# hlesmqh/WS3D

Measured on AMD Instinct MI355X. Metric: KITTI scenes/sec (16384 pts) Stage-1 RPN fwd, 1/2/4/8 GPU; FPS+group HBM GB/s, higher is better.
Workload: dtype f32

## Files before the change

### include/ws3d_ops.h

```cpp
#ifndef WS3D_OPS_H
#define WS3D_OPS_H

#include <stddef.h>
#include <stdint.h>

#ifdef __cplusplus
extern "C" {
#endif

#define WS3D_OK 0
#define WS3D_E_INVALID (-1)
#define WS3D_E_LAUNCH (-2)
#define WS3D_E_WORKSPACE (-3)
#define WS3D_E_UNSUPPORTED (-4)

#if defined(__GNUC__)
#define WS3D_API __attribute__((visibility("default")))
#else
#define WS3D_API
#endif

typedef void *ws3d_stream_t;

#define WS3D_ABI_VERSION 6
WS3D_API int ws3d_abi_version(void);
WS3D_API int ws3d_tune(int key, int value);
WS3D_API int ws3d_dist_mode(void);
WS3D_API const char *ws3d_last_error(void);
WS3D_API int ws3d_device_info(char *name, int name_len, int *cu_count, int *lds_bytes_per_block);


WS3D_API int ws3d_furthest_point_sampling(int b, int n, int m, const float *xyz, float *temp, int32_t *idx,
                                 ws3d_stream_t stream);

WS3D_API int ws3d_furthest_point_sampling_gather(int b, int n, int m, const float *xyz, float *temp,
                                        int32_t *idx, float *new_xyz, ws3d_stream_t stream);

WS3D_API size_t ws3d_fps_workspace_bytes(int b, int n);
WS3D_API int ws3d_furthest_point_sampling_ws(int b, int n, int m, const float *xyz, float *temp, int32_t *idx,
                                             float *new_xyz , void *workspace, size_t workspace_bytes,
                                             ws3d_stream_t stream);

WS3D_API int ws3d_furthest_point_sampling_nested(int b, int n, int m, const float *xyz, int32_t *idx, float *new_xyz,
                                        ws3d_stream_t stream);

WS3D_API int ws3d_furthest_point_sampling_nested_chain(int b, int n, int levels, const int *m, const float *xyz, int32_t *const *idx,
                                                       float *const *new_xyz, ws3d_stream_t stream);

WS3D_API int ws3d_fps_ragged_limit(void);
WS3D_API int ws3d_furthest_point_sampling_ragged(int clouds, const int32_t *offsets, const int32_t *sizes_host, int m, const float *xyz,
                                                 int32_t *idx, ws3d_stream_t stream);

WS3D_API int ws3d_gather_points(int b, int c, int n, int npoints, const float *points, const int32_t *idx,
                       float *out, ws3d_stream_t stream);

WS3D_API int ws3d_gather_points_grad(int b, int c, int n, int npoints, const float *grad_out,
                            const int32_t *idx, float *grad_points, ws3d_stream_t stream);

WS3D_API int ws3d_ball_query(int b, int n, int m, float radius, int nsample, const float *new_xyz,
                    const float *xyz, int32_t *idx, const void *sorted, ws3d_stream_t stream);
WS3D_API int ws3d_ball_query_fill(int b, int n, int m, float radius, int nsample, const float *new_xyz,
                         const float *xyz, int32_t *idx, const void *sorted, ws3d_stream_t stream);
WS3D_API int ws3d_ball_query_pairs(int b, int n, int m, float radius, int nsample, const float *new_xyz, const float *xyz, int32_t *idx,
                          const void *sorted_grid, int32_t *rowc, int32_t *rowsrc, int32_t *total, ws3d_stream_t stream);

WS3D_API int ws3d_ball_query_pairs2(int b, int n, int m, const float *new_xyz, const float *xyz, const void *sorted_grid,
                                    float radius0, int nsample0, int32_t *idx0, int32_t *rowc0, int32_t *rowsrc0, int32_t *total0,
                                    float radius1, int nsample1, int32_t *idx1, int32_t *rowc1, int32_t *rowsrc1, int32_t *total1,
                                    ws3d_stream_t stream);


WS3D_API size_t ws3d_sorted_points_bytes(int b, int n);
WS3D_API int ws3d_sort_points_x(int b, int n, const float *xyz, void *sorted, ws3d_stream_t stream);
WS3D_API int ws3d_sort_points_xz(int b, int n, const float *xyz, void *sorted, ws3d_stream_t stream);
WS3D_API int ws3d_sort_points_grid(int b, int n, const float *xyz, void *sorted, ws3d_stream_t stream);
WS3D_API int ws3d_sort_points_jobs(int b, int njobs, const int *n, const int *kind, const float *const *xyz, void *const *sorted,
                                   ws3d_stream_t stream);

WS3D_API int ws3d_group_points(int b, int c, int n, int npoints, int nsample, const float *points,
                      const int32_t *idx, float *out, ws3d_stream_t stream);

WS3D_API int ws3d_group_points_grad(int b, int c, int n, int npoints, int nsample, const float *grad_out,
                           const int32_t *idx, float *grad_points, ws3d_stream_t stream);

WS3D_API int ws3d_query_and_group(int b, int n, int m, int c, float radius, int nsample, int use_xyz,
                         const float *xyz, const float *new_xyz, const float *features,
                         int32_t *idx_out, float *out, const void *sorted, ws3d_stream_t stream);

WS3D_API int ws3d_three_nn(int b, int n, int m, const float *unknown, const float *known, float *dist2,
                  int32_t *idx, const void *sorted_known, ws3d_stream_t stream);

WS3D_API int ws3d_three_nn_weights(long rows, const float *dist2, float *weight, ws3d_stream_t stream);
WS3D_API int ws3d_three_nn_w(int b, int n, int m, const float *unknown, const float *known, float *dist2, int32_t *idx, float *weight,
                             const void *sorted_known, ws3d_stream_t stream);
WS3D_API int ws3d_three_nn_wq(int b, int n, int m, const float *unknown, const float *known, float *dist2, int32_t *idx, float *weight,
                              const void *sorted_known, const void *sorted_unknown, ws3d_stream_t stream);
WS3D_API int ws3d_three_nn_jobs(int b, int njobs, const int *n, const int *m, const float *const *unknown, const void *const *sorted_known,
                                float *const *dist2, int32_t *const *idx, float *const *weight, const void *const *sorted_unknown,
                                ws3d_stream_t stream);

WS3D_API int ws3d_pool_nsample(long rows, int nsample, const float *x, float *out, uint8_t *arg, ws3d_stream_t stream);
WS3D_API int ws3d_pool_nsample_grad(long rows, int nsample, const float *grad_out, const uint8_t *arg, float *grad_x,
                                    ws3d_stream_t stream);

WS3D_API int ws3d_gemm_pool(long rows, int nsample, int k_dim, int o_dim, const float *x_rows, const float *wt,
                            const float *bias, int relu, float *out, int out_stride, const int32_t *gate, long gate_limit, ws3d_stream_t stream);

WS3D_API int ws3d_gather_gemm(int b, int n, int m, int nsample, int c_feat, int o_dim, const float *feats, const float *xyz,
                     const float *new_xyz, const int32_t *nbr, const float *wt, const float *bias, int relu, float *out,
                     ws3d_stream_t stream);

WS3D_API int ws3d_gather_gemm2(int b, int n, int m, int nsample, int c_feat, int o1, int o2, const float *feats, const float *xyz,
                      const float *new_xyz, const int32_t *nbr, const float *w1t, const float *b1, int relu1, const float *w2t,
                      const float *b2, int relu2, float *out, ws3d_stream_t stream);

WS3D_API int ws3d_pgather_gemm2(int b, int n, int m, int nsample, int o1, int o2, const float *pmat, int p_stride, const float *xyz,
                       const float *new_xyz, const int32_t *nbr, const float *w1x, const float *b1, int relu1,
                       const float *w2t, const float *b2, int relu2, float *out, const int32_t *gate, long gate_limit, ws3d_stream_t stream);
WS3D_API int ws3d_pgather_rows(int b, int n, int m, int nsample, int o1, const float *pmat, int p_stride, const float *xyz, const float *new_xyz,
                      const int32_t *nbr, const float *w1x, const float *b1, int relu1, float *out, ws3d_stream_t stream);

WS3D_API int ws3d_qinterp_rows(int b, int n, int m, int o, const float *q, const int32_t *idx, const float *weight, const float *lin,
                      const float *skip, int c1, const float *wb, const float *bias, int relu, float *out, ws3d_stream_t stream);


WS3D_API int ws3d_compact_pairs(long centres, int nsample, const int32_t *nbr, int32_t *rowc, int32_t *rowsrc, int32_t *total, ws3d_stream_t stream);
WS3D_API int ws3d_compact_pairs_count(long centres, int nsample, const int32_t *nbr, int32_t *cnt, ws3d_stream_t stream);
WS3D_API int ws3d_compact_pairs_rows(long centres, int nsample, const int32_t *nbr, const int32_t *cnt, const int32_t *incl, int32_t *rowc,
                            int32_t *rowsrc, int32_t *total, ws3d_stream_t stream);
WS3D_API int ws3d_pgather_gemm2_compact(int b, int n, int m, long max_rows, int o1, int o2, const float *pmat, int p_stride, const float *xyz,
                               const float *new_xyz, const int32_t *rowc, const int32_t *rowsrc, const int32_t *total, const float *w1x,
                               const float *b1, int relu1, const float *w2t, const float *b2, int relu2, float *out, long limit, ws3d_stream_t stream);
WS3D_API int ws3d_pgather_gemm3_compact(int b, int n, int m, long max_rows, int o1, int o2, int o3, const float *pmat, int p_stride, const float *xyz,
                               const float *new_xyz, const int32_t *rowc, const int32_t *rowsrc, const int32_t *total, const float *w1x,
                               const float *b1, int relu1, const float *w2t, const float *b2, int relu2, const float *w3t, const float *b3,
                               float *out, int out_stride, long limit, ws3d_stream_t stream);
WS3D_API int ws3d_gemm_pool_compact(long max_rows, int k_dim, int o_dim, const float *x_rows, const int32_t *rowc, const int32_t *total,
                           const float *wt, const float *bias, float *out, int out_stride, long limit, ws3d_stream_t stream);
typedef struct ws3d_compact_mlp_args {
    int b, n, m;
    long max_rows;
    int o1, o2, o3;
    const float *pmat;
    int p_stride;
    const float *xyz, *new_xyz;
    const int32_t *rowc, *rowsrc, *total;
    const float *w1x, *b1;
    int relu1;
    const float *w2t, *b2;
    int relu2;
    const float *w3t, *b3;
    float *mid;
    float *out;
    int out_stride;
    long limit;
} ws3d_compact_mlp_args;
WS3D_API int ws3d_compact_mlp_pair(int kind, const ws3d_compact_mlp_args *scale0, const ws3d_compact_mlp_args *scale1, ws3d_stream_t stream);
WS3D_API int ws3d_chain_mlp3_ticket_ints(void);
WS3D_API size_t ws3d_chain_mlp3_blob_floats(int o2);
WS3D_API int ws3d_chain_mlp3_pack(const ws3d_compact_mlp_args *scale, float *blob, ws3d_stream_t stream);
WS3D_API int ws3d_chain_mlp3(const ws3d_compact_mlp_args *scale0, const ws3d_compact_mlp_args *scale1, const float *blob0, const float *blob1,
                             int32_t *ticket, int workgroups, ws3d_stream_t stream);

WS3D_API int ws3d_sa_mlp3_pool_compact(int b, int n, int m, long max_rows, int c1, int c2, int c3, const float *xyz, const float *new_xyz,
                              const float *feat, const int32_t *rowc, const int32_t *rowsrc, const int32_t *total, const float *w1t,
                              const float *b1, const float *w2t, const float *b2, const float *w3t, const float *b3, float *out,
                              int out_stride, long limit, ws3d_stream_t stream);

WS3D_API int ws3d_sa_mlp3_pool_lists(int b, int n, int m, int nsample, int c1, int c2, int c3, const float *xyz, const float *new_xyz,
                            const float *feat, const int32_t *nbr, const float *w1t, const float *b1, const float *w2t, const float *b2,
                            const float *w3t, const float *b3, int relu3, float *out, int out_stride, const int32_t *gate, long gate_limit,
                            ws3d_stream_t stream);

WS3D_API int ws3d_interp_gemm(int b, int n, int m, int c2, int c1, int o_dim, const float *known_feats, const float *unknown_feats,
                     const int32_t *idx, const float *weight, const float *wt, const float *bias, int relu, float *out,
                     ws3d_stream_t stream);

WS3D_API size_t ws3d_conv1x1_wgrad_workspace_bytes(int b, int o, int c, long l);
WS3D_API int ws3d_conv1x1_wgrad(int b, int o, int c, long l, const float *grad_out, const float *x, float *grad_w,
                                void *workspace, size_t workspace_bytes, ws3d_stream_t stream);

WS3D_API size_t ws3d_bn_workspace_bytes(int b, int c, long l);
WS3D_API int ws3d_bn_relu_train_fwd(int b, int c, long l, const float *x, const float *gamma, const float *beta, float eps,
                                    float momentum, int relu, float *running_mean, float *running_var,
                                    int64_t *num_batches_tracked, float *y, float *save_mean, float *save_invstd,
                                    void *workspace, size_t workspace_bytes, ws3d_stream_t stream);
WS3D_API int ws3d_bn_relu_train_bwd(int b, int c, long l, const float *x, const float *dy, const float *gamma,
                                    const float *beta, const float *save_mean, const float *save_invstd, int relu, float *dx,
                                    float *dgamma, float *dbeta, void *workspace, size_t workspace_bytes, ws3d_stream_t stream);

WS3D_API int ws3d_three_interpolate(int b, int c, int m, int n, const float *points, const int32_t *idx,
                           const float *weight, float *out, ws3d_stream_t stream);

WS3D_API int ws3d_three_interpolate_grad(int b, int c, int n, int m, const float *grad_out,
                                const int32_t *idx, const float *weight, float *grad_points,
                                ws3d_stream_t stream);

WS3D_API size_t ws3d_scatter_workspace_bytes(int b, int c, int n_targets, long slots_per_scene);
WS3D_API int ws3d_group_points_grad_det(int b, int c, int n, int npoints, int nsample, const float *grad_out,
                                        const int32_t *idx, float *grad_points, void *workspace,
                                        size_t workspace_bytes, ws3d_stream_t stream);
WS3D_API int ws3d_three_interpolate_grad_det(int b, int c, int n, int m, const float *grad_out, const int32_t *idx,
                                             const float *weight, float *grad_points, void *workspace,
                                             size_t workspace_bytes, ws3d_stream_t stream);

WS3D_API int ws3d_bias_act_inplace(int b, int o_ch, long l, int relu, float *y, const float *bias,
                                   ws3d_stream_t stream);

WS3D_API int ws3d_rowmax_bias_act(int b, int o_ch, long m, int s, int relu, const float *y, const float *bias,
                                  float *out, ws3d_stream_t stream);

WS3D_API int ws3d_query_and_group_nlc(int b, int n, int m, int c, float radius, int nsample, int use_xyz,
                                      const float *xyz, const float *new_xyz, const float *features_nlc,
                                      int32_t *idx_out, float *out_nlc, const void *sorted, ws3d_stream_t stream);
WS3D_API int ws3d_three_interpolate_nlc(int b, int c, int m, int n, const float *feats_nlc, const int32_t *idx,
                                        const float *weight, float *out_nlc, int out_stride, ws3d_stream_t stream);
WS3D_API int ws3d_rowmax_rows(long rows_out, int ns, int o_ch, const float *y, float *out, int out_stride,
                              ws3d_stream_t stream);

WS3D_API int ws3d_sa_mlp3_pool(long rows, int nsample, int c1, int c2, int c3, const float *x_rows4,
                               const float *w1t, const float *b1, const float *w2t, const float *b2,
                               const float *w3t, const float *b3, int relu3, float *out, int out_stride,
                               ws3d_stream_t stream);

WS3D_API int ws3d_mlp2_rows(long rows, int k_dim, int o1, int o2, const float *x_rows, const float *w1t, const float *b1, int relu1,
                   const float *w2t, const float *b2, int relu2, float *out, int *ticket, ws3d_stream_t stream);

WS3D_API size_t ws3d_rpn_heads_blob_bytes(int o2);
WS3D_API int ws3d_rpn_heads_pack(int o2, const float *w1t, const float *b1, int relu1, const float *w2t, const float *b2, int relu2, void *blob,
                        ws3d_stream_t stream);
WS3D_API int ws3d_rpn_heads(long rows, const float *x_rows, int heads, const void *blob_cls, float *out_cls, int *ticket_cls, int o2_reg,
                   const void *blob_reg, float *out_reg, int *ticket_reg, int workgroups, ws3d_stream_t stream);

WS3D_API size_t ws3d_gemm_rows_pack_bytes(int k_dim, int n_dim);
WS3D_API int ws3d_gemm_rows_pack(int k_dim, int n_dim, const float *wt, void *pack, ws3d_stream_t stream);
WS3D_API int ws3d_gemm_rows_split(long rows, int k_dim, int n_dim, const float *a, const void *pack, const float *bias, int relu, float *out,
                         ws3d_stream_t stream);

WS3D_API int ws3d_qinterp_gemm(int b, int n, int m, int c, int o_dim, const float *q, const int32_t *idx, const float *weight, const float *lin,
                      const float *skip, int c1, const float *wb, const float *b1, int relu1, const float *w2t, const float *b2, int relu2,
                      float *out, ws3d_stream_t stream);


WS3D_API int ws3d_boxes_overlap_bev(int num_a, const float *boxes_a, int num_b, const float *boxes_b,
                           float *ans, ws3d_stream_t stream);

WS3D_API int ws3d_boxes_iou_bev(int num_a, const float *boxes_a, int num_b, const float *boxes_b,
                       float *ans, ws3d_stream_t stream);

WS3D_API int ws3d_boxes_iou3d_paired(int n, const float *boxes_a, const float *boxes_b, float *overlap_bev, float *iou2d, float *iou3d,
                                     ws3d_stream_t stream);

WS3D_API int ws3d_nms_mask(int boxes_num, const float *boxes, float thresh, int normal, int full_grid,
                  uint64_t *mask, ws3d_stream_t stream);

WS3D_API size_t ws3d_nms_workspace_bytes(int boxes_num);
WS3D_API int ws3d_nms(int boxes_num, const float *boxes, float thresh, int normal, int max_keep,
                      void *workspace, size_t workspace_bytes, int64_t *keep, int32_t *num_keep,
                      ws3d_stream_t stream);

WS3D_API int ws3d_nms_batched(int batch, int boxes_num, const float *boxes, float thresh, int normal,
                              int max_keep, void *workspace, size_t workspace_bytes, int64_t *keep,
                              int32_t *num_keep, ws3d_stream_t stream);


WS3D_API int ws3d_radius_nms_batched(int batch, int n, const float *centers, float radius, int max_keep,
                                     void *workspace, size_t workspace_bytes, int64_t *keep,
                                     int32_t *num_keep, ws3d_stream_t stream);

WS3D_API int ws3d_topk_sorted(int b, int n, int k, const float *scores, float *out_scores, int64_t *out_idx,
                              ws3d_stream_t stream);
WS3D_API size_t ws3d_topk_workspace_bytes(int b, int n);
WS3D_API int ws3d_topk_sorted_ws(int b, int n, int k, const float *scores, float *out_scores, int64_t *out_idx, void *workspace,
                                 size_t workspace_bytes, ws3d_stream_t stream);
WS3D_API int ws3d_topk_sorted_sigmoid(int b, int n, int k, const float *logits, float *out_scores, int64_t *out_idx, ws3d_stream_t stream);
WS3D_API int ws3d_topk_sorted_sigmoid_ws(int b, int n, int k, const float *logits, float *out_scores, int64_t *out_idx, void *workspace,
                                         size_t workspace_bytes, ws3d_stream_t stream);

WS3D_API int ws3d_decode_center_boxes(int b, int n, int bins, float loc_scope, float loc_bin_size, float h, float w,
                                      float l, const float *xyz, const float *rpn_reg, float *boxes,
                                      ws3d_stream_t stream);

WS3D_API int ws3d_gather_boxes_bev(int b, int n, int top, const float *box, const int64_t *order, float *box_sorted, float *bev,
                          ws3d_stream_t stream);
WS3D_API int ws3d_decode_gather_boxes_bev(int b, int n, int top, int bins, float loc_scope, float loc_bin_size, float h, float w, float l,
                                          const float *xyz, const float *rpn_reg, const int64_t *order, float *box_sorted, float *bev,
                                          ws3d_stream_t stream);
WS3D_API int ws3d_select_proposals(int b, int top, int keep_stride, int k, const float *box_sorted, const float *scores_sorted,
                          const int64_t *keep, const int32_t *num, float extra_width, float *boxes_out, float *scores_out,
                          int64_t *count, float *pooled_boxes, ws3d_stream_t stream);
WS3D_API int ws3d_select_proposals_packed(int b, int top, int keep_stride, int k, const float *box_sorted, const float *scores_sorted,
                                          const int64_t *keep, const int32_t *num, float extra_width, float *boxes_out, float *scores_out,
                                          int64_t *count, float *pooled_boxes, float *packed, ws3d_stream_t stream);
WS3D_API int ws3d_select_proposals_send(int b, int top, int keep_stride, int k, const float *box_sorted, const float *scores_sorted,
                                        const int64_t *keep, const int32_t *num, float extra_width, float *boxes_out, float *scores_out,
                                        int64_t *count, float *pooled_boxes, float *send, long send_stride, ws3d_stream_t stream);
WS3D_API int ws3d_split_points_clear(long rows, int c, const float *pc, float *xyz, float *feats, void *clear, size_t clear_bytes,
                                     ws3d_stream_t stream);


WS3D_API int ws3d_roipool3d(int batch_size, int pts_num, int boxes_num, int feature_in_len,
                   int sampled_pts_num, const float *xyz, const float *boxes3d,
                   const float *pts_feature, float *pooled_features, int32_t *pooled_empty_flag,
                   int32_t *pts_idx, ws3d_stream_t stream);
WS3D_API int ws3d_roipool3d_fill(int batch_size, int pts_num, int boxes_num, int feature_in_len,
                   int sampled_pts_num, const float *xyz, const float *boxes3d,
                   const float *pts_feature, float *pooled_features, int32_t *pooled_empty_flag,
                   int32_t *pts_idx, ws3d_stream_t stream);

WS3D_API size_t ws3d_roipool3d_workspace_bytes(int batch_size, int pts_num);
WS3D_API int ws3d_roipool3d_ws(int batch_size, int pts_num, int boxes_num, int feature_in_len, int sampled_pts_num, const float *xyz,
                               const float *boxes3d, const float *pts_feature, float *pooled_features, int32_t *pooled_empty_flag,
                               int32_t *pts_idx, int fill, void *workspace, size_t workspace_bytes, ws3d_stream_t stream);


WS3D_API int ws3d_pts_in_boxes3d(int boxes_num, int pts_num, const float *pts, const float *boxes3d,
                        int64_t *flag, ws3d_stream_t stream);


WS3D_API int ws3d_instance_clouds(int batch, int pts_num, int centres_num, int feat_len, int sampled_pts_num, float radius, int mask_mode,
                                  float mask_thresh, const float *pts, const float *score, const float *feats, const float *centres,
                                  const int32_t *num, float *cloud, float *cloud_feats, int32_t *count, int32_t *pts_idx,
                                  ws3d_stream_t stream);
WS3D_API int ws3d_instance_clouds_count(int batch, int pts_num, int centres_num, float radius, const float *pts, const float *centres,
                                        const int32_t *num, int32_t *count, ws3d_stream_t stream);
WS3D_API int ws3d_instance_clouds_emit(int batch, int pts_num, int centres_num, int feat_len, float radius, int mask_mode, float mask_thresh,
                                       const float *pts, const float *score, const float *feats, const float *centres, const int32_t *num,
                                       const int64_t *offsets, float *rows, float *row_feats, int32_t *row_idx, ws3d_stream_t stream);


WS3D_API int ws3d_click_prepare(int batch, int pts_num, int clicks_num, int side, const float *offsets, float gauss_height, float gauss_status,
                                float gauss_cov, float centre_y, const float *pts, const float *clicks, const int32_t *num, float *score,
                                float *cand, int32_t *cand_num, ws3d_stream_t stream);



WS3D_API int ws3d_kitti_overlaps(int metric, int criterion, int frames, long max_pairs, const int32_t *gt_off, const int32_t *dt_off,
                                 const int64_t *out_off, const double *dt_boxes, const double *gt_boxes, double *out,
                                 ws3d_stream_t stream);

WS3D_API int ws3d_kitti_collect_scores(int frames, int max_dt, const int32_t *gt_off, const int32_t *dt_off, const int64_t *out_off,
                                       const double *overlaps, const int32_t *ignored_gt, const int32_t *ignored_dt,
                                       const double *dt_score, double min_overlap, double *tp_score, int32_t *tp_flag,
                                       ws3d_stream_t stream);

WS3D_API size_t ws3d_kitti_count_workspace_bytes(int frames, int num_thresh);
WS3D_API int ws3d_kitti_count(int metric, int frames, int max_dt, int num_thresh, const double *thresholds, const int32_t *gt_off,
                              const int32_t *dt_off, const int32_t *dc_off, const int64_t *out_off, const double *overlaps,
                              const int32_t *ignored_gt, const int32_t *ignored_dt, const double *dt_score, const double *dt_alpha,
                              const double *gt_alpha, const double *dt_bbox, const double *dc_bbox, double min_overlap, int compute_aos,
                              void *workspace, size_t workspace_bytes, double *pr, ws3d_stream_t stream);


WS3D_API int ws3d_stage2_embed(long rows, int pts_per_cloud, const float *pts, const float *box_ce, float extend, const float *wx0,
                               const float *bx0, const float *wx1, const float *bx1, const float *wf0, const float *bf0, const float *wf1,
                               const float *bf1, const float *wm, const float *bm, float *xyz_out, float *feat, ws3d_stream_t stream);
WS3D_API int ws3d_stage2_boxes(int rows, int loc_bins, int head_bins, float loc_scope, float h, float w, float l, const float *rcnn_reg,
                               float *pred_boxes3d, float *box_ce, ws3d_stream_t stream);
WS3D_API int ws3d_stage2_select(int batch, int slots, float cls_thresh, float iou_thresh, const float *size_window, float ground_y,
                                const float *box_ce, const float *rcnn_ref, const float *rcnn_cls, const float *rcnn_iou, const float *center,
                                const int32_t *num, float *boxes, int32_t *keep, float *key, ws3d_stream_t stream);

WS3D_API int ws3d_stage2_canonical_ragged(int rows, int clouds, const int32_t *offsets, const float *pts, const float *box_ce, float extend,
                                          float *pts_out, ws3d_stream_t stream);
WS3D_API int ws3d_furthest_point_sampling_ragged_gather(int clouds, const int32_t *offsets, const int32_t *sizes_host, int m, const float *xyz,
                                                        int32_t *idx, float *new_xyz, ws3d_stream_t stream);
WS3D_API int ws3d_ball_query_ragged(int clouds, const int32_t *offsets, int m, float radius, int nsample, const float *xyz, const float *new_xyz,
                                    int global_rows, int32_t *idx, ws3d_stream_t stream);

WS3D_API int ws3d_stage2_rcnn_loss(int rows, int loc_bins, int head_bins, float loc_scope, float h, float w, float l, const float *rcnn_cls,
                                   const float *rcnn_reg, const float *pred_boxes3d, const float *gt_boxes, const float *cls, float *vals,
                                   int32_t *counts, float *grad_cls, float *grad_reg, ws3d_stream_t stream);
WS3D_API int ws3d_stage2_ioun_loss(int rows, const float *rcnn_iou, const float *rcnn_ref, const float *pred_boxes3d, const float *refined_box,
                                   const float *gt_boxes, const float *cls, float *vals, int32_t *counts, float *grad_iou, float *grad_ref,
                                   ws3d_stream_t stream);

WS3D_API int ws3d_rpn_center_labels(int batch, int n, int kmax, int pts_stride, float gauss_height, float gauss_status, double gauss_cov,
                                    const float *pts, const float *centres, const int32_t *count, float *cls_label, float *reg_label,
                                    ws3d_stream_t stream);
WS3D_API size_t ws3d_rpn_loss_workspace_bytes(int rows);
WS3D_API int ws3d_rpn_loss(int rows, int bins, double loc_scope, double loc_bin_size, double alpha, double gamma, double weight_cls,
                           double weight_reg, const float *rpn_cls, const float *rpn_reg, const float *cls_label, const float *reg_label,
                           float *vals, int32_t *counts, float *grad_cls, float *grad_reg, void *workspace, size_t workspace_bytes,
                           ws3d_stream_t stream);

WS3D_API int ws3d_scan_prepare_limit(void);
WS3D_API size_t ws3d_scan_prepare_workspace_bytes(int scenes, long total_points);
WS3D_API int ws3d_scan_prepare(int scenes, const int32_t *offsets, long total_points, int max_scan_points, const float *raw, const float *calib,
                               const int32_t *img_hw, const float *scope, int npoints, uint64_t seed, const int64_t *scene_key, int key_bits,
                               float *pts_input, int32_t *src_index, int32_t *valid_count, int32_t *status, void *workspace,
                               size_t workspace_bytes, ws3d_stream_t stream);


WS3D_API int ws3d_roipool3d_plan(int batch_size, int pts_num, int boxes_num, int feature_in_len, int sampled_pts_num, int aligned16,
                                 size_t workspace_bytes);

WS3D_API int ws3d_ball_query_plan(int b, int n, int m, int c, int nsample, int fused, int nlc, int flavour, int pairs, int scales, int wide_nw,
                                  int32_t *plan);

#ifdef __cplusplus
}
#endif
#endif
```

### ws3d_amd/_lib.py

```python
from __future__ import annotations

import ctypes as C
import os

_HERE = os.path.dirname(os.path.abspath(__file__))
DIST_MODE = int(os.environ.get("WS3D_DIST_MODE", "0") or 0)
LIB_PATH = os.environ.get("WS3D_HIP_LIB") or os.path.join(
    _HERE, "libws3d_hip.so" if DIST_MODE == 0 else "libws3d_hip_dm%d.so" % DIST_MODE)

E_INVALID, E_LAUNCH, E_WORKSPACE, E_UNSUPPORTED = -1, -2, -3, -4
ABI_VERSION = 6

_vp = C.c_void_p
_i = C.c_int
_f = C.c_float
_sz = C.c_size_t

class CompactMlpArgs(C.Structure):
    _fields_ = [("b", _i), ("n", _i), ("m", _i), ("max_rows", C.c_long), ("o1", _i), ("o2", _i), ("o3", _i), ("pmat", _vp), ("p_stride", _i),
                ("xyz", _vp), ("new_xyz", _vp), ("rowc", _vp), ("rowsrc", _vp), ("total", _vp), ("w1x", _vp), ("b1", _vp), ("relu1", _i),
                ("w2t", _vp), ("b2", _vp), ("relu2", _i), ("w3t", _vp), ("b3", _vp), ("mid", _vp), ("out", _vp), ("out_stride", _i), ("limit", C.c_long)]


SIGNATURES = {
    "ws3d_abi_version": (_i, []),
    "ws3d_tune": (_i, [_i, _i]),
    "ws3d_dist_mode": (_i, []),
    "ws3d_last_error": (C.c_char_p, []),
    "ws3d_device_info": (_i, [C.c_char_p, _i, C.POINTER(_i), C.POINTER(_i)]),
    "ws3d_furthest_point_sampling": (_i, [_i, _i, _i, _vp, _vp, _vp, _vp]),
    "ws3d_furthest_point_sampling_gather": (_i, [_i, _i, _i, _vp, _vp, _vp, _vp, _vp]),
    "ws3d_furthest_point_sampling_nested": (_i, [_i, _i, _i, _vp, _vp, _vp, _vp]),
    "ws3d_furthest_point_sampling_nested_chain": (_i, [_i, _i, _i, _vp, _vp, _vp, _vp, _vp]),
    "ws3d_fps_ragged_limit": (_i, []),
    "ws3d_furthest_point_sampling_ragged": (_i, [_i, _vp, _vp, _i, _vp, _vp, _vp]),
    "ws3d_fps_workspace_bytes": (_sz, [_i, _i]),
    "ws3d_furthest_point_sampling_ws": (_i, [_i, _i, _i, _vp, _vp, _vp, _vp, _vp, _sz, _vp]),
    "ws3d_gather_points": (_i, [_i, _i, _i, _i, _vp, _vp, _vp, _vp]),
    "ws3d_gather_points_grad": (_i, [_i, _i, _i, _i, _vp, _vp, _vp, _vp]),
    "ws3d_ball_query": (_i, [_i, _i, _i, _f, _i, _vp, _vp, _vp, _vp, _vp]),
    "ws3d_ball_query_fill": (_i, [_i, _i, _i, _f, _i, _vp, _vp, _vp, _vp, _vp]),
    "ws3d_ball_query_pairs": (_i, [_i, _i, _i, _f, _i, _vp, _vp, _vp, _vp, _vp, _vp, _vp, _vp]),
    "ws3d_ball_query_pairs2": (_i, [_i, _i, _i, _vp, _vp, _vp, C.c_float, _i, _vp, _vp, _vp, _vp, C.c_float, _i, _vp, _vp, _vp, _vp, _vp]),
    "ws3d_sorted_points_bytes": (_sz, [_i, _i]),
    "ws3d_sort_points_x": (_i, [_i, _i, _vp, _vp, _vp]),
    "ws3d_sort_points_xz": (_i, [_i, _i, _vp, _vp, _vp]),
    "ws3d_sort_points_grid": (_i, [_i, _i, _vp, _vp, _vp]),
    "ws3d_sort_points_jobs": (_i, [_i, _i, _vp, _vp, _vp, _vp, _vp]),
    "ws3d_group_points": (_i, [_i, _i, _i, _i, _i, _vp, _vp, _vp, _vp]),
    "ws3d_group_points_grad": (_i, [_i, _i, _i, _i, _i, _vp, _vp, _vp, _vp]),
    "ws3d_query_and_group": (_i, [_i, _i, _i, _i, _f, _i, _i, _vp, _vp, _vp, _vp, _vp, _vp, _vp]),
    "ws3d_three_nn": (_i, [_i, _i, _i, _vp, _vp, _vp, _vp, _vp, _vp]),
    "ws3d_three_interpolate": (_i, [_i, _i, _i, _i, _vp, _vp, _vp, _vp, _vp]),
    "ws3d_three_interpolate_grad": (_i, [_i, _i, _i, _i, _vp, _vp, _vp, _vp, _vp]),
    "ws3d_bn_workspace_bytes": (C.c_size_t, [_i, _i, C.c_long]),
    "ws3d_bn_relu_train_fwd": (_i, [_i, _i, C.c_long, _vp, _vp, _vp, C.c_float, C.c_float, _i, _vp, _vp, _vp, _vp, _vp, _vp,
                                    _vp, C.c_size_t, _vp]),
    "ws3d_bn_relu_train_bwd": (_i, [_i, _i, C.c_long, _vp, _vp, _vp, _vp, _vp, _vp, _i, _vp, _vp, _vp, _vp, C.c_size_t, _vp]),
    "ws3d_conv1x1_wgrad_workspace_bytes": (C.c_size_t, [_i, _i, _i, C.c_long]),
    "ws3d_conv1x1_wgrad": (_i, [_i, _i, _i, C.c_long, _vp, _vp, _vp, _vp, C.c_size_t, _vp]),
    "ws3d_gemm_pool": (_i, [C.c_long, _i, _i, _i, _vp, _vp, _vp, _i, _vp, _i, _vp, C.c_long, _vp]),
    "ws3d_pool_nsample": (_i, [C.c_long, _i, _vp, _vp, _vp, _vp]),
    "ws3d_pool_nsample_grad": (_i, [C.c_long, _i, _vp, _vp, _vp, _vp]),
    "ws3d_scatter_workspace_bytes": (C.c_size_t, [_i, _i, _i, C.c_long]),
    "ws3d_group_points_grad_det": (_i, [_i, _i, _i, _i, _i, _vp, _vp, _vp, _vp, C.c_size_t, _vp]),
    "ws3d_three_interpolate_grad_det": (_i, [_i, _i, _i, _i, _vp, _vp, _vp, _vp, _vp, C.c_size_t, _vp]),
    "ws3d_query_and_group_nlc": (_i, [_i, _i, _i, _i, _f, _i, _i, _vp, _vp, _vp, _vp, _vp, _vp, _vp]),
    "ws3d_three_interpolate_nlc": (_i, [_i, _i, _i, _i, _vp, _vp, _vp, _vp, _i, _vp]),
    "ws3d_rowmax_rows": (_i, [C.c_long, _i, _i, _vp, _vp, _i, _vp]),
    "ws3d_sa_mlp3_pool": (_i, [C.c_long, _i, _i, _i, _i, _vp, _vp, _vp, _vp, _vp, _vp, _vp, _i, _vp, _i, _vp]),
    "ws3d_qinterp_gemm": (_i, [_i, _i, _i, _i, _i, _vp, _vp, _vp, _vp, _vp, _i, _vp, _vp, _i, _vp, _vp, _i, _vp, _vp]),
    "ws3d_mlp2_rows": (_i, [C.c_long, _i, _i, _i, _vp, _vp, _vp, _i, _vp, _vp, _i, _vp, _vp, _vp]),
    "ws3d_rpn_heads_blob_bytes": (_sz, [_i]),
    "ws3d_rpn_heads_pack": (_i, [_i, _vp, _vp, _i, _vp, _vp, _i, _vp, _vp]),
    "ws3d_rpn_heads": (_i, [C.c_long, _vp, _i, _vp, _vp, _vp, _i, _vp, _vp, _vp, _i, _vp]),
    "ws3d_gemm_rows_pack_bytes": (_sz, [_i, _i]),
    "ws3d_gemm_rows_pack": (_i, [_i, _i, _vp, _vp, _vp]),
    "ws3d_gemm_rows_split": (_i, [C.c_long, _i, _i, _vp, _vp, _vp, _i, _vp, _vp]),
    "ws3d_decode_center_boxes": (_i, [_i, _i, _i, _f, _f, _f, _f, _f, _vp, _vp, _vp, _vp]),
    "ws3d_topk_sorted": (_i, [_i, _i, _i, _vp, _vp, _vp, _vp]),
    "ws3d_topk_workspace_bytes": (C.c_size_t, [_i, _i]),
    "ws3d_topk_sorted_ws": (_i, [_i, _i, _i, _vp, _vp, _vp, _vp, C.c_size_t, _vp]),
    "ws3d_topk_sorted_sigmoid": (_i, [_i, _i, _i, _vp, _vp, _vp, _vp]),
    "ws3d_topk_sorted_sigmoid_ws": (_i, [_i, _i, _i, _vp, _vp, _vp, _vp, C.c_size_t, _vp]),
    "ws3d_three_nn_weights": (_i, [C.c_long, _vp, _vp, _vp]),
    "ws3d_three_nn_w": (_i, [_i, _i, _i, _vp, _vp, _vp, _vp, _vp, _vp, _vp]),
    "ws3d_three_nn_wq": (_i, [_i, _i, _i, _vp, _vp, _vp, _vp, _vp, _vp, _vp, _vp]),
    "ws3d_three_nn_jobs": (_i, [_i, _i, _vp, _vp, _vp, _vp, _vp, _vp, _vp, _vp, _vp]),
    "ws3d_bias_act_inplace": (_i, [_i, _i, C.c_long, _i, _vp, _vp, _vp]),
    "ws3d_rowmax_bias_act": (_i, [_i, _i, C.c_long, _i, _i, _vp, _vp, _vp, _vp]),
    "ws3d_boxes_overlap_bev": (_i, [_i, _vp, _i, _vp, _vp, _vp]),
    "ws3d_boxes_iou_bev": (_i, [_i, _vp, _i, _vp, _vp, _vp]),
    "ws3d_boxes_iou3d_paired": (_i, [_i, _vp, _vp, _vp, _vp, _vp, _vp]),
    "ws3d_nms_mask": (_i, [_i, _vp, _f, _i, _i, _vp, _vp]),
    "ws3d_nms_workspace_bytes": (_sz, [_i]),
    "ws3d_nms": (_i, [_i, _vp, _f, _i, _i, _vp, _sz, _vp, _vp, _vp]),
    "ws3d_nms_batched": (_i, [_i, _i, _vp, _f, _i, _i, _vp, _sz, _vp, _vp, _vp]),
    "ws3d_radius_nms_batched": (_i, [_i, _i, _vp, _f, _i, _vp, _sz, _vp, _vp, _vp]),
    "ws3d_gather_gemm": (_i, [_i, _i, _i, _i, _i, _i, _vp, _vp, _vp, _vp, _vp, _vp, _i, _vp, _vp]),
    "ws3d_gather_gemm2": (_i, [_i, _i, _i, _i, _i, _i, _i, _vp, _vp, _vp, _vp, _vp, _vp, _i, _vp, _vp, _i, _vp, _vp]),
    "ws3d_pgather_gemm2": (_i, [_i, _i, _i, _i, _i, _i, _vp, _i, _vp, _vp, _vp, _vp, _vp, _i, _vp, _vp, _i, _vp, _vp, C.c_long, _vp]),
    "ws3d_pgather_rows": (_i, [_i, _i, _i, _i, _i, _vp, _i, _vp, _vp, _vp, _vp, _vp, _i, _vp, _vp]),
    "ws3d_qinterp_rows": (_i, [_i, _i, _i, _i, _vp, _vp, _vp, _vp, _vp, _i, _vp, _vp, _i, _vp, _vp]),
    "ws3d_compact_pairs": (_i, [C.c_long, _i, _vp, _vp, _vp, _vp, _vp]),
    "ws3d_compact_pairs_count": (_i, [C.c_long, _i, _vp, _vp, _vp]),
    "ws3d_compact_pairs_rows": (_i, [C.c_long, _i, _vp, _vp, _vp, _vp, _vp, _vp, _vp]),
    "ws3d_pgather_gemm2_compact": (_i, [_i, _i, _i, C.c_long, _i, _i, _vp, _i, _vp, _vp, _vp, _vp, _vp, _vp, _vp, _i, _vp, _vp, _i, _vp, C.c_long, _vp]),
    "ws3d_pgather_gemm3_compact": (_i, [_i, _i, _i, C.c_long, _i, _i, _i, _vp, _i, _vp, _vp, _vp, _vp, _vp, _vp, _vp, _i, _vp, _vp, _i, _vp, _vp, _vp, _i, C.c_long, _vp]),
    "ws3d_gemm_pool_compact": (_i, [C.c_long, _i, _i, _vp, _vp, _vp, _vp, _vp, _vp, _i, C.c_long, _vp]),
    "ws3d_compact_mlp_pair": (_i, [_i, C.POINTER(CompactMlpArgs), C.POINTER(CompactMlpArgs), _vp]),
    "ws3d_chain_mlp3_ticket_ints": (_i, []),
    "ws3d_chain_mlp3_blob_floats": (_sz, [_i]),
    "ws3d_chain_mlp3_pack": (_i, [C.POINTER(CompactMlpArgs), _vp, _vp]),
    "ws3d_chain_mlp3": (_i, [C.POINTER(CompactMlpArgs), C.POINTER(CompactMlpArgs), _vp, _vp, _vp, _i, _vp]),
    "ws3d_sa_mlp3_pool_compact": (_i, [_i, _i, _i, C.c_long, _i, _i, _i, _vp, _vp, _vp, _vp, _vp, _vp, _vp, _vp, _vp, _vp, _vp, _vp, _vp, _i, C.c_long, _vp]),
    "ws3d_sa_mlp3_pool_lists": (_i, [_i, _i, _i, _i, _i, _i, _i, _vp, _vp, _vp, _vp, _vp, _vp, _vp, _vp, _vp, _vp, _i, _vp, _i, _vp, C.c_long, _vp]),
    "ws3d_interp_gemm": (_i, [_i, _i, _i, _i, _i, _i, _vp, _vp, _vp, _vp, _vp, _vp, _i, _vp, _vp]),
    "ws3d_gather_boxes_bev": (_i, [_i, _i, _i, _vp, _vp, _vp, _vp, _vp]),
    "ws3d_select_proposals": (_i, [_i, _i, _i, _i, _vp, _vp, _vp, _vp, _f, _vp, _vp, _vp, _vp, _vp]),
    "ws3d_decode_gather_boxes_bev": (_i, [_i, _i, _i, _i, _f, _f, _f, _f, _f, _vp, _vp, _vp, _vp, _vp, _vp]),
    "ws3d_select_proposals_packed": (_i, [_i, _i, _i, _i, _vp, _vp, _vp, _vp, _f, _vp, _vp, _vp, _vp, _vp, _vp]),
    "ws3d_select_proposals_send": (_i, [_i, _i, _i, _i, _vp, _vp, _vp, _vp, _f, _vp, _vp, _vp, _vp, _vp, C.c_long, _vp]),
    "ws3d_split_points_clear": (_i, [C.c_long, _i, _vp, _vp, _vp, _vp, C.c_size_t, _vp]),
    "ws3d_roipool3d": (_i, [_i, _i, _i, _i, _i, _vp, _vp, _vp, _vp, _vp, _vp, _vp]),
    "ws3d_roipool3d_fill": (_i, [_i, _i, _i, _i, _i, _vp, _vp, _vp, _vp, _vp, _vp, _vp]),
    "ws3d_roipool3d_workspace_bytes": (C.c_size_t, [_i, _i]),
    "ws3d_roipool3d_ws": (_i, [_i, _i, _i, _i, _i, _vp, _vp, _vp, _vp, _vp, _vp, _i, _vp, C.c_size_t, _vp]),
    "ws3d_pts_in_boxes3d": (_i, [_i, _i, _vp, _vp, _vp, _vp]),
    "ws3d_instance_clouds": (_i, [_i, _i, _i, _i, _i, _f, _i, _f, _vp, _vp, _vp, _vp, _vp, _vp, _vp, _vp, _vp, _vp]),
    "ws3d_instance_clouds_count": (_i, [_i, _i, _i, _f, _vp, _vp, _vp, _vp, _vp]),
    "ws3d_instance_clouds_emit": (_i, [_i, _i, _i, _i, _f, _i, _f, _vp, _vp, _vp, _vp, _vp, _vp, _vp, _vp, _vp, _vp]),
    "ws3d_click_prepare": (_i, [_i, _i, _i, _i, _vp, _f, _f, _f, _f, _vp, _vp, _vp, _vp, _vp, _vp, _vp]),
    "ws3d_kitti_overlaps": (_i, [_i, _i, _i, C.c_long, _vp, _vp, _vp, _vp, _vp, _vp, _vp]),
    "ws3d_kitti_collect_scores": (_i, [_i, _i, _vp, _vp, _vp, _vp, _vp, _vp, _vp, C.c_double, _vp, _vp, _vp]),
    "ws3d_kitti_count_workspace_bytes": (_sz, [_i, _i]),
    "ws3d_kitti_count": (_i, [_i, _i, _i, _i, _vp, _vp, _vp, _vp, _vp, _vp, _vp, _vp, _vp, _vp, _vp, _vp, _vp, C.c_double, _i, _vp,
                              _sz, _vp, _vp]),
    "ws3d_stage2_embed": (_i, [C.c_long, _i, _vp, _vp, _f] + [_vp] * 10 + [_vp, _vp, _vp]),
    "ws3d_stage2_boxes": (_i, [_i, _i, _i, _f, _f, _f, _f, _vp, _vp, _vp, _vp]),
    "ws3d_stage2_select": (_i, [_i, _i, _f, _f, C.POINTER(_f), _f, _vp, _vp, _vp, _vp, _vp, _vp, _vp, _vp, _vp, _vp]),
    "ws3d_stage2_canonical_ragged": (_i, [_i, _i, _vp, _vp, _vp, _f, _vp, _vp]),
    "ws3d_furthest_point_sampling_ragged_gather": (_i, [_i, _vp, _vp, _i, _vp, _vp, _vp, _vp]),
    "ws3d_ball_query_ragged": (_i, [_i, _vp, _i, _f, _i, _vp, _vp, _i, _vp, _vp]),
    "ws3d_stage2_rcnn_loss": (_i, [_i, _i, _i, _f, _f, _f, _f] + [_vp] * 9 + [_vp]),
    "ws3d_stage2_ioun_loss": (_i, [_i] + [_vp] * 10 + [_vp]),
    "ws3d_rpn_center_labels": (_i, [_i, _i, _i, _i, _f, _f, C.c_double] + [_vp] * 5 + [_vp]),
    "ws3d_rpn_loss_workspace_bytes": (_sz, [_i]),
    "ws3d_rpn_loss": (_i, [_i, _i] + [C.c_double] * 6 + [_vp] * 8 + [_vp, _sz, _vp]),
    "ws3d_scan_prepare_limit": (_i, []),
    "ws3d_scan_prepare_workspace_bytes": (_sz, [_i, C.c_long]),
    "ws3d_scan_prepare": (_i, [_i, _vp, C.c_long, _i, _vp, _vp, _vp, _vp, _i, C.c_uint64, _vp, _i, _vp, _vp, _vp, _vp, _vp, _sz, _vp]),
    "ws3d_roipool3d_plan": (_i, [_i, _i, _i, _i, _i, _i, _sz]),
    "ws3d_ball_query_plan": (_i, [_i, _i, _i, _i, _i, _i, _i, _i, _i, _i, _i, _vp]),
}


class Ws3dError(RuntimeError):
    pass


_lib = None


def load() -> C.CDLL:
    global _lib
    if _lib is not None:
        return _lib
    if not os.path.exists(LIB_PATH):
        raise Ws3dError(
            f"{LIB_PATH} is missing: the MI355X HIP library has not been built "
            "(run `python -m ws3d_amd.build`).  ws3d_amd has no CPU fallback.")
    import torch
    try:
        lib = C.CDLL(LIB_PATH)
    except OSError as e:
        raise Ws3dError(f"cannot load {LIB_PATH}: {e}") from e
    for name, (res, args) in SIGNATURES.items():
        fn = getattr(lib, name)
        fn.restype = res
        fn.argtypes = args
    if lib.ws3d_abi_version() != ABI_VERSION:
        raise Ws3dError(f"{LIB_PATH} exports ABI version {lib.ws3d_abi_version()}, this package binds version {ABI_VERSION}: "
                        "rebuild it (`python -m ws3d_amd.build`)")
    if not os.environ.get("WS3D_HIP_LIB") and lib.ws3d_dist_mode() != DIST_MODE:
        raise Ws3dError(f"{LIB_PATH} was built with WS3D_DIST_MODE={lib.ws3d_dist_mode()}, expected {DIST_MODE}: rebuild it")
    _lib = lib
    return lib


def check(rc: int, what: str = "") -> None:
    if rc != 0:
        msg = load().ws3d_last_error()
        raise Ws3dError(f"{what or 'ws3d'} failed (rc={rc}): {msg.decode() if msg else ''}")
```

### ws3d_amd/build.py

```python
from __future__ import annotations

import argparse
import concurrent.futures as cf
import glob
import os
import shutil
import subprocess
import sys

HERE = os.path.dirname(os.path.abspath(__file__))
CSRC = os.path.join(HERE, "csrc")
OBJ = os.path.join(CSRC, "build")
LIB = os.path.join(HERE, "libws3d_hip.so")
DIST_MODES = (0, 1, 2)


def lib_path(dist_mode: int = 0) -> str:
    return LIB if dist_mode == 0 else os.path.join(HERE, "libws3d_hip_dm%d.so" % dist_mode)
ARCH = "gfx950"
SOURCES = ["core.hip", "fps.hip", "fps_v3.hip", "fps_bucket.hip", "fps_nested.hip", "fps_ragged.hip", "fps_pruned.hip", "ballquery_group.hip", "interpolate.hip", "roipool3d.hip", "iou3d.hip", "proposals.hip", "scatter_det.hip", "sa_mlp.hip", "bn_relu.hip", "gemm_pool.hip", "conv_wgrad.hip", "chain_mlp.hip", "rpn_heads.hip", "gemm_rows.hip", "kitti_eval.hip", "instance_clouds.hip", "click.hip", "stage2.hip", "stage2_ragged.hip", "stage2_loss.hip", "rpn_targets.hip", "scan_prepare.hip"]
CXXFLAGS = ["-O3", "-std=c++17", "-fPIC", "-ffp-contract=off", "-fno-fast-math",
            "-fvisibility=hidden", "-Wall", "-Wno-unused-function"]


def hipcc() -> str:
    for cand in (os.environ.get("HIPCC"), shutil.which("hipcc"), "/opt/rocm/bin/hipcc"):
        if cand and os.path.exists(cand):
            return cand
    raise RuntimeError("hipcc not found (looked at $HIPCC, PATH, /opt/rocm/bin)")


def _deps(src: str):
    return [src, *glob.glob(os.path.join(CSRC, "*.h")), os.path.join(HERE, "..", "include", "ws3d_ops.h"),
            os.path.join(CSRC, "exports.map"), os.path.abspath(__file__)]


def _compile(src: str, force: bool, verbose: bool, dist_mode: int = 0) -> str:
    path = os.path.join(CSRC, src)
    obj = os.path.join(OBJ if dist_mode == 0 else OBJ + "_dm%d" % dist_mode, os.path.splitext(src)[0] + ".o")
    if not force and os.path.exists(obj) and all(
            os.path.getmtime(obj) >= os.path.getmtime(d) for d in _deps(path)):
        return obj
    cmd = [hipcc(), f"--offload-arch={ARCH}", *CXXFLAGS, f"-DWS3D_DIST_MODE={dist_mode}", *os.environ.get("WS3D_EXTRA_DEFS", "").split(), "-c", path, "-o", obj]
    if verbose:
        print(" ".join(cmd), flush=True)
    r = subprocess.run(cmd, capture_output=True, text=True)
    if r.returncode != 0:
        raise RuntimeError(f"hipcc failed for {src}:\n{r.stdout}\n{r.stderr}")
    if verbose and r.stderr.strip():
        print(r.stderr)
    return obj


def build(force: bool = False, verbose: bool = False, dist_mode: int = 0) -> str:
    LIB = lib_path(dist_mode)
    os.makedirs(OBJ if dist_mode == 0 else OBJ + "_dm%d" % dist_mode, exist_ok=True)
    with cf.ThreadPoolExecutor(max_workers=min(len(SOURCES), os.cpu_count() or 4, 16)) as ex:
        objs = list(ex.map(lambda s: _compile(s, force, verbose, dist_mode), SOURCES))
    if force or not os.path.exists(LIB) or any(os.path.getmtime(o) > os.path.getmtime(LIB) for o in objs):
        cmd = [hipcc(), f"--offload-arch={ARCH}", "-shared", "-fPIC", "-Wl,--version-script=" + os.path.join(CSRC, "exports.map"), "-o", LIB, *objs]
        if verbose:
            print(" ".join(cmd), flush=True)
        r = subprocess.run(cmd, capture_output=True, text=True)
        if r.returncode != 0:
            raise RuntimeError(f"link failed:\n{r.stdout}\n{r.stderr}")
    return LIB


def rebuild_one(src: str, verbose: bool = False) -> str:
    _compile(src, True, verbose)
    objs = [os.path.join(OBJ, os.path.splitext(s_)[0] + ".o") for s_ in SOURCES]
    missing = [o for o in objs if not os.path.exists(o)]
    if missing:
        return build(False, verbose)
    cmd = [hipcc(), f"--offload-arch={ARCH}", "-shared", "-fPIC", "-Wl,--version-script=" + os.path.join(CSRC, "exports.map"), "-o", LIB, *objs]
    r = subprocess.run(cmd, capture_output=True, text=True)
    if r.returncode != 0:
        raise RuntimeError(f"link failed:\n{r.stdout}\n{r.stderr}")
    return LIB


if __name__ == "__main__":
    ap = argparse.ArgumentParser()
    ap.add_argument("--force", action="store_true")
    ap.add_argument("--verbose", action="store_true")
    ap.add_argument("--dist-mode", type=int, default=0, choices=DIST_MODES)
    ap.add_argument("--all-dist-modes", action="store_true")
    ap.add_argument("--only", default=None, help="recompile this one source (forced) and relink")
    a = ap.parse_args()
    if a.only:
        print(rebuild_one(a.only, a.verbose))
        sys.exit(0)
    for dm in (DIST_MODES if a.all_dist_modes else (a.dist_mode,)):
        print(build(a.force, a.verbose, dm))
    sys.exit(0)
```

### ws3d_amd/compat.py

```python
from __future__ import annotations

import sys
import types

import os

import torch

from . import _lib
from ._lib import Ws3dError, check


def _dev(*tensors):
    dev = None
    for t in tensors:
        if t is None:
            continue
        if not t.is_cuda:
            raise Ws3dError("ws3d_amd ops need HIP ('cuda') tensors; there is no CPU fallback")
        if not t.is_contiguous():
            raise Ws3dError("ws3d_amd ops need contiguous tensors (the reference asserts the same)")
        if dev is None:
            dev = t.device
        elif t.device != dev:
# ... 378 lines not shown
    with _on(dev):
        check(_lib.load().ws3d_rowmax_rows(R, ns, O, _p(y), view.data_ptr(), out.size(1), _stream()), "rowmax_rows")
    return out


def bn_relu_train_fwd(x, gamma, beta, running_mean, running_var, momentum, eps, relu=True, num_batches_tracked=None):
    dev = _dev(x, gamma, beta, running_mean, running_var, num_batches_tracked)
    if num_batches_tracked is not None and num_batches_tracked.dtype != torch.int64:
        raise TypeError("num_batches_tracked must be int64")
    _f32(x, "x"); _f32(gamma, "gamma"); _f32(beta, "beta")
    b, c = x.size(0), x.size(1)
    l = x.numel() // max(b * c, 1)
    y = torch.empty_like(x)
    mean = torch.empty((c,), dtype=torch.float32, device=dev)
    invstd = torch.empty((c,), dtype=torch.float32, device=dev)
    lib = _lib.load()
    nbytes = lib.ws3d_bn_workspace_bytes(b, c, l)
    ws = torch.empty((nbytes + 7) // 8, dtype=torch.float64, device=dev)
    with _on(dev):
        check(lib.ws3d_bn_relu_train_fwd(b, c, l, _p(x), _p(gamma), _p(beta), float(eps), float(momentum), int(bool(relu)),
                                         _p(running_mean), _p(running_var), _p(num_batches_tracked), _p(y), _p(mean), _p(invstd), _p(ws), nbytes,
                                         _stream()), "bn_relu_train_fwd")
    return y, mean, invstd


def bn_relu_train_bwd(x, dy, gamma, beta, save_mean, save_invstd, relu=True):
    dev = _dev(x, dy, gamma, beta, save_mean, save_invstd)
    _f32(x, "x"); _f32(dy, "dy")
    b, c = x.size(0), x.size(1)
    l = x.numel() // max(b * c, 1)
    dx = torch.empty_like(x)
    dgamma = torch.empty((c,), dtype=torch.float32, device=dev)
    dbeta = torch.empty((c,), dtype=torch.float32, device=dev)
    lib = _lib.load()
    nbytes = lib.ws3d_bn_workspace_bytes(b, c, l)
    ws = torch.empty((nbytes + 7) // 8, dtype=torch.float64, device=dev)
    with _on(dev):
        check(lib.ws3d_bn_relu_train_bwd(b, c, l, _p(x), _p(dy), _p(gamma), _p(beta), _p(save_mean), _p(save_invstd),
                                         int(bool(relu)), _p(dx), _p(dgamma), _p(dbeta), _p(ws), nbytes, _stream()),
              "bn_relu_train_bwd")
    return dx, dgamma, dbeta


def conv1x1_wgrad(grad_out, x, shape=None):
    dev = _dev(grad_out, x)
    _f32(grad_out, "grad_out"); _f32(x, "x")
    b, o, c = x.size(0), grad_out.size(1), x.size(1)
    l = x.numel() // max(b * c, 1)
    if grad_out.numel() != b * o * l:
        raise Ws3dError("conv1x1_wgrad: grad_out and x disagree in shape")
    gw = torch.empty((o, c) if shape is None else tuple(shape), dtype=torch.float32, device=dev)
    lib = _lib.load()
    nbytes = lib.ws3d_conv1x1_wgrad_workspace_bytes(b, o, c, l)
    ws = torch.empty((nbytes + 3) // 4, dtype=torch.float32, device=dev)
    with _on(dev):
        check(lib.ws3d_conv1x1_wgrad(b, o, c, l, _p(grad_out), _p(x), _p(gw), _p(ws), nbytes, _stream()), "conv1x1_wgrad")
    return gw


def _gate(gate):
    if gate is None:
        return None, 0
    total, limit = gate
    return total.data_ptr(), int(limit)


def gemm_pool(x_rows, wt, bias, relu, nsample, out, col0=0, gate=None):
    dev = _dev(x_rows, wt, bias)
    _f32(x_rows, "x_rows"); _f32(wt, "wt")
    rows, k = x_rows.shape
    o = wt.size(1)
    if rows % 64 or rows // 64 > 65535 or o % 64 or k % 4 or nsample not in (16, 32) or wt.size(0) != k:
        return False
    view = out[:, col0:col0 + o]
    with _on(dev):
        check(_lib.load().ws3d_gemm_pool(rows, nsample, k, o, _p(x_rows), _p(wt), _p(bias), int(bool(relu)), view.data_ptr(),
                                         out.size(1), *_gate(gate), _stream()), "gemm_pool")
    return True


def gather_gemm(feats, xyz, new_xyz, nbr, wt_feat_then_xyz, bias, relu):
    dev = _dev(feats, xyz, new_xyz, nbr, wt_feat_then_xyz)
    _f32(feats, "feats"); _f32(xyz, "xyz"); _f32(new_xyz, "new_xyz"); _i32(nbr, "nbr"); _f32(wt_feat_then_xyz, "wt")
    B, N, C = feats.shape
    M, ns = nbr.size(1), nbr.size(2)
    O = wt_feat_then_xyz.size(1)
    rows = B * M * ns
    if C % 4 or O % 64 or rows % 64 or rows // 64 > 65535 or wt_feat_then_xyz.size(0) != C + 3 or not feats.is_contiguous():
        return None
    out = torch.empty((rows, O), dtype=torch.float32, device=dev)
    with _on(dev):
        check(_lib.load().ws3d_gather_gemm(B, N, M, ns, C, O, _p(feats), _p(xyz), _p(new_xyz), _p(nbr), _p(wt_feat_then_xyz), _p(bias),
                                           int(bool(relu)), _p(out), _stream()), "gather_gemm")
    return out


def gather_gemm2(feats, xyz, new_xyz, nbr, w1t_feat_then_xyz, b1, relu1, w2t, b2, relu2):
    dev = _dev(feats, xyz, new_xyz, nbr, w1t_feat_then_xyz, w2t)
    _f32(feats, "feats"); _f32(xyz, "xyz"); _f32(new_xyz, "new_xyz"); _i32(nbr, "nbr"); _f32(w1t_feat_then_xyz, "w1t"); _f32(w2t, "w2t")
    B, N, C = feats.shape
    M, ns = nbr.size(1), nbr.size(2)
    O1, O2 = w1t_feat_then_xyz.size(1), w2t.size(1)
    rows = B * M * ns
    if (C % 4 or O1 not in (64, 128, 256) or O2 % 4 or rows % 64 or w1t_feat_then_xyz.size(0) != C + 3 or w2t.size(0) != O1 or
            not feats.is_contiguous() or not w2t.is_contiguous() or not w1t_feat_then_xyz.is_contiguous()):
        return None
    out = torch.empty((rows, O2), dtype=torch.float32, device=dev)
    with _on(dev):
        check(_lib.load().ws3d_gather_gemm2(B, N, M, ns, C, O1, O2, _p(feats), _p(xyz), _p(new_xyz), _p(nbr), _p(w1t_feat_then_xyz), _p(b1),
                                            int(bool(relu1)), _p(w2t), _p(b2), int(bool(relu2)), _p(out), _stream()), "gather_gemm2")
    return out


def pgather_gemm2(pmat, col0, o1, xyz, new_xyz, nbr, w1x, b1, relu1, w2t, b2, relu2, out=None, gate=None):
    dev = _dev(pmat, xyz, new_xyz, nbr, w1x, w2t)
    _f32(pmat, "pmat"); _f32(xyz, "xyz"); _f32(new_xyz, "new_xyz"); _i32(nbr, "nbr"); _f32(w1x, "w1x"); _f32(w2t, "w2t")
    B, N = xyz.size(0), xyz.size(1)
    M, ns = nbr.size(1), nbr.size(2)
    O2 = w2t.size(1)
    if (o1 not in (64, 128) or O2 % 4 or (M * ns) % 64 or pmat.dim() != 2 or pmat.size(0) != B * N or pmat.stride(1) != 1 or
            col0 < 0 or col0 + o1 > pmat.size(1) or tuple(w1x.shape) != (3, o1) or w2t.size(0) != o1 or not w1x.is_contiguous() or not w2t.is_contiguous()):
        return None
    if out is None:
        out = torch.empty((B * M * ns, O2), dtype=torch.float32, device=dev)
    elif tuple(out.shape) != (B * M * ns, O2) or not out.is_contiguous():
        raise ValueError("pgather_gemm2: out must be a contiguous (B*M*ns, O2) tensor")
    with _on(dev):
        check(_lib.load().ws3d_pgather_gemm2(B, N, M, ns, o1, O2, pmat.data_ptr() + 4 * col0, pmat.stride(0), _p(xyz), _p(new_xyz), _p(nbr), _p(w1x), _p(b1),
                                             int(bool(relu1)), _p(w2t), _p(b2), int(bool(relu2)), _p(out), *_gate(gate), _stream()), "pgather_gemm2")
    return out


def pgather_rows(pmat, col0, o1, xyz, new_xyz, nbr, w1x, b1, relu1):
    dev = _dev(pmat, xyz, new_xyz, nbr, w1x)
    _f32(pmat, "pmat"); _f32(xyz, "xyz"); _f32(new_xyz, "new_xyz"); _i32(nbr, "nbr"); _f32(w1x, "w1x")
    B, N = xyz.size(0), xyz.size(1)
    M, ns = nbr.size(1), nbr.size(2)
    if (o1 % 4 or col0 % 4 or pmat.dim() != 2 or pmat.size(0) != B * N or pmat.stride(1) != 1 or pmat.stride(0) % 4 or col0 < 0 or
            col0 + o1 > pmat.size(1) or tuple(w1x.shape) != (3, o1) or not w1x.is_contiguous() or pmat.data_ptr() % 16):
        return None
    out = torch.empty((B * M * ns, o1), dtype=torch.float32, device=dev)
    with _on(dev):
        check(_lib.load().ws3d_pgather_rows(B, N, M, ns, o1, pmat.data_ptr() + 4 * col0, pmat.stride(0), _p(xyz), _p(new_xyz), _p(nbr), _p(w1x), _p(b1),
                                            int(bool(relu1)), _p(out), _stream()), "pgather_rows")
    return out


def qinterp_rows(q, idx, weight, lin=None, skip=None, wb=None, bias=None, relu=True):
    dev = _dev(q, idx, weight)
    _f32(q, "q"); _i32(idx, "idx"); _f32(weight, "weight")
    B, M, O = q.shape
    N = idx.size(1)
    c1 = 0 if skip is None else skip.size(2)
    if (O % 4 or not q.is_contiguous() or (lin is None and c1 > 4) or (lin is not None and (tuple(lin.shape) != (B * N, O) or not lin.is_contiguous())) or
            (lin is None and c1 > 0 and (wb is None or tuple(wb.shape) != (c1, O) or not wb.is_contiguous() or not skip.is_contiguous()))):
        return None
    out = torch.empty((B * N, O), dtype=torch.float32, device=dev)
    with _on(dev):
        check(_lib.load().ws3d_qinterp_rows(B, N, M, O, _p(q), _p(idx), _p(weight), _p(lin), _p(skip), c1, _p(wb), _p(bias), int(bool(relu)), _p(out),
                                            _stream()), "qinterp_rows")
    return out


def qinterp_gemm(q, idx, weight, w2t, b2, relu2, lin=None, skip=None, wb=None, bias=None, relu=True):
    dev = _dev(q, idx, weight, w2t)
    _f32(q, "q"); _i32(idx, "idx"); _f32(weight, "weight"); _f32(w2t, "w2t")
    B, M, C = q.shape
    N = idx.size(1)
    O = w2t.size(1)
    c1 = 0 if skip is None else skip.size(2)
    if ((B * N) % 64 or C % 16 or O % 128 or w2t.size(0) != C or not q.is_contiguous() or not w2t.is_contiguous() or not idx.is_contiguous() or
            not weight.is_contiguous() or (lin is None and c1 > 4) or (lin is not None and (tuple(lin.shape) != (B * N, C) or not lin.is_contiguous())) or
            (lin is None and c1 > 0 and (wb is None or tuple(wb.shape) != (c1, C) or not wb.is_contiguous() or not skip.is_contiguous()))):
        return None
    out = torch.empty((B * N, O), dtype=torch.float32, device=dev)
    with _on(dev):
        check(_lib.load().ws3d_qinterp_gemm(B, N, M, C, O, _p(q), _p(idx), _p(weight), _p(lin), _p(skip), c1, _p(wb), _p(bias), int(bool(relu)), _p(w2t),
                                            _p(b2), int(bool(relu2)), _p(out), _stream()), "qinterp_gemm")
    return out


def compact_pairs(nbr, ordered=False):
    if not ordered:
        dev = _dev(nbr)
        _i32(nbr, "nbr")
        B, M, ns = nbr.shape
        rowc = torch.empty(B * M * ns, dtype=torch.int32, device=dev)
        rowsrc = torch.empty(B * M * ns, dtype=torch.int32, device=dev)
        total = torch.zeros(1, dtype=torch.int32, device=dev)
        with _on(dev):
            check(_lib.load().ws3d_compact_pairs(B * M, ns, _p(nbr), _p(rowc), _p(rowsrc), _p(total), _stream()), "compact_pairs")
        return rowc, rowsrc, total
    dev = _dev(nbr)
    _i32(nbr, "nbr")
    B, M, ns = nbr.shape
    centres = B * M
    cnt = torch.empty(centres, dtype=torch.int32, device=dev)
    rowc = torch.empty(centres * ns, dtype=torch.int32, device=dev)
    rowsrc = torch.empty(centres * ns, dtype=torch.int32, device=dev)
    total = torch.empty(1, dtype=torch.int32, device=dev)
    with _on(dev):
        lib = _lib.load()
        check(lib.ws3d_compact_pairs_count(centres, ns, _p(nbr), _p(cnt), _stream()), "compact_pairs_count")
        incl = torch.cumsum(cnt, dim=0, dtype=torch.int32)
        check(lib.ws3d_compact_pairs_rows(centres, ns, _p(nbr), _p(cnt), _p(incl), _p(rowc), _p(rowsrc), _p(total), _stream()), "compact_pairs_rows")
    return rowc, rowsrc, total


def pgather_gemm2_compact(pmat, col0, o1, xyz, new_xyz, pairs, w1x, b1, relu1, w2t, b2, relu2, limit=-1):
    rowc, rowsrc, total = pairs
    dev = _dev(pmat, xyz, new_xyz, rowc, w1x, w2t)
    _f32(pmat, "pmat"); _f32(xyz, "xyz"); _f32(new_xyz, "new_xyz"); _f32(w1x, "w1x"); _f32(w2t, "w2t")
    B, N = xyz.size(0), xyz.size(1)
    M = new_xyz.size(1)
    O2 = w2t.size(1)
    rows = rowc.numel()
    if (o1 not in (64, 128, 256) or O2 % 4 or pmat.dim() != 2 or pmat.size(0) != B * N or pmat.stride(1) != 1 or col0 < 0 or col0 + o1 > pmat.size(1) or
            tuple(w1x.shape) != (3, o1) or w2t.size(0) != o1 or not w1x.is_contiguous() or not w2t.is_contiguous()):
        return None
    out = torch.empty((rows, O2), dtype=torch.float32, device=dev)
    with _on(dev):
        check(_lib.load().ws3d_pgather_gemm2_compact(B, N, M, rows, o1, O2, pmat.data_ptr() + 4 * col0, pmat.stride(0), _p(xyz), _p(new_xyz), _p(rowc),
                                                     _p(rowsrc), _p(total), _p(w1x), _p(b1), int(bool(relu1)), _p(w2t), _p(b2), int(bool(relu2)), _p(out),
                                                     int(limit), _stream()), "pgather_gemm2_compact")
    return out


def pgather_gemm3_compact(pmat, col0, o1, xyz, new_xyz, pairs, w1x, b1, relu1, w2t, b2, relu2, w3t, b3, out2d, col_offset, limit=-1, max_lds=160 * 1024):
    rowc, rowsrc, total = pairs
    dev = _dev(pmat, xyz, new_xyz, rowc, w1x, w2t, w3t, out2d)
    _f32(pmat, "pmat"); _f32(xyz, "xyz"); _f32(new_xyz, "new_xyz"); _f32(w1x, "w1x"); _f32(w2t, "w2t"); _f32(w3t, "w3t"); _f32(out2d, "out2d")
    B, N = xyz.size(0), xyz.size(1)
    M = new_xyz.size(1)
    O2, O3 = w2t.size(1), w3t.size(1)
    rows = rowc.numel()
    lds = 4 * ((o1 + (O2 + 15) // 16 * 16) * 65 + 2 * 16 * 64)
    if (o1 not in (64, 128) or O2 % 4 or O3 % 128 or lds > min(max_lds, 160 * 1024 - 1024) or pmat.dim() != 2 or pmat.size(0) != B * N or pmat.stride(1) != 1 or
            col0 < 0 or col0 + o1 > pmat.size(1) or tuple(w1x.shape) != (3, o1) or w2t.size(0) != o1 or w3t.size(0) != O2 or not w1x.is_contiguous() or
            not w2t.is_contiguous() or not w3t.is_contiguous() or out2d.dim() != 2 or out2d.stride(1) != 1 or col_offset < 0 or col_offset + O3 > out2d.size(1)):
        return False
    with _on(dev):
        check(_lib.load().ws3d_pgather_gemm3_compact(B, N, M, rows, o1, O2, O3, pmat.data_ptr() + 4 * col0, pmat.stride(0), _p(xyz), _p(new_xyz), _p(rowc),
                                                     _p(rowsrc), _p(total), _p(w1x), _p(b1), int(bool(relu1)), _p(w2t), _p(b2), int(bool(relu2)), _p(w3t), _p(b3),
                                                     out2d.data_ptr() + 4 * col_offset, out2d.stride(0), int(limit), _stream()), "pgather_gemm3_compact")
    return True


def gemm_pool_compact(x_rows, pairs, wt, bias, out2d, col_offset, limit=-1):
    rowc, rowsrc, total = pairs
    dev = _dev(x_rows, rowc, wt, out2d)
    _f32(x_rows, "x_rows"); _f32(wt, "wt"); _f32(out2d, "out2d")
    rows, k = x_rows.shape
    o = wt.size(1)
    if (k % 4 or o % 64 or wt.size(0) != k or rows != rowc.numel() or not x_rows.is_contiguous() or not wt.is_contiguous() or out2d.dim() != 2 or
            out2d.stride(1) != 1 or col_offset < 0 or col_offset + o > out2d.size(1)):
        return False
    with _on(dev):
        check(_lib.load().ws3d_gemm_pool_compact(rows, k, o, _p(x_rows), _p(rowc), _p(total), _p(wt), _p(bias), out2d.data_ptr() + 4 * col_offset,
                                                 out2d.stride(0), int(limit), _stream()), "gemm_pool_compact")
    return True


def compact_mlp_pair(kind, scales, max_lds=160 * 1024, mids=None):
    import ctypes as C
    if len(scales) != 2 or scales[0]["o1"] != scales[1]["o1"]:
        return None if kind == 2 else False
    blocks, keep, outs = [], [], []
    for si, a in enumerate(scales):
        rowc, rowsrc, total = a["pairs"]
        pmat, xyz, new_xyz, w1x, w2t, w3t, out2d, o1, col0, col = a["pmat"], a["xyz"], a["new_xyz"], a["w1x"], a["w2t"], a["w3t"], a["out2d"], a["o1"], a["col0"], a["col_offset"]
        dev = _dev(pmat, xyz, new_xyz, rowc, w1x, w2t, w3t, out2d)
        for t_, nm in ((pmat, "pmat"), (xyz, "xyz"), (new_xyz, "new_xyz"), (w1x, "w1x"), (w2t, "w2t"), (w3t, "w3t"), (out2d, "out2d")):
            _f32(t_, nm)
        B, N, M = xyz.size(0), xyz.size(1), new_xyz.size(1)
        O2, O3 = w2t.size(1), w3t.size(1)
        rows = rowc.numel()
        lds3 = 4 * ((o1 + (O2 + 15) // 16 * 16) * 65 + 2 * 16 * 64)
        ok = (O2 % 4 == 0 and pmat.dim() == 2 and pmat.size(0) == B * N and pmat.stride(1) == 1 and col0 >= 0 and col0 + o1 <= pmat.size(1) and
              tuple(w1x.shape) == (3, o1) and w2t.size(0) == o1 and w3t.size(0) == O2 and w1x.is_contiguous() and w2t.is_contiguous() and w3t.is_contiguous() and
              out2d.dim() == 2 and out2d.stride(1) == 1 and col >= 0 and col + O3 <= out2d.size(1))
        if kind == 3:
            ok = ok and o1 in (64, 128) and O3 % 128 == 0 and lds3 <= min(max_lds, 160 * 1024 - 1024)
        elif kind == 2:
            ok = ok and o1 in (64, 128, 256)
        else:
            ok = ok and O3 % 64 == 0 and mids is not None and tuple(mids[si].shape) == (rows, O2) and mids[si].is_contiguous()
        if not ok:
            return None if kind == 2 else False
        mid = mids[si] if kind == 1 else (torch.empty((rows, O2), dtype=torch.float32, device=dev) if kind == 2 else None)
        outs.append(mid)
        keep.append((pmat, xyz, new_xyz, rowc, rowsrc, total, w1x, w2t, w3t, out2d, mid, a["b1"], a["b2"], a["b3"]))
        blocks.append(_lib.CompactMlpArgs(B, N, M, rows, o1, O2, O3, pmat.data_ptr() + 4 * col0, pmat.stride(0), _p(xyz), _p(new_xyz), _p(rowc), _p(rowsrc),
                                          _p(total), _p(w1x), _p(a["b1"]), int(bool(a["relu1"])), _p(w2t), _p(a["b2"]), int(bool(a["relu2"])), _p(w3t), _p(a["b3"]),
                                          _p(mid), out2d.data_ptr() + 4 * col, out2d.stride(0), -1))
    with _on(dev):
        rc = _lib.load().ws3d_compact_mlp_pair(int(kind), C.byref(blocks[0]), C.byref(blocks[1]), _stream())
    if rc == _lib.E_UNSUPPORTED:
        return None if kind == 2 else False
    check(rc, "compact_mlp_pair")
    return outs if kind == 2 else True


CHAIN_WORKGROUPS = 0
TUNE_KEYS = {"chain_wgs": 0, "mlp2_wgs": 1, "sa1_wgs": 2, "fp_wgs": 3, "pair_wgs": 4, "bq_wide_nw": 5}


def tune(name: str, value: int = -1) -> int:
    rc = _lib.load().ws3d_tune(TUNE_KEYS[name], int(value))
    if rc < 0:
        check(rc, "tune")
    return rc


_CHAIN_BLOBS = {}


def chain_ticket_ints() -> int:
    return int(_lib.load().ws3d_chain_mlp3_ticket_ints())


def _chain_blob(block, tensors, dev):
    import ctypes as C
    key = tuple((t.data_ptr(), t._version) if t is not None else None for t in tensors)
    hit = _CHAIN_BLOBS.get(key)
    if hit is None:
        n = int(_lib.load().ws3d_chain_mlp3_blob_floats(block.o2))
        blob = torch.empty(n, dtype=torch.float32, device=dev)
        with _on(dev):
            check(_lib.load().ws3d_chain_mlp3_pack(C.byref(block), _p(blob), _stream()), "chain_mlp3_pack")
        if torch.cuda.is_current_stream_capturing():
            return blob
        hit = _CHAIN_BLOBS[key] = (blob, tensors)
    return hit[0]


def chain_mlp3(scales, ticket):
    import ctypes as C
    if len(scales) not in (1, 2) or ticket is None or ticket.dtype != torch.int32 or ticket.numel() < chain_ticket_ints() or not ticket.is_contiguous():
        return False
    blocks, keep, blobs = [], [], []
    for a in scales:
        rowc, rowsrc, total = a["pairs"]
        pmat, xyz, new_xyz, w1x, w2t, w3t, out2d, o1, col0, col = a["pmat"], a["xyz"], a["new_xyz"], a["w1x"], a["w2t"], a["w3t"], a["out2d"], a["o1"], a["col0"], a["col_offset"]
        dev = _dev(pmat, xyz, new_xyz, rowc, w1x, w2t, w3t, out2d, ticket)
        for t_, nm in ((pmat, "pmat"), (xyz, "xyz"), (new_xyz, "new_xyz"), (w1x, "w1x"), (w2t, "w2t"), (w3t, "w3t"), (out2d, "out2d")):
            _f32(t_, nm)
        B, N, M = xyz.size(0), xyz.size(1), new_xyz.size(1)
        O2, O3 = w2t.size(1), w3t.size(1)
        ok = (o1 == 64 and O2 <= 96 and O3 == 128 and pmat.dim() == 2 and pmat.size(0) == B * N and pmat.stride(1) == 1 and pmat.stride(0) % 4 == 0 and
              col0 >= 0 and col0 % 4 == 0 and col0 + o1 <= pmat.size(1) and tuple(w1x.shape) == (3, o1) and w2t.size(0) == o1 and w3t.size(0) == O2 and
              w1x.is_contiguous() and w2t.is_contiguous() and w3t.is_contiguous() and out2d.dim() == 2 and out2d.stride(1) == 1 and col >= 0 and
              col % 4 == 0 and col + O3 <= out2d.size(1) and xyz.is_contiguous() and new_xyz.is_contiguous())
        if not ok:
            return False
        keep.append((pmat, xyz, new_xyz, rowc, rowsrc, total, w1x, w2t, w3t, out2d, a["b1"], a["b2"], a["b3"]))
        blocks.append(_lib.CompactMlpArgs(B, N, M, rowc.numel(), o1, O2, O3, pmat.data_ptr() + 4 * col0, pmat.stride(0), _p(xyz), _p(new_xyz), _p(rowc), _p(rowsrc),
                                          _p(total), _p(w1x), _p(a["b1"]), int(bool(a["relu1"])), _p(w2t), _p(a["b2"]), int(bool(a["relu2"])), _p(w3t), _p(a["b3"]),
                                          None, out2d.data_ptr() + 4 * col, out2d.stride(0), int(a.get("limit", -1))))
        blobs.append(_chain_blob(blocks[-1], (w1x, a["b1"], w2t, a["b2"], w3t, a["b3"]), dev))
    with _on(dev):
        rc = _lib.load().ws3d_chain_mlp3(C.byref(blocks[0]), C.byref(blocks[1]) if len(blocks) > 1 else None, _p(blobs[0]), _p(blobs[1]) if len(blobs) > 1 else None,
                                         _p(ticket), int(CHAIN_WORKGROUPS), _stream())
    if rc == _lib.E_UNSUPPORTED:
        return False
    check(rc, "chain_mlp3")
    return True


def interp_gemm(known_feats, unknown_feats, idx, weight, wt, bias, relu):
    dev = _dev(known_feats, idx, weight, wt)
    _f32(known_feats, "known_feats"); _i32(idx, "idx"); _f32(weight, "weight"); _f32(wt, "wt")
    B, M, C2 = known_feats.shape
    N = idx.size(1)
    C1 = 0 if unknown_feats is None else unknown_feats.size(2)
    O = wt.size(1)
    rows = B * N
    if (C2 % 4 or O % 64 or rows % 64 or rows // 64 > 65535 or wt.size(0) != C2 + C1 or not known_feats.is_contiguous() or
            (unknown_feats is not None and not unknown_feats.is_contiguous())):
        return None
    out = torch.empty((rows, O), dtype=torch.float32, device=dev)
    with _on(dev):
        check(_lib.load().ws3d_interp_gemm(B, N, M, C2, C1, O, _p(known_feats), _p(unknown_feats), _p(idx), _p(weight), _p(wt), _p(bias),
                                           int(bool(relu)), _p(out), _stream()), "interp_gemm")
    return out


def mlp2_rows(x2d, w1t, b1, relu1, w2t, b2, relu2, ticket=None):
    dev = _dev(x2d, w1t, w2t)
    _f32(x2d, "x2d"); _f32(w1t, "w1t"); _f32(w2t, "w2t")
    R, K = x2d.shape
    O1, O2 = w1t.size(1), w2t.size(1)
    if (K != 128 or O1 != 128 or w1t.size(0) != 128 or w2t.size(0) != 128 or O2 > 64 or R % 32 or not x2d.is_contiguous() or
            not w1t.is_contiguous() or not w2t.is_contiguous()):
        return None
    out = torch.empty((R, O2), dtype=torch.float32, device=dev)
    if ticket is None:
        ticket = torch.zeros(1, dtype=torch.int32, device=dev)
    with _on(dev):
        check(_lib.load().ws3d_mlp2_rows(R, K, O1, O2, _p(x2d), _p(w1t), _p(b1), int(bool(relu1)), _p(w2t), _p(b2), int(bool(relu2)),
                                         _p(out), _p(ticket), _stream()), "mlp2_rows")
    return out


def rpn_heads_pack(w1t, b1, relu1, w2t, b2, relu2):
    dev = _dev(w1t, w2t)
    _f32(w1t, "w1t"); _f32(w2t, "w2t")
    O2 = w2t.size(1) if w2t.dim() == 2 else 0
    n = int(_lib.load().ws3d_rpn_heads_blob_bytes(O2))
    if n == 0 or tuple(w1t.shape) != (128, 128) or w2t.size(0) != 128 or not w1t.is_contiguous() or not w2t.is_contiguous():
        return None
    for b, nm, o in ((b1, "b1", 128), (b2, "b2", O2)):
        if b is not None:
            _f32(b, nm)
            if b.numel() != o or not b.is_contiguous():
                return None
    blob = torch.empty((n + 15) // 16 * 4, dtype=torch.float32, device=dev)
    with _on(dev):
        check(_lib.load().ws3d_rpn_heads_pack(O2, _p(w1t), _p(b1), int(bool(relu1)), _p(w2t), _p(b2), int(bool(relu2)), _p(blob), _stream()),
              "rpn_heads_pack")
    return blob


def rpn_heads(x2d, heads, blob_cls, blob_reg, o2_reg, tickets, workgroups=0):
    dev = _dev(x2d)
    _f32(x2d, "x2d")
    if (x2d.dim() != 2 or x2d.size(1) != 128 or x2d.size(0) % 32 or not x2d.is_contiguous() or heads not in (1, 2, 3) or
            tickets is None or tickets.dtype != torch.int32 or tickets.numel() < 2 or not tickets.is_contiguous()):
        return None
    R = x2d.size(0)
    out_cls = torch.empty((R, 1), dtype=torch.float32, device=dev) if heads & 1 else None
    out_reg = torch.empty((R, int(o2_reg)), dtype=torch.float32, device=dev) if heads & 2 else None
    with _on(dev):
        rc = _lib.load().ws3d_rpn_heads(R, _p(x2d), int(heads), _p(blob_cls) if heads & 1 else None, _p(out_cls), _p(tickets[0:1]),
                                        int(o2_reg) if heads & 2 else 0, _p(blob_reg) if heads & 2 else None, _p(out_reg), _p(tickets[1:2]),
                                        int(workgroups), _stream())
    if rc == _lib.E_UNSUPPORTED:
        return None
    check(rc, "rpn_heads")
    return out_cls, out_reg


def gemm_rows_pack(wt):
    dev = _dev(wt)
    _f32(wt, "wt")
    if wt.dim() != 2:
        return None
    K, N = wt.shape
    n = int(_lib.load().ws3d_gemm_rows_pack_bytes(K, N))
    if n == 0:
        return None
    pack = torch.empty((n + 15) // 16 * 4, dtype=torch.float32, device=dev)
    with _on(dev):
        check(_lib.load().ws3d_gemm_rows_pack(K, N, _p(wt), _p(pack), _stream()), "gemm_rows_pack")
    return pack


def gemm_rows_split(x2d, pack, n_dim, bias=None, relu=False, out=None):
    if pack is None or x2d.dim() != 2 or not x2d.is_contiguous() or (bias is not None and (not bias.is_contiguous() or bias.numel() != n_dim)):
        return None
    dev = _dev(x2d, pack, bias, out)
    _f32(x2d, "x2d")
    R, K = x2d.shape
    n_dim = int(n_dim)
    if R % 64 or K % 32 or n_dim % 64 or pack.numel() * pack.element_size() < K * n_dim * 6:
        return None
    if bias is not None:
        _f32(bias, "bias")
    if out is None:
        out = torch.empty((R, n_dim), dtype=torch.float32, device=dev)
    elif tuple(out.shape) != (R, n_dim) or out.dtype != torch.float32:
        return None
    with _on(dev):
        rc = _lib.load().ws3d_gemm_rows_split(R, K, n_dim, _p(x2d), _p(pack), _p(bias), int(bool(relu)), _p(out), _stream())
    if rc == _lib.E_UNSUPPORTED:
        return None
    check(rc, "gemm_rows_split")
    return out


def pool_nsample(x):
    dev = _dev(x)
    _f32(x, "x")
    ns = x.size(-1)
    out = torch.empty(x.shape[:-1], dtype=torch.float32, device=dev)
    arg = torch.empty(x.shape[:-1], dtype=torch.uint8, device=dev)
    with _on(dev):
        check(_lib.load().ws3d_pool_nsample(out.numel(), ns, _p(x), _p(out), _p(arg), _stream()), "pool_nsample")
    return out, arg


def pool_nsample_grad(grad_out, arg, nsample):
    dev = _dev(grad_out, arg)
    _f32(grad_out, "grad_out")
    if arg.dtype != torch.uint8 or not arg.is_contiguous():
        raise TypeError("arg must be a contiguous uint8 tensor")
    grad_x = torch.empty(tuple(grad_out.shape) + (nsample,), dtype=torch.float32, device=dev)
    with _on(dev):
        check(_lib.load().ws3d_pool_nsample_grad(grad_out.numel(), nsample, _p(grad_out), _p(arg), _p(grad_x), _stream()),
              "pool_nsample_grad")
    return grad_x


SA_MLP3_SHAPES = {(16, 16, 32), (32, 32, 64)}


def sa_mlp3_pool(x_rows4, nsample, layers, out, col0=0):
    (w1, b1, r1), (w2, b2, r2), (w3, b3, r3) = layers
    widths = (w1.size(1), w2.size(1), w3.size(1))
    if (x_rows4.size(1) != 4 or widths not in SA_MLP3_SHAPES or nsample not in (16, 32) or not (r1 and r2)
            or b1 is None or b2 is None or b3 is None):
        return False
    dev = _dev(x_rows4, out)
    view = out[:, col0:col0 + widths[2]]
    with _on(dev):
        check(_lib.load().ws3d_sa_mlp3_pool(x_rows4.size(0), nsample, widths[0], widths[1], widths[2], _p(x_rows4),
                                            _p(w1), _p(b1), _p(w2), _p(b2), _p(w3), _p(b3), int(bool(r3)),
                                            view.data_ptr(), out.size(1), _stream()), "sa_mlp3_pool")
    return True


def sa_mlp3_pool_compact(xyz, new_xyz, feat1, pairs, layers, out, col0=0, limit=-1):
    (w1, b1, r1), (w2, b2, r2), (w3, b3, r3) = layers
    widths = (w1.size(1), w2.size(1), w3.size(1))
    if (widths not in ((16, 16, 32), (32, 32, 64)) or w1.size(0) != 4 or not (r1 and r2 and r3) or b1 is None or b2 is None or b3 is None or
            feat1.numel() != xyz.size(0) * xyz.size(1) or not feat1.is_contiguous()):
        return False
    rowc, rowsrc, total = pairs
    dev = _dev(xyz, new_xyz, feat1, rowc, out)
    _f32(xyz, "xyz"); _f32(new_xyz, "new_xyz"); _f32(feat1, "feat1"); _f32(out, "out")
    view = out[:, col0:col0 + widths[2]]
    with _on(dev):
        check(_lib.load().ws3d_sa_mlp3_pool_compact(xyz.size(0), xyz.size(1), new_xyz.size(1), rowc.numel(), widths[0], widths[1], widths[2], _p(xyz),
                                                    _p(new_xyz), _p(feat1), _p(rowc), _p(rowsrc), _p(total), _p(w1), _p(b1), _p(w2), _p(b2), _p(w3),
                                                    _p(b3), view.data_ptr(), out.size(1), int(limit), _stream()), "sa_mlp3_pool_compact")
    return True


def sa_mlp3_pool_lists(xyz, new_xyz, feat1, nbr, layers, out, col0=0, gate=None):
    (w1, b1, r1), (w2, b2, r2), (w3, b3, r3) = layers
    widths = (w1.size(1), w2.size(1), w3.size(1))
    ns = nbr.size(2)
    if (widths not in ((16, 16, 32), (32, 32, 64)) or w1.size(0) != 4 or ns not in (16, 32) or not (r1 and r2) or b1 is None or b2 is None or b3 is None or
            feat1.numel() != xyz.size(0) * xyz.size(1) or not feat1.is_contiguous() or nbr.numel() % 32):
        return False
    dev = _dev(xyz, new_xyz, feat1, nbr, out)
    _f32(xyz, "xyz"); _f32(new_xyz, "new_xyz"); _f32(feat1, "feat1"); _i32(nbr, "nbr"); _f32(out, "out")
    view = out[:, col0:col0 + widths[2]]
    with _on(dev):
        check(_lib.load().ws3d_sa_mlp3_pool_lists(xyz.size(0), xyz.size(1), new_xyz.size(1), ns, widths[0], widths[1], widths[2], _p(xyz), _p(new_xyz),
                                                  _p(feat1), _p(nbr), _p(w1), _p(b1), _p(w2), _p(b2), _p(w3), _p(b3), int(bool(r3)), view.data_ptr(),
                                                  out.size(1), *_gate(gate), _stream()), "sa_mlp3_pool_lists")
    return True


def three_nn_wrapper(b, n, m, unknown_tensor, known_tensor, dist2_tensor, idx_tensor, sorted_known=None):
    dev = _dev(unknown_tensor, known_tensor, dist2_tensor, idx_tensor)
    _f32(unknown_tensor, "unknown"); _f32(known_tensor, "known"); _i32(idx_tensor, "idx")
    with _on(dev):
        check(_lib.load().ws3d_three_nn(b, n, m, _p(unknown_tensor), _p(known_tensor), _p(dist2_tensor),
                                         _p(idx_tensor), _p(sorted_known) if sorted_known is not None else None,
                                         _stream()), "three_nn")


def three_interpolate_wrapper(b, c, m, n, points_tensor, idx_tensor, weight_tensor, out_tensor):
    dev = _dev(points_tensor, idx_tensor, weight_tensor, out_tensor)
    _f32(points_tensor, "points"); _i32(idx_tensor, "idx"); _f32(weight_tensor, "weight")
    with _on(dev):
        check(_lib.load().ws3d_three_interpolate(b, c, m, n, _p(points_tensor), _p(idx_tensor),
                                                  _p(weight_tensor), _p(out_tensor), _stream()),
              "three_interpolate")


def three_interpolate_grad_wrapper(b, c, n, m, grad_out_tensor, idx_tensor, weight_tensor, grad_points_tensor):
    dev = _dev(grad_out_tensor, idx_tensor, weight_tensor, grad_points_tensor)
    _f32(grad_out_tensor, "grad_out"); _i32(idx_tensor, "idx"); _f32(weight_tensor, "weight")
    with _on(dev):
        check(_lib.load().ws3d_three_interpolate_grad(b, c, n, m, _p(grad_out_tensor), _p(idx_tensor),
                                                       _p(weight_tensor), _p(grad_points_tensor), _stream()),
              "three_interpolate_grad")


def group_points_grad_det(b, c, n, npoints, nsample, grad_out_tensor, idx_tensor, grad_points_tensor):
    dev = _dev(grad_out_tensor, idx_tensor, grad_points_tensor)
    _f32(grad_out_tensor, "grad_out"); _i32(idx_tensor, "idx"); _f32(grad_points_tensor, "grad_points")
    lib = _lib.load()
    nbytes = lib.ws3d_scatter_workspace_bytes(b, c, n, npoints * nsample)
    ws = torch.empty(max(nbytes, 256), dtype=torch.uint8, device=dev)
    with _on(dev):
        check(lib.ws3d_group_points_grad_det(b, c, n, npoints, nsample, _p(grad_out_tensor), _p(idx_tensor),
                                             _p(grad_points_tensor), _p(ws), nbytes, _stream()), "group_points_grad_det")
    return 1


def three_interpolate_grad_det(b, c, n, m, grad_out_tensor, idx_tensor, weight_tensor, grad_points_tensor):
    dev = _dev(grad_out_tensor, idx_tensor, weight_tensor, grad_points_tensor)
    _f32(grad_out_tensor, "grad_out"); _i32(idx_tensor, "idx"); _f32(weight_tensor, "weight")
    lib = _lib.load()
    nbytes = lib.ws3d_scatter_workspace_bytes(b, c, m, n * 3)
    ws = torch.empty(max(nbytes, 256), dtype=torch.uint8, device=dev)
    with _on(dev):
        check(lib.ws3d_three_interpolate_grad_det(b, c, n, m, _p(grad_out_tensor), _p(idx_tensor), _p(weight_tensor),
                                                  _p(grad_points_tensor), _p(ws), nbytes, _stream()),
              "three_interpolate_grad_det")
    return 1


def topk_sorted(scores, k, spread=None, sigmoid=False):
    dev = _dev(scores)
    _f32(scores, "scores")
    B, N = scores.shape
    vals = torch.empty((B, k), dtype=torch.float32, device=dev)
    idx = torch.empty((B, k), dtype=torch.int64, device=dev)
    lib = _lib.load()
    if spread is None:
        spread = TOPK_SEGMENTS and not torch.cuda.is_current_stream_capturing()
    need = int(lib.ws3d_topk_workspace_bytes(B, N)) if spread else 0
    with _on(dev):
        if need:
            ws = torch.empty(need // 8, dtype=torch.int64, device=dev)
            check((lib.ws3d_topk_sorted_sigmoid_ws if sigmoid else lib.ws3d_topk_sorted_ws)(B, N, k, _p(scores), _p(vals), _p(idx), _p(ws), need,
                                                                                            _stream()), "topk_sorted")
        else:
            check((lib.ws3d_topk_sorted_sigmoid if sigmoid else lib.ws3d_topk_sorted)(B, N, k, _p(scores), _p(vals), _p(idx), _stream()), "topk_sorted")
    return vals, idx


def decode_center_boxes(xyz, rpn_reg, loc_scope, loc_bin_size, mean_size):
    dev = _dev(xyz, rpn_reg)
    _f32(xyz, "xyz"); _f32(rpn_reg, "rpn_reg")
    B, N = xyz.size(0), xyz.size(1)
    bins = int(loc_scope / loc_bin_size) * 2
    if rpn_reg.size(2) != 4 * bins or not rpn_reg.is_contiguous() or not xyz.is_contiguous():
        raise ValueError("decode_center_boxes: rpn_reg must be contiguous (B,N,%d)" % (4 * bins))
    boxes = torch.empty((B, N, 7), dtype=torch.float32, device=dev)
    h, w, l = mean_size
    with _on(dev):
        check(_lib.load().ws3d_decode_center_boxes(B, N, bins, float(loc_scope), float(loc_bin_size), float(h), float(w),
                                                   float(l), _p(xyz), _p(rpn_reg), _p(boxes), _stream()), "decode_center_boxes")
    return boxes


def decode_gather_boxes_bev(xyz, rpn_reg, order, loc_scope, loc_bin_size, mean_size):
    dev = _dev(xyz, rpn_reg, order)
    _f32(xyz, "xyz"); _f32(rpn_reg, "rpn_reg")
    B, N, top = xyz.size(0), xyz.size(1), order.size(1)
    bins = int(loc_scope / loc_bin_size) * 2
    if rpn_reg.size(2) != 4 * bins or not rpn_reg.is_contiguous() or not xyz.is_contiguous():
        raise ValueError("decode_gather_boxes_bev: rpn_reg must be contiguous (B,N,%d)" % (4 * bins))
    if order.dtype != torch.int64 or not order.is_contiguous():
        raise ValueError("decode_gather_boxes_bev: order must be a contiguous int64 tensor")
    out = torch.empty((B, top, 7), dtype=torch.float32, device=dev)
    bev = torch.empty((B, top, 5), dtype=torch.float32, device=dev)
    h, w, l = mean_size
    with _on(dev):
        check(_lib.load().ws3d_decode_gather_boxes_bev(B, N, top, bins, float(loc_scope), float(loc_bin_size), float(h), float(w), float(l),
                                                       _p(xyz), _p(rpn_reg), _p(order), _p(out), _p(bev), _stream()), "decode_gather_boxes_bev")
    return out, bev


def split_points_clear(pointcloud, clear=None):
    dev = _dev(pointcloud) if clear is None else _dev(pointcloud, clear)
    _f32(pointcloud, "pointcloud")
    if not pointcloud.is_contiguous() or pointcloud.dim() != 3 or pointcloud.size(2) < 3:
        raise ValueError("split_points_clear: pointcloud must be a contiguous (B,N,C>=3) tensor")
    B, N, Cc = pointcloud.shape
    xyz = torch.empty((B, N, 3), dtype=torch.float32, device=dev)
    feats = torch.empty((B, N, Cc - 3), dtype=torch.float32, device=dev) if Cc > 3 else None
    nbytes = 0 if clear is None else clear.numel() * clear.element_size()
    if clear is not None and (not clear.is_contiguous() or nbytes % 16 or clear.data_ptr() % 16):
        raise ValueError("split_points_clear: `clear` must be contiguous, 16-byte aligned and a multiple of 16 bytes long")
    with _on(dev):
        check(_lib.load().ws3d_split_points_clear(B * N, Cc, _p(pointcloud), _p(xyz), _p(feats), _p(clear), nbytes, _stream()), "split_points_clear")
    return xyz, feats


def gather_boxes_bev(box, order):
    dev = _dev(box, order)
    _f32(box, "box")
    if order.dtype != torch.int64 or not order.is_contiguous() or not box.is_contiguous():
        raise ValueError("gather_boxes_bev: box must be contiguous fp32 and order contiguous int64")
    B, N, top = box.size(0), box.size(1), order.size(1)
    box_sorted = torch.empty((B, top, 7), dtype=torch.float32, device=dev)
    bev = torch.empty((B, top, 5), dtype=torch.float32, device=dev)
    with _on(dev):
        check(_lib.load().ws3d_gather_boxes_bev(B, N, top, _p(box), _p(order), _p(box_sorted), _p(bev), _stream()), "gather_boxes_bev")
    return box_sorted, bev


def select_proposals(box_sorted, scores_sorted, keep, num, k, extra_width=None, packed=False):
    dev = _dev(box_sorted, scores_sorted, keep, num)
    _f32(box_sorted, "box_sorted"); _f32(scores_sorted, "scores")
    if keep.dtype != torch.int64 or num.dtype != torch.int32:
        raise ValueError("select_proposals: keep must be int64 and num int32 (ws3d_nms_batched outputs)")
    B, top = box_sorted.size(0), box_sorted.size(1)
    boxes = torch.empty((B, k, 7), dtype=torch.float32, device=dev)
    scores = torch.empty((B, k), dtype=torch.float32, device=dev)
    count = torch.empty((B,), dtype=torch.int64, device=dev)
    pooled = torch.empty((B, k, 7), dtype=torch.float32, device=dev) if extra_width is not None else None
    send = packed if torch.is_tensor(packed) else None
    if send is not None:
        if send.dtype != torch.float32 or send.device != dev or send.dim() != 2 or send.size(0) < B or send.size(1) != k * 8 + 1 or not send.is_contiguous():
            raise ValueError("select_proposals: the send buffer must be a contiguous float32 (>= %d, %d) tensor on %s, got %s %s"
                             % (B, k * 8 + 1, dev, tuple(send.shape), send.dtype))
        with _on(dev):
            check(_lib.load().ws3d_select_proposals_send(B, top, keep.size(1), k, _p(box_sorted.contiguous()), _p(scores_sorted.contiguous()),
                                                         _p(keep), _p(num), float(extra_width or 0.0), _p(boxes), _p(scores), _p(count), _p(pooled),
                                                         _p(send), k * 8 + 1, _stream()), "select_proposals")
        return boxes, scores, count, pooled, send[:B, :k * 8].unflatten(1, (k, 8))
    pk = torch.empty((B, k, 8), dtype=torch.float32, device=dev) if packed else None
    with _on(dev):
        if packed:
            check(_lib.load().ws3d_select_proposals_packed(B, top, keep.size(1), k, _p(box_sorted.contiguous()), _p(scores_sorted.contiguous()),
                                                           _p(keep), _p(num), float(extra_width or 0.0), _p(boxes), _p(scores), _p(count), _p(pooled),
                                                           _p(pk), _stream()), "select_proposals")
        else:
            check(_lib.load().ws3d_select_proposals(B, top, keep.size(1), k, _p(box_sorted.contiguous()), _p(scores_sorted.contiguous()),
                                                    _p(keep), _p(num), float(extra_width or 0.0), _p(boxes), _p(scores), _p(count), _p(pooled),
                                                    _stream()), "select_proposals")
    return (boxes, scores, count, pooled, pk) if packed else (boxes, scores, count, pooled)


def bias_act_inplace(y, bias, relu=True):
    dev = _dev(y, bias)
    _f32(y, "y"); _f32(bias, "bias")
    B, O = y.size(0), y.size(1)
    L = y.numel() // max(B * O, 1)
    with _on(dev):
        check(_lib.load().ws3d_bias_act_inplace(B, O, L, int(bool(relu)), _p(y), _p(bias), _stream()), "bias_act")
    return y


def rowmax_bias_act(y, bias=None, relu=True):
    dev = _dev(y) if bias is None else _dev(y, bias)
    _f32(y, "y")
    if bias is not None:
        _f32(bias, "bias")
    B, O, M, S = y.shape
    out = torch.empty((B, O, M), dtype=torch.float32, device=dev)
    with _on(dev):
        check(_lib.load().ws3d_rowmax_bias_act(B, O, M, S, int(bool(relu)), _p(y), _p(bias) if bias is not None else None,
                                               _p(out), _stream()), "rowmax_bias_act")
    return out


def boxes_overlap_bev_gpu(boxes_a, boxes_b, ans_overlap):
    dev = _dev(boxes_a, boxes_b, ans_overlap)
    _f32(boxes_a, "boxes_a"); _f32(boxes_b, "boxes_b"); _f32(ans_overlap, "ans")
    with _on(dev):
        check(_lib.load().ws3d_boxes_overlap_bev(boxes_a.size(0), _p(boxes_a), boxes_b.size(0), _p(boxes_b),
                                                  _p(ans_overlap), _stream()), "boxes_overlap_bev")
    return 1


def boxes_iou_bev_gpu(boxes_a, boxes_b, ans_iou):
    dev = _dev(boxes_a, boxes_b, ans_iou)
    _f32(boxes_a, "boxes_a"); _f32(boxes_b, "boxes_b"); _f32(ans_iou, "ans")
    with _on(dev):
        check(_lib.load().ws3d_boxes_iou_bev(boxes_a.size(0), _p(boxes_a), boxes_b.size(0), _p(boxes_b),
                                              _p(ans_iou), _stream()), "boxes_iou_bev")
    return 1


def boxes_iou3d_paired(boxes_a, boxes_b):
    dev = _dev(boxes_a, boxes_b)
    _f32(boxes_a, "boxes_a"); _f32(boxes_b, "boxes_b")
    if boxes_a.dim() != 2 or boxes_a.size(1) != 7 or boxes_a.shape != boxes_b.shape:
        raise ValueError("boxes_iou3d_paired: boxes must both be (n,7), got %s and %s" % (tuple(boxes_a.shape), tuple(boxes_b.shape)))
    n = boxes_a.size(0)
    out = torch.empty((3, n), dtype=torch.float32, device=dev)
    if n == 0:
        return out[0], out[1], out[2]
    with _on(dev):
        check(_lib.load().ws3d_boxes_iou3d_paired(n, _p(boxes_a), _p(boxes_b), _p(out[0]), _p(out[1]), _p(out[2]), _stream()), "boxes_iou3d_paired")
    return out[0], out[1], out[2]


def nms_device(boxes, thresh, normal=False, max_keep=0):
    dev = _dev(boxes)
    _f32(boxes, "boxes")
    n = boxes.size(0)
# ... 506 lines not shown
```

### ws3d_amd/csrc/common.h

```cpp
#pragma once
#include <hip/hip_runtime.h>
#include <stdint.h>

#include "../../include/ws3d_ops.h"

#define WS3D_WAVE 64

namespace ws3d {

void set_error(const char *fmt, ...);
int check_launch(const char *what);
int raise_lds_cap(const void *fn, size_t bytes, const char *what);
int cu_count();

typedef float floatx16 __attribute__((ext_vector_type(16)));

enum : int { TUNE_CHAIN_WGS = 0, TUNE_MLP2_WGS = 1, TUNE_SA1_WGS = 2, TUNE_FP_WGS = 3, TUNE_PAIR_WGS = 4, TUNE_BQ_WIDE_NW = 5, TUNE_COUNT = 8 };
extern int g_tune[TUNE_COUNT];

static inline hipStream_t as_stream(ws3d_stream_t s) { return reinterpret_cast<hipStream_t>(s); }

#ifndef WS3D_DIST_MODE
#define WS3D_DIST_MODE 0
#endif
__device__ __forceinline__ float sqdist3(float dx, float dy, float dz) {
#if WS3D_DIST_MODE == 0
    return __builtin_fmaf(dz, dz, __builtin_fmaf(dx, dx, dy * dy));
#elif WS3D_DIST_MODE == 1
    return (dx * dx + dy * dy) + dz * dz;
#else
    return __builtin_fmaf(dz, dz, __builtin_fmaf(dy, dy, dx * dx));
#endif
}

__device__ __forceinline__ float cosf_cr(float a) { return (float)cos((double)a); }
__device__ __forceinline__ float sinf_cr(float a) { return (float)sin((double)a); }
__device__ __forceinline__ float atan2f_cr(float y, float x) { return (float)atan2((double)y, (double)x); }

template <int CTRL>
__device__ __forceinline__ float dpp_f(float v) {
    return __builtin_bit_cast(
        float, __builtin_amdgcn_update_dpp(0, __builtin_bit_cast(int, v), CTRL, 0xF, 0xF, false));
}
enum : int {
    DPP_QUAD_XOR1 = 0xB1,
    DPP_QUAD_XOR2 = 0x4E,
    DPP_ROW_HALF_MIRROR = 0x141,
    DPP_ROW_MIRROR = 0x140,
};

__device__ __forceinline__ float min_f32(float a, float b) {
    float r;
    asm("v_min_f32 %0, %1, %2" : "=v"(r) : "v"(a), "v"(b));
    return r;
}
__device__ __forceinline__ float max_f32(float a, float b) {
    float r;
    asm("v_max_f32 %0, %1, %2" : "=v"(r) : "v"(a), "v"(b));
    return r;
}

__device__ __forceinline__ float row16_max(float v) {
    float r;
    asm("s_nop 1\n\t"
        "v_max_f32_dpp %0, %1, %1 quad_perm:[1,0,3,2] row_mask:0xf bank_mask:0xf\n\t"
        "s_nop 1\n\t"
        "v_max_f32_dpp %0, %0, %0 quad_perm:[2,3,0,1] row_mask:0xf bank_mask:0xf\n\t"
        "s_nop 1\n\t"
        "v_max_f32_dpp %0, %0, %0 row_half_mirror row_mask:0xf bank_mask:0xf\n\t"
        "s_nop 1\n\t"
        "v_max_f32_dpp %0, %0, %0 row_mirror row_mask:0xf bank_mask:0xf"
        : "=&v"(r) : "v"(v));
    return r;
}

__device__ __forceinline__ float readlane_f(float v, int lane) {
    return __builtin_bit_cast(float, __builtin_amdgcn_readlane(__builtin_bit_cast(int, v), lane));
}

#ifndef WS3D_WAVE_MAX_BCAST
#define WS3D_WAVE_MAX_BCAST 1
#endif
__device__ __forceinline__ float wave_max(float v) {
#if WS3D_WAVE_MAX_BCAST
    float r;
    asm("s_nop 1\n\t"
        "v_max_f32_dpp %0, %1, %1 quad_perm:[1,0,3,2] row_mask:0xf bank_mask:0xf\n\t"
        "s_nop 1\n\t"
        "v_max_f32_dpp %0, %0, %0 quad_perm:[2,3,0,1] row_mask:0xf bank_mask:0xf\n\t"
        "s_nop 1\n\t"
        "v_max_f32_dpp %0, %0, %0 row_half_mirror row_mask:0xf bank_mask:0xf\n\t"
        "s_nop 1\n\t"
        "v_max_f32_dpp %0, %0, %0 row_mirror row_mask:0xf bank_mask:0xf\n\t"
        "s_nop 1\n\t"
        "v_max_f32_dpp %0, %0, %0 row_bcast:15 row_mask:0xa bank_mask:0xf\n\t"
        "s_nop 1\n\t"
        "v_max_f32_dpp %0, %0, %0 row_bcast:31 row_mask:0xc bank_mask:0xf"
        : "=&v"(r) : "v"(v));
    return readlane_f(r, 63);
#else
    v = row16_max(v);
    const float a = readlane_f(v, 0), b = readlane_f(v, 16), c = readlane_f(v, 32), d = readlane_f(v, 48);
    return max_f32(max_f32(a, b), max_f32(c, d));
#endif
}

__device__ __forceinline__ void lds_barrier() {
    asm volatile("s_waitcnt lgkmcnt(0)\n\ts_barrier" ::: "memory");
}

__device__ __forceinline__ int lane_id() { return (int)__lane_id(); }

__device__ __forceinline__ int mbcnt(uint64_t mask) {
    return (int)__builtin_amdgcn_mbcnt_hi((uint32_t)(mask >> 32),
                                          __builtin_amdgcn_mbcnt_lo((uint32_t)mask, 0u));
}

}
```

### ws3d_amd/csrc/gemm_rows.hip

```cpp
#include "common.h"
#include "split_bf16.h"

namespace ws3d {

typedef unsigned rows_u4 __attribute__((ext_vector_type(4)));
typedef float rows_f4 __attribute__((ext_vector_type(4)));

constexpr int GR_THREADS = 256;
constexpr int GR_TM = 64;
constexpr int GR_KB = 32;
constexpr int GR_FRAG = 1024;
#ifndef WS3D_GR_TALL_MIN_TILES
#define WS3D_GR_TALL_MIN_TILES 512
#endif
constexpr int GR_TALL_MIN_TILES = WS3D_GR_TALL_MIN_TILES;
constexpr int GR_MAX_DIM = 4096;
__host__ __device__ constexpr int gr_tile_rows(int nbt, int mbw) { return nbt == 4 ? 32 * mbw : 64 * mbw; }
__host__ __device__ constexpr int gr_a_stage(int tm) { return tm / 32 * 2 * 3 * GR_FRAG; }
__host__ __device__ constexpr int gr_lds_bytes(int tm) { return 2 * gr_a_stage(tm); }
static_assert(gr_lds_bytes(128) <= 64 * 1024 && gr_lds_bytes(128) * 2 <= 160 * 1024, "inside the default per-workgroup cap, two workgroups per CU");

__global__ __launch_bounds__(256) void gemm_rows_pack_kernel(int K, int N, const float *__restrict__ wt, rows_u4 *__restrict__ pack) {
    const int nb_all = N / 32;
    const long total = (long)(K / GR_KB) * nb_all * 2 * 64;
    for (long i = (long)blockIdx.x * blockDim.x + threadIdx.x; i < total; i += (long)gridDim.x * blockDim.x) {
        const int lane = (int)(i & 63), s = (int)((i >> 6) & 1);
        const long f = i >> 7;
        const int nb = (int)(f % nb_all), kb = (int)(f / nb_all);
        const int col = nb * 32 + (lane & 31), k0 = kb * GR_KB + 16 * s + 8 * (lane >> 5);
        float v[8];
#pragma unroll
        for (int j = 0; j < 8; ++j) v[j] = wt[(long)(k0 + j) * N + col];
        bf16x8 q1, q2, q3;
        split8(v, q1, q2, q3);
        rows_u4 *dst = pack + ((f * 2 + s) * 3) * 64 + lane;
        dst[0] = __builtin_bit_cast(rows_u4, q1);
        dst[64] = __builtin_bit_cast(rows_u4, q2);
        dst[128] = __builtin_bit_cast(rows_u4, q3);
    }
}

template <int NBT, int MBW>
__global__ __launch_bounds__(GR_THREADS, 2) void gemm_rows_kernel(int K, int N, int ntn, const float *__restrict__ a, const rows_u4 *__restrict__ pack,
                                                                  const float *__restrict__ bias, int relu, float *__restrict__ out) {
    extern __shared__ __attribute__((aligned(16))) unsigned char smem_rows[];
    constexpr int TM = gr_tile_rows(NBT, MBW);
    constexpr int UNITS = TM / 64;
    constexpr int STAGE = gr_a_stage(TM);
    const int tid = threadIdx.x, w = tid >> 6, lane = tid & 63, r = lane & 31, h = lane >> 5;
    const int tn = (int)(blockIdx.x % (unsigned)ntn);
    const long tm = blockIdx.x / (unsigned)ntn;
    const int nb_all = N / 32, nkb = K / GR_KB;
    const int nbl = NBT == 4 ? w : (w & 1), mb0 = NBT == 4 ? 0 : (w >> 1) * MBW;

    const int srow = (lane & 7) + 8 * (lane >> 5) + 16 * w, skq = (lane >> 3) & 3;
    const rows_f4 *ap = reinterpret_cast<const rows_f4 *>(a + (tm * TM + srow) * (long)K + 8 * skq);
    const size_t a_unit = (size_t)16 * K;
    const int a_wr = ((srow >> 5) * 2 + (skq >> 1)) * 3 * GR_FRAG + ((skq & 1) * 32 + (srow & 31)) * 16;
    const rows_u4 *wp = pack + (size_t)(tn * NBT + nbl) * 6 * 64 + lane;
    const size_t w_kb = (size_t)nb_all * 6 * 64;

    floatx16 acc[MBW];
#pragma unroll
    for (int m = 0; m < MBW; ++m)
#pragma unroll
        for (int i = 0; i < 16; ++i) acc[m][i] = 0.f;
    rows_u4 wc[6];
#pragma unroll
    for (int i = 0; i < 6; ++i) wc[i] = rows_u4{0u, 0u, 0u, 0u};

    for (int kb = -1; kb < nkb; ++kb) {
        const bool more = kb + 1 < nkb;
        rows_f4 ra[UNITS][2];
        rows_u4 wn[6];
        if (more) {
#pragma unroll
            for (int u = 0; u < UNITS; ++u) {
                ra[u][0] = ap[u * a_unit + (kb + 1) * (GR_KB / 4)];
                ra[u][1] = ap[u * a_unit + (kb + 1) * (GR_KB / 4) + 1];
            }
#pragma unroll
            for (int i = 0; i < 6; ++i) wn[i] = wp[(kb + 1) * w_kb + i * 64];
        }
        if (kb >= 0) {
            const unsigned char *buf = smem_rows + (kb & 1) * STAGE + lane * 16;
#pragma unroll
            for (int s = 0; s < 2; ++s) {
                const bf16x8 w1 = __builtin_bit_cast(bf16x8, wc[3 * s]), w2 = __builtin_bit_cast(bf16x8, wc[3 * s + 1]),
                               w3 = __builtin_bit_cast(bf16x8, wc[3 * s + 2]);
                bf16x8 a1[MBW], a2[MBW], a3[MBW];
#pragma unroll
                for (int m = 0; m < MBW; ++m) {
                    const unsigned char *af = buf + ((mb0 + m) * 2 + s) * 3 * GR_FRAG;
                    a1[m] = *reinterpret_cast<const bf16x8 *>(af);
                    a2[m] = *reinterpret_cast<const bf16x8 *>(af + GR_FRAG);
                    a3[m] = *reinterpret_cast<const bf16x8 *>(af + 2 * GR_FRAG);
                }
                split_mfma6<MBW>(w1, w2, w3, a1, a2, a3, acc);
            }
        }
        if (more) {
            unsigned char *nxt = smem_rows + ((kb + 1) & 1) * STAGE + a_wr;
#pragma unroll
            for (int u = 0; u < UNITS; ++u) {
                const float v[8] = {ra[u][0][0], ra[u][0][1], ra[u][0][2], ra[u][0][3], ra[u][1][0], ra[u][1][1], ra[u][1][2], ra[u][1][3]};
                bf16x8 q1, q2, q3;
                split8(v, q1, q2, q3);
                *reinterpret_cast<bf16x8 *>(nxt + u * 12 * GR_FRAG) = q1;
                *reinterpret_cast<bf16x8 *>(nxt + u * 12 * GR_FRAG + GR_FRAG) = q2;
                *reinterpret_cast<bf16x8 *>(nxt + u * 12 * GR_FRAG + 2 * GR_FRAG) = q3;
            }
#pragma unroll
            for (int i = 0; i < 6; ++i) wc[i] = wn[i];
        }
        __syncthreads();
    }

    const int n0 = (tn * NBT + nbl) * 32 + 4 * h;
    rows_f4 b4[4];
    if (bias) {
#pragma unroll
        for (int g = 0; g < 4; ++g) b4[g] = *reinterpret_cast<const rows_f4 *>(bias + n0 + 8 * g);
    }
#pragma unroll
    for (int m = 0; m < MBW; ++m) {
        float *orow = out + (tm * TM + (mb0 + m) * 32 + r) * (long)N + n0;
#pragma unroll
        for (int g = 0; g < 4; ++g) {
            rows_f4 y;
#pragma unroll
            for (int e = 0; e < 4; ++e) y[e] = acc[m][4 * g + e];
            if (bias) y = y + b4[g];
            if (relu) {
#pragma unroll
                for (int e = 0; e < 4; ++e) y[e] = relu_keep_nan(y[e]);
            }
            *reinterpret_cast<rows_f4 *>(orow + 8 * g) = y;
        }
    }
}

static bool gr_dims_ok(int K, int N) { return K >= GR_KB && K <= GR_MAX_DIM && K % GR_KB == 0 && N >= 64 && N <= GR_MAX_DIM && N % 64 == 0; }

}

extern "C" size_t ws3d_gemm_rows_pack_bytes(int k_dim, int n_dim) {
    return ws3d::gr_dims_ok(k_dim, n_dim) ? (size_t)k_dim * n_dim * 6 : 0;
}

extern "C" int ws3d_gemm_rows_pack(int k_dim, int n_dim, const float *wt, void *pack, ws3d_stream_t stream) {
    using namespace ws3d;
    if (!wt || !pack || (reinterpret_cast<uintptr_t>(pack) & 15) || (reinterpret_cast<uintptr_t>(wt) & 3)) {
        set_error("ws3d_gemm_rows_pack: invalid argument");
        return WS3D_E_INVALID;
    }
    if (!gr_dims_ok(k_dim, n_dim)) {
        set_error("ws3d_gemm_rows_pack: unsupported shape K=%d N=%d (K %% 32, N %% 64, both <= %d)", k_dim, n_dim, GR_MAX_DIM);
        return WS3D_E_UNSUPPORTED;
    }
    const long threads = (long)(k_dim / GR_KB) * (n_dim / 32) * 128;
    hipLaunchKernelGGL(gemm_rows_pack_kernel, dim3((unsigned)((threads + 255) / 256)), dim3(256), 0, as_stream(stream), k_dim, n_dim, wt,
                       static_cast<rows_u4 *>(pack));
    return check_launch("ws3d_gemm_rows_pack");
}

extern "C" int ws3d_gemm_rows_split(long rows, int k_dim, int n_dim, const float *a, const void *pack, const float *bias, int relu, float *out,
                                    ws3d_stream_t stream) {
    using namespace ws3d;
    if (rows < 0 || k_dim <= 0 || n_dim <= 0 || !a || !pack || !out) {
        set_error("ws3d_gemm_rows_split: invalid argument (rows=%ld K=%d N=%d)", rows, k_dim, n_dim);
        return WS3D_E_INVALID;
    }
    const uintptr_t al = reinterpret_cast<uintptr_t>(a) | reinterpret_cast<uintptr_t>(pack) | reinterpret_cast<uintptr_t>(out) | reinterpret_cast<uintptr_t>(bias);
    const int nbt = n_dim % 128 == 0 ? 4 : 2;
    if (!gr_dims_ok(k_dim, n_dim) || rows % GR_TM || (al & 15) || (rows / GR_TM) * (n_dim / (32 * nbt)) > 0x7fffffffL) {
        set_error("ws3d_gemm_rows_split: unsupported shape or alignment (rows=%ld K=%d N=%d; rows %% 64, K %% 32, N %% 64, 16-byte pointers)", rows,
                  k_dim, n_dim);
        return WS3D_E_UNSUPPORTED;
    }
    if (rows == 0) return WS3D_OK;
    const int ntn = n_dim / (32 * nbt);
    const bool tall = nbt == 4 && rows % 128 == 0 && (rows / 128) * ntn >= GR_TALL_MIN_TILES;
    const int tm = tall ? 128 : 64;
    const unsigned grid = (unsigned)((rows / tm) * ntn);
    auto go = [&](auto kern) -> int {
        hipLaunchKernelGGL(kern, dim3(grid), dim3(GR_THREADS), (size_t)gr_lds_bytes(tm), as_stream(stream), k_dim, n_dim, ntn, a,
                           static_cast<const rows_u4 *>(pack), bias, relu ? 1 : 0, out);
        return WS3D_OK;
    };
    if (int rc = nbt == 2 ? go(gemm_rows_kernel<2, 1>) : tall ? go(gemm_rows_kernel<4, 4>) : go(gemm_rows_kernel<4, 2>)) return rc;
    return check_launch("ws3d_gemm_rows_split");
}
```

### ws3d_amd/fastpath.py

```python
from __future__ import annotations

import contextlib
import contextvars

import torch
import torch.nn as nn

from . import compat as _C
from . import nn_blocks, pn2_ops

FUSED_SA_MLP = True
SA1_FROM_LISTS = True
FUSED_GEMM_POOL = True
FUSED_INTERP_GEMM = True
NESTED_FPS = True
GEOMETRY_AHEAD = True
_AHEAD_OVERRIDE = contextvars.ContextVar("ws3d_geometry_ahead", default=None)


@contextlib.contextmanager
def geometry_ahead(on: bool):
    token = _AHEAD_OVERRIDE.set(bool(on))
    try:
        yield
    finally:
        _AHEAD_OVERRIDE.reset(token)


@contextlib.contextmanager
def compact_only_scales(keys):
    token = _COMPACT_ONLY.set(frozenset(keys))
    try:
        yield
    finally:
        _COMPACT_ONLY.reset(token)


def primed_compact_scales(net, pointcloud: torch.Tensor, margin: float = None):
    margin = PRIMED_MARGIN if margin is None else margin
    keys, per_level = set(), {}
    for row in list_fill(net, pointcloud):
        si = per_level.get(row["level"], 0)
        per_level[row["level"]] = si + 1
        if row["fill"] <= margin * COMPACT_MAX_FILL:
            keys.add((row["level"] - 1, si))
    return frozenset(keys)


def _geometry_ahead_now() -> bool:
    v = _AHEAD_OVERRIDE.get()
    return GEOMETRY_AHEAD if v is None else v
GEOMETRY_IN_CAPTURE = False
PER_POINT_L1 = True
COMPACT_MAX_FILL = 0.55
COMPACT_PAIRS = True
PAIR_DISPATCH = "device"
PRIMED_MARGIN = 0.85
_COMPACT_ONLY = contextvars.ContextVar("ws3d_compact_only_scales", default=frozenset())
CHAIN_MLP = True
PAIRED_SCALES = True
MERGED_THREE_NN = True
FUSED_PROLOGUE = True
MERGED_BINNING = True
PER_POINT_FP = True
FUSED_MLP2_ROWS = True
FUSED_HEADS = True
SPLIT_GEMMS = True
FUSED_GATHER_GEMM2 = True
BIN_INPUT_AHEAD = True
FUSED_QINTERP_GEMM_MIN_ROWS = 30000
FUSED_COMPACT3_MAX_LDS = 64 * 1024
FUSED_GATHER_GEMM = True
GRID_MIN_N = 256
DUAL_SCALE_SEARCH = True
NESTED_CHAIN = True
QUERY_CELL_ORDER = True
PARALLEL_SCALES = True
PARALLEL_HEADS = True


def _row_weights(block):
    w, shift, act = block._folded()
    if act is not None and not isinstance(act, nn.ReLU):
        raise NotImplementedError("fast path supports ReLU / no activation only")
    cache = block.__dict__.get("_row_cache")
    if cache is None or cache[0] is not w:
        cache = (w, w.t().contiguous())
        if not torch.cuda.is_current_stream_capturing():
            block.__dict__["_row_cache"] = cache
    return cache[1], shift, act is not None


def _row_weights_xyz_last(block):
    wt, bias, relu = _row_weights(block)
    cache = block.__dict__.get("_row_cache_xyz_last")
    if cache is None or cache[0] is not wt:
        cache = (wt, torch.cat((wt[3:], wt[:3]), dim=0).contiguous())
        if not torch.cuda.is_current_stream_capturing():
            block.__dict__["_row_cache_xyz_last"] = cache
    return cache[1], bias, relu


def _split_rows(block, wt: torch.Tensor, c2: int):
    cache = block.__dict__.get("_split_cache")
    if cache is None or cache[0] is not wt or cache[1] != c2:
        cache = (wt, c2, wt[:c2].contiguous(), wt[c2:].contiguous())
        if not torch.cuda.is_current_stream_capturing():
            block.__dict__["_split_cache"] = cache
    return cache[2], cache[3]


_SPLIT_GEMM_LIBRARY_WINS = frozenset({(512, 1024, 512)})


def _split_gemm_wins(rows: int, k: int, n: int) -> bool:
    return (rows, k, n) not in _SPLIT_GEMM_LIBRARY_WINS


def _split_gemm(x2d: torch.Tensor, holder, key: str, wt: torch.Tensor, bias=None, relu: bool = False):
    if not SPLIT_GEMMS or x2d.dim() != 2 or not _split_gemm_wins(x2d.size(0), wt.size(0), wt.size(1)):
        return None
    packs = holder.__dict__.get("_gemm_rows_packs")
    ent = None if packs is None else packs.get(key)
    if ent is None or ent[0] is not wt:
        if torch.cuda.is_current_stream_capturing():
            return None
        ent = (wt, _C.gemm_rows_pack(wt))
        holder.__dict__.setdefault("_gemm_rows_packs", {})[key] = ent
    if ent[1] is None:
        return None
    return _C.gemm_rows_split(x2d, ent[1], wt.size(1), bias, relu)


def gemm_rows_packs(model):
    return [ent[1] for m in model.modules() for ent in m.__dict__.get("_gemm_rows_packs", {}).values() if ent[1] is not None]


def _layer(x2d: torch.Tensor, block) -> torch.Tensor:
    wt, bias, relu = _row_weights(block)
    y = _split_gemm(x2d, block, "row", wt, bias, relu)
    if y is not None:
        return y
    if bias is None:
        y = torch.mm(x2d, wt)
        return torch.relu_(y) if relu else y
    if relu:
        return torch._addmm_activation(bias, x2d, wt, use_gelu=False)
    return torch.addmm(bias, x2d, wt)


def _blocks(seq):
    return [m for m in seq if isinstance(m, nn_blocks._ConvBlock)]


def mlp_rows(x2d: torch.Tensor, seq, ticket=None) -> torch.Tensor:
    blocks = _blocks(seq)
    if FUSED_MLP2_ROWS and len(blocks) == 2 and x2d.size(1) == 128 and x2d.is_contiguous():
        (w1, b1, r1), (w2, b2, r2) = _row_weights(blocks[0]), _row_weights(blocks[1])
        y = _C.mlp2_rows(x2d, w1, b1, r1, w2, b2, r2, ticket)
        if y is not None:
            return y
    for blk in blocks:
        x2d = _layer(x2d, blk)
    return x2d


def _heads_blob(seq):
    blocks = _blocks(seq)
    if len(blocks) != 2:
        return None
    (w1, b1, r1), (w2, b2, r2) = _row_weights(blocks[0]), _row_weights(blocks[1])
    cache = blocks[0].__dict__.get("_heads_blob")
    if cache is None or cache[0] is not w1 or cache[1] is not b1 or cache[2] is not w2 or cache[3] is not b2:
        cache = (w1, b1, w2, b2, _C.rpn_heads_pack(w1, b1, r1, w2, b2, r2), w2.size(1))
        if not torch.cuda.is_current_stream_capturing():
            blocks[0].__dict__["_heads_blob"] = cache
    return None if cache[4] is None else (cache[4], cache[5])


def heads_blobs(rpn):
    return [blk.__dict__["_heads_blob"][4] for seq in (rpn.rpn_cls_layer, rpn.rpn_reg_layer) for blk in _blocks(seq)[:1]
            if "_heads_blob" in blk.__dict__]


def _fused_heads(rows: torch.Tensor, blobs, which: int, tickets):
    if blobs is None or not all(blobs[i] is not None for i in (0, 1) if which & (1 << i)):
        return None
    (bc, oc), (br, orr) = blobs[0] or (None, 1), blobs[1] or (None, 0)
    if oc != 1 or (which & 2 and orr == 1):
        return None
    return _C.rpn_heads(rows, which, bc, br, orr, tickets, _C.tune("mlp2_wgs") * (2 if which == 3 else 1))


def supported(model) -> bool:
    try:
        for m in model.modules():
            if isinstance(m, nn_blocks._ConvBlock):
                if not m._pointwise or not isinstance(getattr(m, "activation", None), (nn.ReLU, type(None))):
                    return False
        for sa in model.rpn.backbone_net.SA_modules:
            if sa.pool_method != "max_pool" or sa.npoint is None:
                return False
            for g, mlp in zip(sa.groupers, sa.mlps):
                if not isinstance(g, pn2_ops.QueryAndGroup) or any(b.conv.out_channels % 4 for b in _blocks(mlp)):
                    return False
        return True
    except AttributeError:
        return False


def _gather_gemm_ok(sa, grouper, blocks, c_feat: int, B: int) -> bool:
    return (FUSED_GATHER_GEMM and c_feat >= 16 and c_feat % 4 == 0 and grouper.use_xyz and len(blocks) >= 2 and
            blocks[0].conv.out_channels % 64 == 0 and (B * sa.npoint * grouper.nsample) % 64 == 0 and
            (B * sa.npoint * grouper.nsample) // 64 <= 65535)


def _pair_limit(rows: int, dense_available: bool, key=None) -> int:
    if PAIR_DISPATCH != "device" or not dense_available or (key is not None and key in _COMPACT_ONLY.get()):
        return -1
    return max(0, int(COMPACT_MAX_FILL * rows))


@torch.no_grad()
def list_fill(net, pointcloud: torch.Tensor):
    xyz = pointcloud[..., 0:3].contiguous()
    rows = []
    for level, sa in enumerate(net.SA_modules):
        _, new_xyz = (pn2_ops.furthest_point_sample_gather_nested if NESTED_FPS and level >= 1 else pn2_ops.furthest_point_sample_gather)(xyz, sa.npoint)
        srt = pn2_ops.sort_points_x(xyz)
        for g in sa.groupers:
            nbr = _C.ball_query_lists(g.radius, g.nsample, xyz, new_xyz, srt)
            total = _C.compact_pairs(nbr)[2]
            rows.append({"level": level + 1, "n": xyz.size(1), "npoint": sa.npoint, "radius": float(g.radius), "nsample": g.nsample,
                         "distinct_per_list": float(total.item()) / max(nbr.numel() // g.nsample, 1),
                         "fill": float(total.item()) / max(nbr.numel(), 1)})
        xyz = new_xyz
    return rows


class _ZeroArena:

    def __init__(self, numel: int, device, clear: bool = True):
        n = (max(int(numel), 4) + 3) & ~3
        self.buf = (torch.zeros if clear else torch.empty)(n, dtype=torch.float32, device=device)
        self.dirty = not clear
        self.off = 0
        self.fallbacks = 0

    def ensure_clear(self):
        if self.dirty:
            self.buf.zero_()
            self.dirty = False

    def take(self, shape, dtype=torch.float32):
        n = 1
        for d in shape:
            n *= int(d)
        if self.off + n > self.buf.numel():
            self.fallbacks += 1
            self.fallback_shapes = getattr(self, "fallback_shapes", []) + [(tuple(shape), self.off, self.buf.numel())]
            return torch.zeros(shape, dtype=dtype, device=self.buf.device)
        v = self.buf[self.off:self.off + n]
        self.off += (n + 3) & ~3
        return (v if dtype == torch.float32 else v.view(dtype)).view(shape)


LAST_ARENA_FALLBACKS = 0


def _arena_for(net, B: int, device, extra: int = 0, clear: bool = True) -> _ZeroArena:
    n = extra + 64
    if COMPACT_PAIRS:
        for sa in net.SA_modules:
            n += B * sa.npoint * sum(_blocks(mlp)[-1].conv.out_channels for mlp in sa.mlps) + 4
            n += 4 * len(sa.groupers)
        if CHAIN_MLP:
            n += _C.chain_ticket_ints() + 4
    return _ZeroArena(n, device, clear)


class _PairList:
    __slots__ = ("nbr", "pairs")

    def __init__(self, nbr, pairs):
        self.nbr, self.pairs = nbr, pairs


def _per_point_l1(sa, feats: torch.Tensor, nbrs):
    B, N, C = feats.shape
    wts = [(_row_weights_xyz_last(_blocks(mlp)[0])[0] if nbr is not None else None) for mlp, nbr in zip(sa.mlps, nbrs)]
    cache = sa.__dict__.get("_pp_cache")
    if cache is None or len(cache[0]) != len(wts) or any(a is not b for a, b in zip(cache[0], wts)):
        used = [w for w in wts if w is not None]
        wcat = torch.cat([w[:C] for w in used], dim=1).contiguous()
        offs, w1xs, o = [], [], 0
        for w in wts:
            offs.append(o if w is not None else -1)
            w1xs.append(w[C:C + 3].contiguous() if w is not None else None)
            o += w.size(1) if w is not None else 0
        cache = (wts, wcat, offs, w1xs)
        if not torch.cuda.is_current_stream_capturing():
            sa.__dict__["_pp_cache"] = cache
    p = _split_gemm(feats.view(B * N, C), sa, "pp", cache[1])
    return (p if p is not None else torch.mm(feats.view(B * N, C), cache[1])), cache[2], cache[3]


def _lists_and_pairs(radius, nsample, xyz, new_xyz, sorted_xyz, zeros=None):
    total = zeros.take((1,), torch.int32) if zeros is not None else None
    both = _C.ball_query_pairs(radius, nsample, xyz, new_xyz, sorted_xyz, total)
    if both is not None:
        return both
    nbr = _C.ball_query_lists(radius, nsample, xyz, new_xyz, sorted_xyz)
    return nbr, _C.compact_pairs(nbr)


def _neighbour_lists(sa, xyz, new_xyz, sorted_xyz, c_feat: int, zeros=None):
    B = xyz.size(0)
    lists = []
    want_pairs = [(_gather_gemm_ok(sa, g, _blocks(mlp), c_feat, B) and COMPACT_PAIRS and PER_POINT_L1 and _blocks(mlp)[0].conv.out_channels <= 256
                   and len(_blocks(mlp)) == 3) for g, mlp in zip(sa.groupers, sa.mlps)]
    if DUAL_SCALE_SEARCH and len(want_pairs) == 2 and all(want_pairs) and sorted_xyz is not None:
        totals = [zeros.take((1,), torch.int32) for _ in range(2)] if zeros is not None else None
        both = _C.ball_query_pairs2([g.radius for g in sa.groupers], [g.nsample for g in sa.groupers], xyz, new_xyz, sorted_xyz, totals)
        if both is not None:
            return [_PairList(nbr, pairs) for nbr, pairs in both]
    for grouper, mlp in zip(sa.groupers, sa.mlps):
        if not _gather_gemm_ok(sa, grouper, _blocks(mlp), c_feat, B):
            lists.append(None)
            continue
        if COMPACT_PAIRS and PER_POINT_L1 and _blocks(mlp)[0].conv.out_channels <= 256 and len(_blocks(mlp)) == 3:
            nbr, pairs = _lists_and_pairs(grouper.radius, grouper.nsample, xyz, new_xyz, sorted_xyz, zeros)
            lists.append(_PairList(nbr, pairs))
        else:
            lists.append(_C.ball_query_lists(grouper.radius, grouper.nsample, xyz, new_xyz, sorted_xyz))
    return lists


def _side_streams(main: torch.cuda.Stream, count: int = 3, fresh: bool = False):
    from .streams import pass_streams
    return pass_streams(main, count, fresh)


class _Geometry:

    def __init__(self, net, xyz: torch.Tensor, c0: int, zeros=None):
        sas = list(net.SA_modules)
        main = torch.cuda.current_stream(xyz.device)
        s_fps, s_search, s_aux = _side_streams(main, fresh=True)
        self.aux = s_aux
        self.xyz = [xyz]
        srt0 = ev0 = None
        if BIN_INPUT_AHEAD:
            pre = torch.cuda.Event()
            pre.record(main)
        _, nx = pn2_ops.furthest_point_sample_gather(xyz, sas[0].npoint)
        if BIN_INPUT_AHEAD:
            s_search.wait_event(pre)
            with torch.cuda.stream(s_search):
                srt0 = pn2_ops.sort_points_x(xyz)
                ev0 = torch.cuda.Event()
                ev0.record(s_search)
        self.xyz.append(nx)
        start = torch.cuda.Event()
        start.record(main)
        fps_done = [start]
        s_fps.wait_event(start)
        with torch.cuda.stream(s_fps):
            if NESTED_FPS and NESTED_CHAIN and len(sas) > 1:
                for _, nx in pn2_ops.furthest_point_sample_gather_nested_chain(self.xyz[-1], [sa.npoint for sa in sas[1:]]):
                    self.xyz.append(nx)
                ev = torch.cuda.Event()
                ev.record(s_fps)
                fps_done.extend([ev] * (len(sas) - 1))
            else:
                for sa in sas[1:]:
                    _, nx = (pn2_ops.furthest_point_sample_gather_nested if NESTED_FPS else pn2_ops.furthest_point_sample_gather)(self.xyz[-1], sa.npoint)
                    self.xyz.append(nx)
                    ev = torch.cuda.Event()
                    ev.record(s_fps)
                    fps_done.append(ev)
        self.sorted, self.nbr, self.sa_ready = [srt0], [None], [ev0]
        self.nn, self.nn_ready = [], []
        c_feat = [c0] + [sum(_blocks(mlp)[-1].conv.out_channels for mlp in sa.mlps) for sa in sas]
        with torch.cuda.stream(s_search):
            for i in range(1, len(sas)):
                s_search.wait_event(fps_done[i - 1])
                srt = pn2_ops.sort_points_x(self.xyz[i], GRID_MIN_N)
                self.sorted.append(srt)
                s_search.wait_event(fps_done[i])
                self.nbr.append(_neighbour_lists(sas[i], self.xyz[i], self.xyz[i + 1], srt, c_feat[i], zeros))
                ev = torch.cuda.Event()
                ev.record(s_search)
                self.sa_ready.append(ev)
            self.nn, self.nn_ready = [None] * len(sas), [None] * len(sas)
            for i in range(len(sas) - 1, -1, -1):
                self.nn[i] = _C.three_nn_with_weights(self.xyz[i], self.xyz[i + 1], pn2_ops.sort_points_xz(self.xyz[i + 1]),
                                                      self.sorted[i] if QUERY_CELL_ORDER else None)
                ev = torch.cuda.Event()
                ev.record(s_search)
                self.nn_ready[i] = ev
        self.main, self.side = main, (s_fps, s_search, s_aux)

    def release(self):
        if torch.cuda.is_current_stream_capturing():
            return
        done = torch.cuda.Event()
        done.record(self.main)
        for s in self.side:
            s.wait_event(done)


def sa_forward(sa, xyz: torch.Tensor, feats: torch.Tensor, geo: _Geometry = None, level: int = 0, zeros: _ZeroArena = None, binned: list = None,
               new_xyz_pre: torch.Tensor = None, prebinned=None):
    B = xyz.size(0)
    c_feat = 0 if feats is None else feats.size(2)
    if geo is not None:
        new_xyz = geo.xyz[level + 1]
        if level >= 1:
            geo.main.wait_event(geo.sa_ready[level])
            sorted_xyz, nbrs = geo.sorted[level], geo.nbr[level]
        else:
            if geo.sa_ready[0] is not None:
                geo.main.wait_event(geo.sa_ready[0])
            sorted_xyz = geo.sorted[0] if geo.sa_ready[0] is not None else pn2_ops.sort_points_x(xyz)
            nbrs = _neighbour_lists(sa, xyz, new_xyz, None, c_feat, zeros)
    else:
        if new_xyz_pre is not None:
            new_xyz = new_xyz_pre
        else:
            _, new_xyz = (pn2_ops.furthest_point_sample_gather_nested if NESTED_FPS and level >= 1 else pn2_ops.furthest_point_sample_gather)(xyz, sa.npoint)
        sorted_xyz = prebinned[0] if prebinned is not None else pn2_ops.sort_points_x(xyz, GRID_MIN_N)
        nbrs = _neighbour_lists(sa, xyz, new_xyz, sorted_xyz, c_feat, zeros)
    if binned is not None:
        binned.append(sorted_xyz)
    widths = [_blocks(mlp)[-1].conv.out_channels for mlp in sa.mlps]
    if not COMPACT_PAIRS:
        out = torch.empty((B * sa.npoint, sum(widths)), dtype=torch.float32, device=xyz.device)
    elif zeros is not None:
        out = zeros.take((B * sa.npoint, sum(widths)))
    else:
        out = torch.zeros((B * sa.npoint, sum(widths)), dtype=torch.float32, device=xyz.device)
    cols = [sum(widths[:i]) for i in range(len(widths))]
    pp = [None]
    sa1_pairs = {}
    if (DUAL_SCALE_SEARCH and COMPACT_PAIRS and FUSED_SA_MLP and SA1_FROM_LISTS and len(widths) == 2 and feats is not None and feats.size(2) == 1
            and sorted_xyz is not None and all(n_ is None for n_ in nbrs) and all(g_.use_xyz and len(_blocks(m_)) == 3 for g_, m_ in zip(sa.groupers, sa.mlps))):
        totals = [zeros.take((1,), torch.int32) for _ in range(2)] if zeros is not None else None
        both = _C.ball_query_pairs2([g_.radius for g_ in sa.groupers], [g_.nsample for g_ in sa.groupers], xyz, new_xyz, sorted_xyz, totals)
        if both is not None:
            sa1_pairs = dict(enumerate(both))

    def run_scale(si: int) -> None:
        grouper, mlp, width, nbr, col = sa.groupers[si], sa.mlps[si], widths[si], nbrs[si], cols[si]
        blocks = _blocks(mlp)
        pairs = None
        if isinstance(nbr, _PairList):
            nbr, pairs = nbr.nbr, nbr.pairs
        if nbr is not None:
            wt1, b1, r1 = _row_weights_xyz_last(blocks[0])
            if PER_POINT_L1 and len(blocks) >= 3:
                if pp[0] is None:
                    pp[0] = _per_point_l1(sa, feats, nbrs)
                pmat, offs, w1xs = pp[0]
                o1 = blocks[0].conv.out_channels
                y = None
                wt3, b3, r3 = _row_weights(blocks[-1])
                if pairs is not None and o1 <= 256 and len(blocks) == 3 and r3:
                    wt2, b2, r2 = _row_weights(blocks[1])
                    rows, ns, o3 = nbr.numel(), grouper.nsample, wt3.size(1)
                    dense_ok = (o1 in (64, 128) and (sa.npoint * ns) % 64 == 0 and rows // 64 <= 65535 and o3 % 64 == 0 and
                                wt2.size(1) % 4 == 0 and ns in (16, 32))
                    limit = _pair_limit(rows, dense_ok, (level, si))
                    fused = _C.pgather_gemm3_compact(pmat, offs[si], o1, xyz, new_xyz, pairs, w1xs[si], b1, r1, wt2, b2, r2, wt3, b3, out, col,
                                                     limit=limit, max_lds=FUSED_COMPACT3_MAX_LDS)
                    yc = None if fused else _C.pgather_gemm2_compact(pmat, offs[si], o1, xyz, new_xyz, pairs, w1xs[si], b1, r1, wt2, b2, r2, limit=limit)
                    if fused or (yc is not None and _C.gemm_pool_compact(yc, pairs, wt3, b3, out, col, limit=limit)):
                        if limit >= 0:
                            gate = (pairs[2], limit)
                            yd = _C.pgather_gemm2(pmat, offs[si], o1, xyz, new_xyz, nbr, w1xs[si], b1, r1, wt2, b2, r2, out=yc, gate=gate)
                            if yd is None or not _C.gemm_pool(yd, wt3, b3, r3, ns, out, col, gate=gate):
                                yc = _C.pgather_gemm2_compact(pmat, offs[si], o1, xyz, new_xyz, pairs, w1xs[si], b1, r1, wt2, b2, r2, limit=-1)
                                if yc is None or not _C.gemm_pool_compact(yc, pairs, wt3, b3, out, col, limit=-1):
                                    raise RuntimeError("neither the gated dense nor the ungated compact kernels took the shape")
                        return
                if o1 <= 128:
                    wt2, b2, r2 = _row_weights(blocks[1])
                    y = _C.pgather_gemm2(pmat, offs[si], o1, xyz, new_xyz, nbr, w1xs[si], b1, r1, wt2, b2, r2)
                    rest_pp = blocks[2:-1]
                if y is None:
                    y = _C.pgather_rows(pmat, offs[si], o1, xyz, new_xyz, nbr, w1xs[si], b1, r1)
                    rest_pp = blocks[1:-1]
                if y is not None:
                    for blk in rest_pp:
                        y = _layer(y, blk)
                    wt, bias, relu = _row_weights(blocks[-1])
                    if not (FUSED_GEMM_POOL and _C.gemm_pool(y, wt, bias, relu, grouper.nsample, out, col)):
                        _C.rowmax_rows(_layer(y, blocks[-1]), grouper.nsample, out, col)
                    return
            y = None
            rest = blocks[1:-1]
            if FUSED_GATHER_GEMM2 and len(blocks) >= 3 and blocks[0].conv.out_channels <= 128:
                wt2, b2, r2 = _row_weights(blocks[1])
                y = _C.gather_gemm2(feats, xyz, new_xyz, nbr, wt1, b1, r1, wt2, b2, r2)
                if y is not None:
                    rest = blocks[2:-1]
            if y is None:
                y = _C.gather_gemm(feats, xyz, new_xyz, nbr, wt1, b1, r1)
            if y is not None:
                for blk in rest:
                    y = _layer(y, blk)
                wt, bias, relu = _row_weights(blocks[-1])
                if not (FUSED_GEMM_POOL and _C.gemm_pool(y, wt, bias, relu, grouper.nsample, out, col)):
                    _C.rowmax_rows(_layer(y, blocks[-1]), grouper.nsample, out, col)
                return
        if FUSED_SA_MLP and SA1_FROM_LISTS and feats is not None and feats.size(2) == 1 and grouper.use_xyz and len(blocks) == 3:
            layers = [_row_weights(b) for b in blocks]
            if not COMPACT_PAIRS:
                nbr1 = _C.ball_query_lists(grouper.radius, grouper.nsample, xyz, new_xyz, sorted_xyz)
                if _C.sa_mlp3_pool_lists(xyz, new_xyz, feats, nbr1, layers, out, col):
                    return
            else:
                nbr1, pairs1 = sa1_pairs[si] if si in sa1_pairs else _lists_and_pairs(grouper.radius, grouper.nsample, xyz, new_xyz, sorted_xyz, zeros)
                limit = _pair_limit(nbr1.numel(), layers[2][2] and nbr1.numel() % 32 == 0 and grouper.nsample in (16, 32), (level, si))
                if _C.sa_mlp3_pool_compact(xyz, new_xyz, feats, pairs1, layers, out, col, limit=limit):
                    if limit >= 0 and not _C.sa_mlp3_pool_lists(xyz, new_xyz, feats, nbr1, layers, out, col, gate=(pairs1[2], limit)):
                        if not _C.sa_mlp3_pool_compact(xyz, new_xyz, feats, pairs1, layers, out, col, limit=-1):
                            raise RuntimeError("neither ws3d_sa_mlp3_pool_lists nor the ungated compact kernel took the shape")
                    return
        g = _C.query_and_group_nlc(grouper.radius, grouper.nsample, xyz, new_xyz, feats, grouper.use_xyz, sorted_xyz)
        rows = g.view(-1, g.size(3))
        if not (FUSED_SA_MLP and rows.size(1) == 4 and len(blocks) == 3 and
                _C.sa_mlp3_pool(rows, grouper.nsample, [_row_weights(b) for b in blocks], out, col)):
            y = rows
            for blk in blocks[:-1]:
                y = _layer(y, blk)
            wt, bias, relu = _row_weights(blocks[-1])
            if not (FUSED_GEMM_POOL and _C.gemm_pool(y, wt, bias, relu, grouper.nsample, out, col)):
                _C.rowmax_rows(_layer(y, blocks[-1]), grouper.nsample, out, col)

    def run_paired() -> bool:
        if not (PAIRED_SCALES and COMPACT_PAIRS and PER_POINT_L1 and len(widths) == 2 and all(isinstance(n_, _PairList) for n_ in nbrs)):
            return False
        blk = [_blocks(m_) for m_ in sa.mlps]
        if any(len(b_) != 3 or b_[0].conv.out_channels > 256 for b_ in blk) or blk[0][0].conv.out_channels != blk[1][0].conv.out_channels:
            return False
        if any(_pair_limit(n_.nbr.numel(), True, (level, si_)) != -1 for si_, n_ in enumerate(nbrs)):
            return False
        if pp[0] is None:
            pp[0] = _per_point_l1(sa, feats, nbrs)
        pmat, offs, w1xs = pp[0]
        scales = []
        for si_ in range(2):
            _w1, b1, r1 = _row_weights_xyz_last(blk[si_][0])
            wt2, b2, r2 = _row_weights(blk[si_][1])
            wt3, b3, r3 = _row_weights(blk[si_][2])
            if not r3:
                return False
            scales.append({"pmat": pmat, "col0": offs[si_], "o1": blk[si_][0].conv.out_channels, "xyz": xyz, "new_xyz": new_xyz, "pairs": nbrs[si_].pairs,
                           "w1x": w1xs[si_], "b1": b1, "relu1": r1, "w2t": wt2, "b2": b2, "relu2": r2, "w3t": wt3, "b3": b3, "out2d": out, "col_offset": cols[si_]})
        if (CHAIN_MLP and zeros is not None and all(sc_["o1"] == 64 and sc_["w2t"].size(1) <= 96 and sc_["w3t"].size(1) == 128 for sc_ in scales)
                and _C.chain_mlp3(scales, zeros.take((_C.chain_ticket_ints(),), torch.int32))):
            return True
        if _C.compact_mlp_pair(3, scales, max_lds=FUSED_COMPACT3_MAX_LDS):
            return True
        mids = _C.compact_mlp_pair(2, scales)
        if mids is None:
            return False
        if not _C.compact_mlp_pair(1, scales, mids=mids):
            for sc_, mid in zip(scales, mids):
                if not _C.gemm_pool_compact(mid, sc_["pairs"], sc_["w3t"], sc_["b3"], out, sc_["col_offset"], limit=-1):
                    raise RuntimeError("ws3d_gemm_pool_compact declined a shape ws3d_pgather_gemm2_compact took")
        return True

    if run_paired():
        pass
    elif geo is not None and geo.aux is not None and PARALLEL_SCALES and len(widths) == 2:
        if PER_POINT_L1 and any(n is not None and len(_blocks(m)) >= 3 for n, m in zip(nbrs, sa.mlps)):
            pp[0] = _per_point_l1(sa, feats, nbrs)
        fork = torch.cuda.Event()
        fork.record(geo.main)
        geo.aux.wait_event(fork)
        with torch.cuda.stream(geo.aux):
            run_scale(1)
            join = torch.cuda.Event()
            join.record(geo.aux)
        run_scale(0)
        geo.main.wait_event(join)
    else:
        for si in range(len(widths)):
            run_scale(si)
    return new_xyz, out.view(B, sa.npoint, -1)


def fp_forward(fp, unknown: torch.Tensor, known: torch.Tensor, unknown_feats, known_feats: torch.Tensor, nn3=None, sorted_unknown=None,
               known_xz=None):
    B, n = unknown.size(0), unknown.size(1)
    idx, weight = nn3 if nn3 is not None else _C.three_nn_with_weights(unknown, known, known_xz[0] if known_xz is not None else pn2_ops.sort_points_xz(known),
                                                                        sorted_unknown if QUERY_CELL_ORDER else None)
    c2 = known_feats.size(2)
    c1 = 0 if unknown_feats is None else unknown_feats.size(2)
    blocks = _blocks(fp.mlp)
    if PER_POINT_FP and blocks and blocks[0].conv.out_channels % 4 == 0:
        wt1, b1, r1 = _row_weights(blocks[0])
        wa, wb = _split_rows(blocks[0], wt1, c2)
        m = known_feats.size(1)
        q = _split_gemm(known_feats.reshape(B * m, c2), blocks[0], "wa", wa)
        q = (q if q is not None else torch.mm(known_feats.reshape(B * m, c2), wa)).view(B, m, -1)
        fuse2 = len(blocks) == 2 and B * n >= FUSED_QINTERP_GEMM_MIN_ROWS
        if fuse2:
            wt2, b2, r2 = _row_weights(blocks[1])
        if c1 > 4:
            lin = _split_gemm(unknown_feats.reshape(B * n, c1), blocks[0], "wb", wb, b1)
            if lin is None:
                lin = torch.mm(unknown_feats.reshape(B * n, c1), wb) if b1 is None else torch.addmm(b1, unknown_feats.reshape(B * n, c1), wb)
            y = _C.qinterp_gemm(q, idx, weight, wt2, b2, r2, lin=lin, relu=r1) if fuse2 else None
            if y is not None:
                return y.view(B, n, -1)
            y = _C.qinterp_rows(q, idx, weight, lin=lin, relu=r1)
        else:
            sk = None if c1 == 0 else unknown_feats.contiguous()
            y = _C.qinterp_gemm(q, idx, weight, wt2, b2, r2, skip=sk, wb=wb if c1 else None, bias=b1, relu=r1) if fuse2 else None
            if y is not None:
                return y.view(B, n, -1)
            y = _C.qinterp_rows(q, idx, weight, skip=sk, wb=wb if c1 else None, bias=b1, relu=r1)
        if y is not None:
            for blk in blocks[1:]:
                y = _layer(y, blk)
            return y.view(B, n, -1)
    if FUSED_INTERP_GEMM and blocks and blocks[0].conv.out_channels % 64 == 0 and B * n >= 8192:
        wt1, b1, r1 = _row_weights(blocks[0])
        y = _C.interp_gemm(known_feats.contiguous(), None if unknown_feats is None else unknown_feats.contiguous(), idx, weight, wt1, b1, r1)
        if y is not None:
            for blk in blocks[1:]:
                y = _layer(y, blk)
            return y.view(B, n, -1)
    cat = torch.empty((B, n, c2 + c1), dtype=torch.float32, device=unknown.device)
    _C.three_interpolate_nlc(known_feats, idx, weight, cat)
    if c1:
        cat[:, :, c2:] = unknown_feats
    return mlp_rows(cat.view(B * n, c2 + c1), fp.mlp).view(B, n, -1)


@torch.no_grad()
def backbone_forward(net, pointcloud: torch.Tensor, zeros: _ZeroArena = None):
    if FUSED_PROLOGUE and pointcloud.is_cuda and pointcloud.dim() == 3 and pointcloud.is_contiguous() and pointcloud.size(-1) > 3:
        if zeros is None:
            zeros = _arena_for(net, pointcloud.size(0), pointcloud.device, clear=False)
        xyz, feats = _C.split_points_clear(pointcloud, zeros.buf if zeros.dirty else None)
        zeros.dirty = False
    else:
        xyz = pointcloud[..., 0:3].contiguous()
        feats = pointcloud[..., 3:].contiguous() if pointcloud.size(-1) > 3 else None
        if zeros is None:
            zeros = _arena_for(net, xyz.size(0), xyz.device)
        zeros.ensure_clear()
    ahead = _geometry_ahead_now() and (GEOMETRY_IN_CAPTURE or not torch.cuda.is_current_stream_capturing())
    geo = _Geometry(net, xyz, 0 if feats is None else feats.size(2), zeros) if ahead else None
    l_xyz, l_feats, binned = [xyz], [feats], []
    try:
        sas, chain, pre_grid, pre_xz, nn_pre = list(net.SA_modules), None, {}, {}, {}
        for level, sa in enumerate(sas):
            pre = chain[level - 1][1] if (chain is not None and level >= 1) else None
            nx, nf = sa_forward(sa, l_xyz[-1], l_feats[-1], geo, level, zeros, binned, pre, pre_grid.get(level))
            l_xyz.append(nx)
            l_feats.append(nf)
            if geo is None and level == 0 and NESTED_FPS and NESTED_CHAIN and len(sas) > 1:
                chain = pn2_ops.furthest_point_sample_gather_nested_chain(nx, [s_.npoint for s_ in sas[1:]])
                if MERGED_BINNING:
                    lv = [nx] + [c[1] for c in chain]
                    jobs = [(x_, "grid") for x_ in lv[:-1] if x_.size(1) >= GRID_MIN_N] + [(x_, "xz") for x_ in lv if x_.size(1) >= 256]
                    bufs = iter(_C.sort_points_jobs(jobs) if _C.BQ_FINE_GRID else [])
                    if _C.BQ_FINE_GRID:
                        pre_grid = {k + 1: ((next(bufs),) if x_.size(1) >= GRID_MIN_N else (None,)) for k, x_ in enumerate(lv[:-1])}
                        pre_xz = {k + 1: (next(bufs) if x_.size(1) >= 256 else None) for k, x_ in enumerate(lv)}
                        if MERGED_THREE_NN:
                            allx = [l_xyz[0]] + lv
                            qgrid = {0: binned[0]}
                            qgrid.update({k_: v_[0] for k_, v_ in pre_grid.items()})
                            lvls = [k_ for k_ in range(len(sas)) if pre_xz.get(k_ + 1) is not None and allx[k_ + 1].size(1) <= 4096]
                            got = _C.three_nn_jobs([(allx[k_], allx[k_ + 1], pre_xz[k_ + 1], qgrid.get(k_) if QUERY_CELL_ORDER else None) for k_ in lvls])
                            if got is not None:
                                nn_pre = dict(zip(lvls, got))
        for i in range(-1, -(len(net.FP_modules) + 1), -1):
            lvl = len(l_xyz) + i - 1
            nn3 = nn_pre.get(lvl)
            if geo is not None:
                geo.main.wait_event(geo.nn_ready[lvl])
                nn3 = geo.nn[lvl]
            known_level = len(l_xyz) + i
            l_feats[i - 1] = fp_forward(net.FP_modules[i], l_xyz[i - 1], l_xyz[i], l_feats[i - 1], l_feats[i], nn3, binned[len(l_xyz) + i - 1],
                                        (pre_xz[known_level],) if known_level in pre_xz else None)
    finally:
        if geo is not None:
            geo.release()
    return l_xyz[0], l_feats[0]


@torch.no_grad()
def rpn_forward(model, pts_input: torch.Tensor, defer_reg_join: bool = False) -> dict:
    rpn = model.rpn
    zeros = _arena_for(rpn.backbone_net, pts_input.size(0), pts_input.device, extra=8, clear=not FUSED_PROLOGUE)
    xyz, feats = backbone_forward(rpn.backbone_net, pts_input, zeros)
    B, N, C = feats.shape
    rows = feats.view(B * N, C)
    tickets = zeros.take((2,), torch.int32) if (FUSED_MLP2_ROWS or FUSED_HEADS) else (None, None)
    blobs = (_heads_blob(rpn.rpn_cls_layer), _heads_blob(rpn.rpn_reg_layer)) if FUSED_HEADS else None
    reg_ready = None
    if PARALLEL_HEADS and _geometry_ahead_now() and not torch.cuda.is_current_stream_capturing():
        main = torch.cuda.current_stream(rows.device)
        aux = _side_streams(main)[2]
        fork = torch.cuda.Event()
        fork.record(main)
        aux.wait_event(fork)
        with torch.cuda.stream(aux):
            fused = _fused_heads(rows, blobs, 2, tickets)
            rpn_reg = (fused[1] if fused is not None else mlp_rows(rows, rpn.rpn_reg_layer, tickets[1:2])).view(B, N, -1)
            reg_ready = torch.cuda.Event()
            reg_ready.record(aux)
        rpn_reg.record_stream(main)
        fused = _fused_heads(rows, blobs, 1, tickets)
        rpn_cls = (fused[0] if fused is not None else mlp_rows(rows, rpn.rpn_cls_layer, tickets[0:1])).view(B, N, -1)
        if not defer_reg_join:
            main.wait_event(reg_ready)
            reg_ready = None
    else:
        fused = _fused_heads(rows, blobs, 3, tickets)
        if fused is not None:
            rpn_cls, rpn_reg = fused[0].view(B, N, -1), fused[1].view(B, N, -1)
        else:
            rpn_cls = mlp_rows(rows, rpn.rpn_cls_layer, tickets[0:1]).view(B, N, -1)
            rpn_reg = mlp_rows(rows, rpn.rpn_reg_layer, tickets[1:2]).view(B, N, -1)
    global LAST_ARENA_FALLBACKS
    LAST_ARENA_FALLBACKS = zeros.fallbacks if not zeros.fallbacks else getattr(zeros, "fallback_shapes", zeros.fallbacks)
    out = {"rpn_cls": rpn_cls, "rpn_reg": rpn_reg, "backbone_xyz": xyz,
           "backbone_features": feats.transpose(1, 2),
           "backbone_features_nlc": feats}
    if reg_ready is not None:
        out["rpn_reg_ready"] = reg_ready
    return out
```

Baseline: 6992.

## Fuse SA per-point GEMM with FP skip GEMM sharing the same input rows

```diff
diff --git a/include/ws3d_ops.h b/include/ws3d_ops.h
--- a/include/ws3d_ops.h
+++ b/include/ws3d_ops.h
@@ -236,6 +236,8 @@
 WS3D_API int ws3d_gemm_rows_pack(int k_dim, int n_dim, const float *wt, void *pack, ws3d_stream_t stream);
 WS3D_API int ws3d_gemm_rows_split(long rows, int k_dim, int n_dim, const float *a, const void *pack, const float *bias, int relu, float *out,
                          ws3d_stream_t stream);
+WS3D_API int ws3d_gemm_rows_split2(long rows, int k_dim, const float *a, int n0, const void *pack0, const float *bias0, int relu0, float *out0, int n1,
+                          const void *pack1, const float *bias1, int relu1, float *out1, ws3d_stream_t stream);
 
 WS3D_API int ws3d_qinterp_gemm(int b, int n, int m, int c, int o_dim, const float *q, const int32_t *idx, const float *weight, const float *lin,
                       const float *skip, int c1, const float *wb, const float *b1, int relu1, const float *w2t, const float *b2, int relu2,
diff --git a/ws3d_amd/_lib.py b/ws3d_amd/_lib.py
--- a/ws3d_amd/_lib.py
+++ b/ws3d_amd/_lib.py
@@ -77,6 +77,7 @@
     "ws3d_gemm_rows_pack_bytes": (_sz, [_i, _i]),
     "ws3d_gemm_rows_pack": (_i, [_i, _i, _vp, _vp, _vp]),
     "ws3d_gemm_rows_split": (_i, [C.c_long, _i, _i, _vp, _vp, _vp, _i, _vp, _vp]),
+    "ws3d_gemm_rows_split2": (_i, [C.c_long, _i, _vp, _i, _vp, _vp, _i, _vp, _i, _vp, _vp, _i, _vp, _vp]),
     "ws3d_decode_center_boxes": (_i, [_i, _i, _i, _f, _f, _f, _f, _f, _vp, _vp, _vp, _vp]),
     "ws3d_topk_sorted": (_i, [_i, _i, _i, _vp, _vp, _vp, _vp]),
     "ws3d_topk_workspace_bytes": (C.c_size_t, [_i, _i]),
diff --git a/ws3d_amd/build.py b/ws3d_amd/build.py
--- a/ws3d_amd/build.py
+++ b/ws3d_amd/build.py
@@ -18,7 +18,7 @@
 def lib_path(dist_mode: int = 0) -> str:
     return LIB if dist_mode == 0 else os.path.join(HERE, "libws3d_hip_dm%d.so" % dist_mode)
 ARCH = "gfx950"
-SOURCES = ["core.hip", "fps.hip", "fps_v3.hip", "fps_bucket.hip", "fps_nested.hip", "fps_ragged.hip", "fps_pruned.hip", "ballquery_group.hip", "interpolate.hip", "roipool3d.hip", "iou3d.hip", "proposals.hip", "scatter_det.hip", "sa_mlp.hip", "bn_relu.hip", "gemm_pool.hip", "conv_wgrad.hip", "chain_mlp.hip", "rpn_heads.hip", "gemm_rows.hip", "kitti_eval.hip", "instance_clouds.hip", "click.hip", "stage2.hip", "stage2_ragged.hip", "stage2_loss.hip", "rpn_targets.hip", "scan_prepare.hip"]
+SOURCES = ["core.hip", "fps.hip", "fps_v3.hip", "fps_bucket.hip", "fps_nested.hip", "fps_ragged.hip", "fps_pruned.hip", "ballquery_group.hip", "interpolate.hip", "roipool3d.hip", "iou3d.hip", "proposals.hip", "scatter_det.hip", "sa_mlp.hip", "bn_relu.hip", "gemm_pool.hip", "conv_wgrad.hip", "chain_mlp.hip", "rpn_heads.hip", "gemm_rows.hip", "gemm_rows_seg.hip", "kitti_eval.hip", "instance_clouds.hip", "click.hip", "stage2.hip", "stage2_ragged.hip", "stage2_loss.hip", "rpn_targets.hip", "scan_prepare.hip"]
 CXXFLAGS = ["-O3", "-std=c++17", "-fPIC", "-ffp-contract=off", "-fno-fast-math",
             "-fvisibility=hidden", "-Wall", "-Wno-unused-function"]
 
diff --git a/ws3d_amd/compat.py b/ws3d_amd/compat.py
--- a/ws3d_amd/compat.py
+++ b/ws3d_amd/compat.py
@@ -704,7 +704,7 @@
 
 
 CHAIN_WORKGROUPS = 0
-TUNE_KEYS = {"chain_wgs": 0, "mlp2_wgs": 1, "sa1_wgs": 2, "fp_wgs": 3, "pair_wgs": 4, "bq_wide_nw": 5}
+TUNE_KEYS = {"chain_wgs": 0, "mlp2_wgs": 1, "sa1_wgs": 2, "fp_wgs": 3, "pair_wgs": 4, "bq_wide_nw": 5, "gr_tall_min_tiles": 6}
 
 
 def tune(name: str, value: int = -1) -> int:
@@ -878,6 +878,36 @@
         return None
     check(rc, "gemm_rows_split")
     return out
+
+
+def gemm_rows_split2(x2d, pack0, n0, pack1, n1, bias0=None, relu0=False, bias1=None, relu1=False, out0=None, out1=None):
+    if pack0 is None or pack1 is None or x2d.dim() != 2 or not x2d.is_contiguous():
+        return None
+    n0, n1 = int(n0), int(n1)
+    for b, n in ((bias0, n0), (bias1, n1)):
+        if b is not None and (not b.is_contiguous() or b.numel() != n):
+            return None
+    dev = _dev(x2d, pack0, pack1, bias0, bias1, out0, out1)
+    _f32(x2d, "x2d")
+    R, K = x2d.shape
+    if R % 64 or K % 32 or n0 % 128 or n1 % 128 or min(pack0.numel() * pack0.element_size() // n0, pack1.numel() * pack1.element_size() // n1) < K * 6:
+        return None
+    outs = []
+    for b, o, n in ((bias0, out0, n0), (bias1, out1, n1)):
+        if b is not None:
+            _f32(b, "bias")
+        if o is None:
+            o = torch.empty((R, n), dtype=torch.float32, device=dev)
+        elif tuple(o.shape) != (R, n) or o.dtype != torch.float32 or not o.is_contiguous():
+            return None
+        outs.append(o)
+    with _on(dev):
+        rc = _lib.load().ws3d_gemm_rows_split2(R, K, _p(x2d), n0, _p(pack0), _p(bias0), int(bool(relu0)), _p(outs[0]), n1, _p(pack1), _p(bias1),
+                                               int(bool(relu1)), _p(outs[1]), _stream())
+    if rc == _lib.E_UNSUPPORTED:
+        return None
+    check(rc, "gemm_rows_split2")
+    return outs[0], outs[1]
 
 
 def pool_nsample(x):
diff --git a/ws3d_amd/csrc/common.h b/ws3d_amd/csrc/common.h
--- a/ws3d_amd/csrc/common.h
+++ b/ws3d_amd/csrc/common.h
@@ -15,7 +15,8 @@
 
 typedef float floatx16 __attribute__((ext_vector_type(16)));
 
-enum : int { TUNE_CHAIN_WGS = 0, TUNE_MLP2_WGS = 1, TUNE_SA1_WGS = 2, TUNE_FP_WGS = 3, TUNE_PAIR_WGS = 4, TUNE_BQ_WIDE_NW = 5, TUNE_COUNT = 8 };
+enum : int { TUNE_CHAIN_WGS = 0, TUNE_MLP2_WGS = 1, TUNE_SA1_WGS = 2, TUNE_FP_WGS = 3, TUNE_PAIR_WGS = 4, TUNE_BQ_WIDE_NW = 5, TUNE_GR_TALL_MIN_TILES = 6,
+              TUNE_COUNT = 8 };
 extern int g_tune[TUNE_COUNT];
 
 static inline hipStream_t as_stream(ws3d_stream_t s) { return reinterpret_cast<hipStream_t>(s); }
diff --git a/ws3d_amd/csrc/gemm_rows.hip b/ws3d_amd/csrc/gemm_rows.hip
--- a/ws3d_amd/csrc/gemm_rows.hip
+++ b/ws3d_amd/csrc/gemm_rows.hip
@@ -1,24 +1,6 @@
-#include "common.h"
-#include "split_bf16.h"
+#include "gemm_rows_tile.h"
 
 namespace ws3d {
-
-typedef unsigned rows_u4 __attribute__((ext_vector_type(4)));
-typedef float rows_f4 __attribute__((ext_vector_type(4)));
-
-constexpr int GR_THREADS = 256;
-constexpr int GR_TM = 64;
-constexpr int GR_KB = 32;
-constexpr int GR_FRAG = 1024;
-#ifndef WS3D_GR_TALL_MIN_TILES
-#define WS3D_GR_TALL_MIN_TILES 512
-#endif
-constexpr int GR_TALL_MIN_TILES = WS3D_GR_TALL_MIN_TILES;
-constexpr int GR_MAX_DIM = 4096;
-__host__ __device__ constexpr int gr_tile_rows(int nbt, int mbw) { return nbt == 4 ? 32 * mbw : 64 * mbw; }
-__host__ __device__ constexpr int gr_a_stage(int tm) { return tm / 32 * 2 * 3 * GR_FRAG; }
-__host__ __device__ constexpr int gr_lds_bytes(int tm) { return 2 * gr_a_stage(tm); }
-static_assert(gr_lds_bytes(128) <= 64 * 1024 && gr_lds_bytes(128) * 2 <= 160 * 1024, "inside the default per-workgroup cap, two workgroups per CU");
 
 __global__ __launch_bounds__(256) void gemm_rows_pack_kernel(int K, int N, const float *__restrict__ wt, rows_u4 *__restrict__ pack) {
     const int nb_all = N / 32;
@@ -44,103 +26,10 @@
 __global__ __launch_bounds__(GR_THREADS, 2) void gemm_rows_kernel(int K, int N, int ntn, const float *__restrict__ a, const rows_u4 *__restrict__ pack,
                                                                   const float *__restrict__ bias, int relu, float *__restrict__ out) {
     extern __shared__ __attribute__((aligned(16))) unsigned char smem_rows[];
-    constexpr int TM = gr_tile_rows(NBT, MBW);
-    constexpr int UNITS = TM / 64;
-    constexpr int STAGE = gr_a_stage(TM);
-    const int tid = threadIdx.x, w = tid >> 6, lane = tid & 63, r = lane & 31, h = lane >> 5;
     const int tn = (int)(blockIdx.x % (unsigned)ntn);
     const long tm = blockIdx.x / (unsigned)ntn;
-    const int nb_all = N / 32, nkb = K / GR_KB;
-    const int nbl = NBT == 4 ? w : (w & 1), mb0 = NBT == 4 ? 0 : (w >> 1) * MBW;
-
-    const int srow = (lane & 7) + 8 * (lane >> 5) + 16 * w, skq = (lane >> 3) & 3;
-    const rows_f4 *ap = reinterpret_cast<const rows_f4 *>(a + (tm * TM + srow) * (long)K + 8 * skq);
-    const size_t a_unit = (size_t)16 * K;
-    const int a_wr = ((srow >> 5) * 2 + (skq >> 1)) * 3 * GR_FRAG + ((skq & 1) * 32 + (srow & 31)) * 16;
-    const rows_u4 *wp = pack + (size_t)(tn * NBT + nbl) * 6 * 64 + lane;
-    const size_t w_kb = (size_t)nb_all * 6 * 64;
-
-    floatx16 acc[MBW];
-#pragma unroll
-    for (int m = 0; m < MBW; ++m)
-#pragma unroll
-        for (int i = 0; i < 16; ++i) acc[m][i] = 0.f;
-    rows_u4 wc[6];
-#pragma unroll
-    for (int i = 0; i < 6; ++i) wc[i] = rows_u4{0u, 0u, 0u, 0u};
-
-    for (int kb = -1; kb < nkb; ++kb) {
-        const bool more = kb + 1 < nkb;
-        rows_f4 ra[UNITS][2];
-        rows_u4 wn[6];
-        if (more) {
-#pragma unroll
-            for (int u = 0; u < UNITS; ++u) {
-                ra[u][0] = ap[u * a_unit + (kb + 1) * (GR_KB / 4)];
-                ra[u][1] = ap[u * a_unit + (kb + 1) * (GR_KB / 4) + 1];
-            }
-#pragma unroll
-            for (int i = 0; i < 6; ++i) wn[i] = wp[(kb + 1) * w_kb + i * 64];
-        }
-        if (kb >= 0) {
-            const unsigned char *buf = smem_rows + (kb & 1) * STAGE + lane * 16;
-#pragma unroll
-            for (int s = 0; s < 2; ++s) {
-                const bf16x8 w1 = __builtin_bit_cast(bf16x8, wc[3 * s]), w2 = __builtin_bit_cast(bf16x8, wc[3 * s + 1]),
-                               w3 = __builtin_bit_cast(bf16x8, wc[3 * s + 2]);
-                bf16x8 a1[MBW], a2[MBW], a3[MBW];
-#pragma unroll
-                for (int m = 0; m < MBW; ++m) {
-                    const unsigned char *af = buf + ((mb0 + m) * 2 + s) * 3 * GR_FRAG;
-                    a1[m] = *reinterpret_cast<const bf16x8 *>(af);
-                    a2[m] = *reinterpret_cast<const bf16x8 *>(af + GR_FRAG);
-                    a3[m] = *reinterpret_cast<const bf16x8 *>(af + 2 * GR_FRAG);
-                }
-                split_mfma6<MBW>(w1, w2, w3, a1, a2, a3, acc);
-            }
-        }
-        if (more) {
-            unsigned char *nxt = smem_rows + ((kb + 1) & 1) * STAGE + a_wr;
-#pragma unroll
-            for (int u = 0; u < UNITS; ++u) {
-                const float v[8] = {ra[u][0][0], ra[u][0][1], ra[u][0][2], ra[u][0][3], ra[u][1][0], ra[u][1][1], ra[u][1][2], ra[u][1][3]};
-                bf16x8 q1, q2, q3;
-                split8(v, q1, q2, q3);
-                *reinterpret_cast<bf16x8 *>(nxt + u * 12 * GR_FRAG) = q1;
-                *reinterpret_cast<bf16x8 *>(nxt + u * 12 * GR_FRAG + GR_FRAG) = q2;
-                *reinterpret_cast<bf16x8 *>(nxt + u * 12 * GR_FRAG + 2 * GR_FRAG) = q3;
-            }
-#pragma unroll
-            for (int i = 0; i < 6; ++i) wc[i] = wn[i];
-        }
-        __syncthreads();
-    }
-
-    const int n0 = (tn * NBT + nbl) * 32 + 4 * h;
-    rows_f4 b4[4];
-    if (bias) {
-#pragma unroll
-        for (int g = 0; g < 4; ++g) b4[g] = *reinterpret_cast<const rows_f4 *>(bias + n0 + 8 * g);
-    }
-#pragma unroll
-    for (int m = 0; m < MBW; ++m) {
-        float *orow = out + (tm * TM + (mb0 + m) * 32 + r) * (long)N + n0;
-#pragma unroll
-        for (int g = 0; g < 4; ++g) {
-            rows_f4 y;
-#pragma unroll
-            for (int e = 0; e < 4; ++e) y[e] = acc[m][4 * g + e];
-            if (bias) y = y + b4[g];
-            if (relu) {
-#pragma unroll
-                for (int e = 0; e < 4; ++e) y[e] = relu_keep_nan(y[e]);
-            }
-            *reinterpret_cast<rows_f4 *>(orow + 8 * g) = y;
-        }
-    }
+    gemm_rows_tile<NBT, MBW>(smem_rows, K, a, tm, pack, N / 32, bias, relu, out, N, tn);
 }
-
-static bool gr_dims_ok(int K, int N) { return K >= GR_KB && K <= GR_MAX_DIM && K % GR_KB == 0 && N >= 64 && N <= GR_MAX_DIM && N % 64 == 0; }
 
 }
 
@@ -180,8 +69,8 @@
     }
     if (rows == 0) return WS3D_OK;
     const int ntn = n_dim / (32 * nbt);
-    const bool tall = nbt == 4 && rows % 128 == 0 && (rows / 128) * ntn >= GR_TALL_MIN_TILES;
-    const int tm = tall ? 128 : 64;
+    const int tm = nbt == 4 ? gr_pick_tile_rows(rows, ntn) : 64;
+    const bool tall = tm == 128;
     const unsigned grid = (unsigned)((rows / tm) * ntn);
     auto go = [&](auto kern) -> int {
         hipLaunchKernelGGL(kern, dim3(grid), dim3(GR_THREADS), (size_t)gr_lds_bytes(tm), as_stream(stream), k_dim, n_dim, ntn, a,
diff --git a/ws3d_amd/csrc/gemm_rows_seg.hip b/ws3d_amd/csrc/gemm_rows_seg.hip
--- /dev/null
+++ b/ws3d_amd/csrc/gemm_rows_seg.hip
@@ -0,0 +1,56 @@
+#include "gemm_rows_tile.h"
+
+namespace ws3d {
+
+struct GrSeg {
+    const rows_u4 *pack;
+    const float *bias;
+    float *out;
+    int n, relu;
+};
+
+template <int MBW>
+__global__ __launch_bounds__(GR_THREADS, 2) void gemm_rows_seg_kernel(int K, int ntn0, int ntn, const float *__restrict__ a, GrSeg s0, GrSeg s1) {
+    extern __shared__ __attribute__((aligned(16))) unsigned char smem_rows[];
+    int tn = (int)(blockIdx.x % (unsigned)ntn);
+    const long tm = blockIdx.x / (unsigned)ntn;
+    const bool second = tn >= ntn0;
+    if (second) tn -= ntn0;
+    const GrSeg s = second ? s1 : s0;
+    gemm_rows_tile<4, MBW>(smem_rows, K, a, tm, s.pack, s.n / 32, s.bias, s.relu, s.out, s.n, tn);
+}
+
+}
+
+extern "C" int ws3d_gemm_rows_split2(long rows, int k_dim, const float *a, int n0, const void *pack0, const float *bias0, int relu0, float *out0, int n1,
+                                     const void *pack1, const float *bias1, int relu1, float *out1, ws3d_stream_t stream) {
+    using namespace ws3d;
+    if (rows < 0 || k_dim <= 0 || n0 <= 0 || n1 <= 0 || !a || !pack0 || !pack1 || !out0 || !out1) {
+        set_error("ws3d_gemm_rows_split2: invalid argument (rows=%ld K=%d N=%d, %d)", rows, k_dim, n0, n1);
+        return WS3D_E_INVALID;
+    }
+    const uintptr_t al = reinterpret_cast<uintptr_t>(a) | reinterpret_cast<uintptr_t>(pack0) | reinterpret_cast<uintptr_t>(pack1) | reinterpret_cast<uintptr_t>(out0) |
+                         reinterpret_cast<uintptr_t>(out1) | reinterpret_cast<uintptr_t>(bias0) | reinterpret_cast<uintptr_t>(bias1);
+    bool ok = gr_dims_ok(k_dim, n0) && gr_dims_ok(k_dim, n1) && n0 % 128 == 0 && n1 % 128 == 0 && rows % GR_TM == 0 && !(al & 15) &&
+              (rows / GR_TM) * ((n0 + n1) / 128) <= 0x7fffffffL;
+    if (ok) {
+        const uintptr_t b0 = reinterpret_cast<uintptr_t>(out0), e0 = b0 + (uintptr_t)rows * n0 * sizeof(float);
+        const uintptr_t b1 = reinterpret_cast<uintptr_t>(out1), e1 = b1 + (uintptr_t)rows * n1 * sizeof(float);
+        ok = rows == 0 || e0 <= b1 || e1 <= b0;
+    }
+    if (!ok) {
+        set_error("ws3d_gemm_rows_split2: unsupported shape, alignment or overlapping outputs (rows=%ld K=%d N=%d, %d; rows %% 64, K %% 32, N %% 128, "
+                  "16-byte pointers)", rows, k_dim, n0, n1);
+        return WS3D_E_UNSUPPORTED;
+    }
+    if (rows == 0) return WS3D_OK;
+    const GrSeg s0{static_cast<const rows_u4 *>(pack0), bias0, out0, n0, relu0 ? 1 : 0}, s1{static_cast<const rows_u4 *>(pack1), bias1, out1, n1, relu1 ? 1 : 0};
+    const int ntn0 = n0 / 128, ntn = ntn0 + n1 / 128;
+    const int tm = gr_pick_tile_rows(rows, ntn);
+    const unsigned grid = (unsigned)((rows / tm) * ntn);
+    if (tm == 128)
+        hipLaunchKernelGGL(gemm_rows_seg_kernel<4>, dim3(grid), dim3(GR_THREADS), (size_t)gr_lds_bytes(128), as_stream(stream), k_dim, ntn0, ntn, a, s0, s1);
+    else
+        hipLaunchKernelGGL(gemm_rows_seg_kernel<2>, dim3(grid), dim3(GR_THREADS), (size_t)gr_lds_bytes(64), as_stream(stream), k_dim, ntn0, ntn, a, s0, s1);
+    return check_launch("ws3d_gemm_rows_split2");
+}
diff --git a/ws3d_amd/csrc/gemm_rows_tile.h b/ws3d_amd/csrc/gemm_rows_tile.h
--- /dev/null
+++ b/ws3d_amd/csrc/gemm_rows_tile.h
@@ -0,0 +1,128 @@
+#pragma once
+#include "common.h"
+#include "split_bf16.h"
+
+namespace ws3d {
+
+typedef unsigned rows_u4 __attribute__((ext_vector_type(4)));
+typedef float rows_f4 __attribute__((ext_vector_type(4)));
+
+constexpr int GR_THREADS = 256;
+constexpr int GR_TM = 64;
+constexpr int GR_KB = 32;
+constexpr int GR_FRAG = 1024;
+#ifndef WS3D_GR_TALL_MIN_TILES
+#define WS3D_GR_TALL_MIN_TILES 512
+#endif
+constexpr int GR_TALL_MIN_TILES = WS3D_GR_TALL_MIN_TILES;
+constexpr int GR_MAX_DIM = 4096;
+__host__ __device__ constexpr int gr_tile_rows(int nbt, int mbw) { return nbt == 4 ? 32 * mbw : 64 * mbw; }
+__host__ __device__ constexpr int gr_a_stage(int tm) { return tm / 32 * 2 * 3 * GR_FRAG; }
+__host__ __device__ constexpr int gr_lds_bytes(int tm) { return 2 * gr_a_stage(tm); }
+static_assert(gr_lds_bytes(128) <= 64 * 1024 && gr_lds_bytes(128) * 2 <= 160 * 1024, "inside the default per-workgroup cap, two workgroups per CU");
+
+static inline bool gr_dims_ok(int K, int N) { return K >= GR_KB && K <= GR_MAX_DIM && K % GR_KB == 0 && N >= 64 && N <= GR_MAX_DIM && N % 64 == 0; }
+
+static inline int gr_pick_tile_rows(long rows, long ntn) {
+    const long min1 = g_tune[TUNE_GR_TALL_MIN_TILES] > 0 ? g_tune[TUNE_GR_TALL_MIN_TILES] : GR_TALL_MIN_TILES;
+    return (rows % 128 == 0 && (rows / 128) * ntn >= min1) ? 128 : 64;
+}
+
+template <int NBT, int MBW>
+__device__ __forceinline__ void gemm_rows_tile(unsigned char *smem_rows, int K, const float *__restrict__ a, long tm, const rows_u4 *__restrict__ pack,
+                                               int nb_all, const float *__restrict__ bias, int relu, float *__restrict__ out, int N, int tn) {
+    constexpr int TM = gr_tile_rows(NBT, MBW);
+    constexpr int UNITS = TM / 64;
+    constexpr int STAGE = gr_a_stage(TM);
+    const int tid = threadIdx.x, w = tid >> 6, lane = tid & 63, r = lane & 31, h = lane >> 5;
+    const int nkb = K / GR_KB;
+    const int nbl = NBT == 4 ? w : (w & 1), mb0 = NBT == 4 ? 0 : (w >> 1) * MBW;
+
+    const int srow = (lane & 7) + 8 * (lane >> 5) + 16 * w, skq = (lane >> 3) & 3;
+    const rows_f4 *ap = reinterpret_cast<const rows_f4 *>(a + (tm * TM + srow) * (long)K + 8 * skq);
+    const size_t a_unit = (size_t)16 * K;
+    const int a_wr = ((srow >> 5) * 2 + (skq >> 1)) * 3 * GR_FRAG + ((skq & 1) * 32 + (srow & 31)) * 16;
+    const rows_u4 *wp = pack + (size_t)(tn * NBT + nbl) * 6 * 64 + lane;
+    const size_t w_kb = (size_t)nb_all * 6 * 64;
+
+    floatx16 acc[MBW];
+#pragma unroll
+    for (int m = 0; m < MBW; ++m)
+#pragma unroll
+        for (int i = 0; i < 16; ++i) acc[m][i] = 0.f;
+    rows_u4 wc[6];
+#pragma unroll
+    for (int i = 0; i < 6; ++i) wc[i] = rows_u4{0u, 0u, 0u, 0u};
+
+    for (int kb = -1; kb < nkb; ++kb) {
+        const bool more = kb + 1 < nkb;
+        rows_f4 ra[UNITS][2];
+        rows_u4 wn[6];
+        if (more) {
+#pragma unroll
+            for (int u = 0; u < UNITS; ++u) {
+                ra[u][0] = ap[u * a_unit + (kb + 1) * (GR_KB / 4)];
+                ra[u][1] = ap[u * a_unit + (kb + 1) * (GR_KB / 4) + 1];
+            }
+#pragma unroll
+            for (int i = 0; i < 6; ++i) wn[i] = wp[(kb + 1) * w_kb + i * 64];
+        }
+        if (kb >= 0) {
+            const unsigned char *buf = smem_rows + (kb & 1) * STAGE + lane * 16;
+#pragma unroll
+            for (int s = 0; s < 2; ++s) {
+                const bf16x8 w1 = __builtin_bit_cast(bf16x8, wc[3 * s]), w2 = __builtin_bit_cast(bf16x8, wc[3 * s + 1]),
+                               w3 = __builtin_bit_cast(bf16x8, wc[3 * s + 2]);
+                bf16x8 a1[MBW], a2[MBW], a3[MBW];
+#pragma unroll
+                for (int m = 0; m < MBW; ++m) {
+                    const unsigned char *af = buf + ((mb0 + m) * 2 + s) * 3 * GR_FRAG;
+                    a1[m] = *reinterpret_cast<const bf16x8 *>(af);
+                    a2[m] = *reinterpret_cast<const bf16x8 *>(af + GR_FRAG);
+                    a3[m] = *reinterpret_cast<const bf16x8 *>(af + 2 * GR_FRAG);
+                }
+                split_mfma6<MBW>(w1, w2, w3, a1, a2, a3, acc);
+            }
+        }
+        if (more) {
+            unsigned char *nxt = smem_rows + ((kb + 1) & 1) * STAGE + a_wr;
+#pragma unroll
+            for (int u = 0; u < UNITS; ++u) {
+                const float v[8] = {ra[u][0][0], ra[u][0][1], ra[u][0][2], ra[u][0][3], ra[u][1][0], ra[u][1][1], ra[u][1][2], ra[u][1][3]};
+                bf16x8 q1, q2, q3;
+                split8(v, q1, q2, q3);
+                *reinterpret_cast<bf16x8 *>(nxt + u * 12 * GR_FRAG) = q1;
+                *reinterpret_cast<bf16x8 *>(nxt + u * 12 * GR_FRAG + GR_FRAG) = q2;
+                *reinterpret_cast<bf16x8 *>(nxt + u * 12 * GR_FRAG + 2 * GR_FRAG) = q3;
+            }
+#pragma unroll
+            for (int i = 0; i < 6; ++i) wc[i] = wn[i];
+        }
+        __syncthreads();
+    }
+
+    const int n0 = (tn * NBT + nbl) * 32 + 4 * h;
+    rows_f4 b4[4];
+    if (bias) {
+#pragma unroll
+        for (int g = 0; g < 4; ++g) b4[g] = *reinterpret_cast<const rows_f4 *>(bias + n0 + 8 * g);
+    }
+#pragma unroll
+    for (int m = 0; m < MBW; ++m) {
+        float *orow = out + (tm * TM + (mb0 + m) * 32 + r) * (long)N + n0;
+#pragma unroll
+        for (int g = 0; g < 4; ++g) {
+            rows_f4 y;
+#pragma unroll
+            for (int e = 0; e < 4; ++e) y[e] = acc[m][4 * g + e];
+            if (bias) y = y + b4[g];
+            if (relu) {
+#pragma unroll
+                for (int e = 0; e < 4; ++e) y[e] = relu_keep_nan(y[e]);
+            }
+            *reinterpret_cast<rows_f4 *>(orow + 8 * g) = y;
+        }
+    }
+}
+
+}
diff --git a/ws3d_amd/fastpath.py b/ws3d_amd/fastpath.py
--- a/ws3d_amd/fastpath.py
+++ b/ws3d_amd/fastpath.py
@@ -65,6 +65,7 @@
 PER_POINT_FP = True
 FUSED_MLP2_ROWS = True
 FUSED_HEADS = True
+SHARED_ROW_GEMMS = True
 SPLIT_GEMMS = True
 FUSED_GATHER_GEMM2 = True
 BIN_INPUT_AHEAD = True
@@ -120,6 +121,13 @@
 def _split_gemm(x2d: torch.Tensor, holder, key: str, wt: torch.Tensor, bias=None, relu: bool = False):
     if not SPLIT_GEMMS or x2d.dim() != 2 or not _split_gemm_wins(x2d.size(0), wt.size(0), wt.size(1)):
         return None
+    pack = _gemm_rows_pack_of(holder, key, wt)
+    if pack is None:
+        return None
+    return _C.gemm_rows_split(x2d, pack, wt.size(1), bias, relu)
+
+
+def _gemm_rows_pack_of(holder, key: str, wt: torch.Tensor):
     packs = holder.__dict__.get("_gemm_rows_packs")
     ent = None if packs is None else packs.get(key)
     if ent is None or ent[0] is not wt:
@@ -127,9 +135,24 @@
             return None
         ent = (wt, _C.gemm_rows_pack(wt))
         holder.__dict__.setdefault("_gemm_rows_packs", {})[key] = ent
-    if ent[1] is None:
-        return None
-    return _C.gemm_rows_split(x2d, ent[1], wt.size(1), bias, relu)
+    return ent[1]
+
+
+def _shared_row_gemms(x2d: torch.Tensor, sa, wcat: torch.Tensor, fp_block):
+    c1 = x2d.size(1)
+    if not (SHARED_ROW_GEMMS and SPLIT_GEMMS and PER_POINT_FP) or c1 <= 4 or fp_block.conv.out_channels % 4:
+        return None
+    wt1, b1, _r1 = _row_weights(fp_block)
+    if wt1.size(0) <= c1:
+        return None
+    _wa, wb = _split_rows(fp_block, wt1, wt1.size(0) - c1)
+    rows = x2d.size(0)
+    if not (_split_gemm_wins(rows, c1, wcat.size(1)) and _split_gemm_wins(rows, c1, wb.size(1))):
+        return None
+    pack_p, pack_b = _gemm_rows_pack_of(sa, "pp", wcat), _gemm_rows_pack_of(fp_block, "wb", wb)
+    if pack_p is None or pack_b is None:
+        return None
+    return _C.gemm_rows_split2(x2d, pack_p, wcat.size(1), pack_b, wb.size(1), bias1=b1)
 
 
 def gemm_rows_packs(model):
@@ -286,7 +309,7 @@
         self.nbr, self.pairs = nbr, pairs
 
 
-def _per_point_l1(sa, feats: torch.Tensor, nbrs):
+def _per_point_l1(sa, feats: torch.Tensor, nbrs, shared=None):
     B, N, C = feats.shape
     wts = [(_row_weights_xyz_last(_blocks(mlp)[0])[0] if nbr is not None else None) for mlp, nbr in zip(sa.mlps, nbrs)]
     cache = sa.__dict__.get("_pp_cache")
@@ -301,6 +324,11 @@
         cache = (wts, wcat, offs, w1xs)
         if not torch.cuda.is_current_stream_capturing():
             sa.__dict__["_pp_cache"] = cache
+    if shared is not None and shared[0] is not None and not shared[1]:
+        both = _shared_row_gemms(feats.view(B * N, C), sa, cache[1], shared[0])
+        if both is not None:
+            shared[1].append(both[1])
+            return both[0], cache[2], cache[3]
     p = _split_gemm(feats.view(B * N, C), sa, "pp", cache[1])
     return (p if p is not None else torch.mm(feats.view(B * N, C), cache[1])), cache[2], cache[3]
 
@@ -411,7 +439,7 @@
 
 
 def sa_forward(sa, xyz: torch.Tensor, feats: torch.Tensor, geo: _Geometry = None, level: int = 0, zeros: _ZeroArena = None, binned: list = None,
-               new_xyz_pre: torch.Tensor = None, prebinned=None):
+               new_xyz_pre: torch.Tensor = None, prebinned=None, shared=None):
     B = xyz.size(0)
     c_feat = 0 if feats is None else feats.size(2)
     if geo is not None:
@@ -460,7 +488,7 @@
             wt1, b1, r1 = _row_weights_xyz_last(blocks[0])
             if PER_POINT_L1 and len(blocks) >= 3:
                 if pp[0] is None:
-                    pp[0] = _per_point_l1(sa, feats, nbrs)
+                    pp[0] = _per_point_l1(sa, feats, nbrs, shared)
                 pmat, offs, w1xs = pp[0]
                 o1 = blocks[0].conv.out_channels
                 y = None
@@ -547,7 +575,7 @@
         if any(_pair_limit(n_.nbr.numel(), True, (level, si_)) != -1 for si_, n_ in enumerate(nbrs)):
             return False
         if pp[0] is None:
-            pp[0] = _per_point_l1(sa, feats, nbrs)
+            pp[0] = _per_point_l1(sa, feats, nbrs, shared)
         pmat, offs, w1xs = pp[0]
         scales = []
         for si_ in range(2):
@@ -576,7 +604,7 @@
         pass
     elif geo is not None and geo.aux is not None and PARALLEL_SCALES and len(widths) == 2:
         if PER_POINT_L1 and any(n is not None and len(_blocks(m)) >= 3 for n, m in zip(nbrs, sa.mlps)):
-            pp[0] = _per_point_l1(sa, feats, nbrs)
+            pp[0] = _per_point_l1(sa, feats, nbrs, shared)
         fork = torch.cuda.Event()
         fork.record(geo.main)
         geo.aux.wait_event(fork)
@@ -593,7 +621,7 @@
 
 
 def fp_forward(fp, unknown: torch.Tensor, known: torch.Tensor, unknown_feats, known_feats: torch.Tensor, nn3=None, sorted_unknown=None,
-               known_xz=None):
+               known_xz=None, lin=None):
     B, n = unknown.size(0), unknown.size(1)
     idx, weight = nn3 if nn3 is not None else _C.three_nn_with_weights(unknown, known, known_xz[0] if known_xz is not None else pn2_ops.sort_points_xz(known),
                                                                         sorted_unknown if QUERY_CELL_ORDER else None)
@@ -610,7 +638,8 @@
         if fuse2:
             wt2, b2, r2 = _row_weights(blocks[1])
         if c1 > 4:
-            lin = _split_gemm(unknown_feats.reshape(B * n, c1), blocks[0], "wb", wb, b1)
+            if lin is None or tuple(lin.shape) != (B * n, wb.size(1)) or wb.size(0) != c1:
+                lin = _split_gemm(unknown_feats.reshape(B * n, c1), blocks[0], "wb", wb, b1)
             if lin is None:
                 lin = torch.mm(unknown_feats.reshape(B * n, c1), wb) if b1 is None else torch.addmm(b1, unknown_feats.reshape(B * n, c1), wb)
             y = _C.qinterp_gemm(q, idx, weight, wt2, b2, r2, lin=lin, relu=r1) if fuse2 else None
@@ -658,10 +687,12 @@
     geo = _Geometry(net, xyz, 0 if feats is None else feats.size(2), zeros) if ahead else None
     l_xyz, l_feats, binned = [xyz], [feats], []
     try:
-        sas, chain, pre_grid, pre_xz, nn_pre = list(net.SA_modules), None, {}, {}, {}
+        sas, chain, pre_grid, pre_xz, nn_pre, lins = list(net.SA_modules), None, {}, {}, {}, {}
         for level, sa in enumerate(sas):
             pre = chain[level - 1][1] if (chain is not None and level >= 1) else None
-            nx, nf = sa_forward(sa, l_xyz[-1], l_feats[-1], geo, level, zeros, binned, pre, pre_grid.get(level))
+            lins[level] = []
+            shared = (_blocks(net.FP_modules[level].mlp)[:1] or [None])[0] if (SHARED_ROW_GEMMS and 1 <= level < len(net.FP_modules)) else None
+            nx, nf = sa_forward(sa, l_xyz[-1], l_feats[-1], geo, level, zeros, binned, pre, pre_grid.get(level), (shared, lins[level]))
             l_xyz.append(nx)
             l_feats.append(nf)
             if geo is None and level == 0 and NESTED_FPS and NESTED_CHAIN and len(sas) > 1:
@@ -689,7 +720,7 @@
                 nn3 = geo.nn[lvl]
             known_level = len(l_xyz) + i
             l_feats[i - 1] = fp_forward(net.FP_modules[i], l_xyz[i - 1], l_xyz[i], l_feats[i - 1], l_feats[i], nn3, binned[len(l_xyz) + i - 1],
-                                        (pre_xz[known_level],) if known_level in pre_xz else None)
+                                        (pre_xz[known_level],) if known_level in pre_xz else None, (lins.pop(lvl, None) or [None])[0])
     finally:
         if geo is not None:
             geo.release()
```

Result: no change. 6980 (-0.2%).
